# bogwi/sarpro

Measured on AMD Instinct MI355X. Metric: Mpix/s calibrate+CLAHE+synRGB, 400MP dual-pol scene; % HBM roofline, higher is better.
Workload: dtype f64

## Files before the change

### include/sarpro_hip.h

```cpp
#ifndef SARPRO_HIP_H
#define SARPRO_HIP_H

#include <stddef.h>
#include <stdint.h>

#ifdef __cplusplus
extern "C" {
#endif

#define SARPRO_HIP_OK 0
#define SARPRO_HIP_ERR_INVALID_ARG (-1)
#define SARPRO_HIP_ERR_SHAPE_MISMATCH (-2)
#define SARPRO_HIP_ERR_UNSUPPORTED_SHAPE (-3)
#define SARPRO_HIP_ERR_HIP (-4)
#define SARPRO_HIP_ERR_RCCL (-5)
#define SARPRO_HIP_ERR_OOM (-6)
#define SARPRO_HIP_ERR_NO_DEVICE (-7)
#define SARPRO_HIP_ERR_IO (-8)
#define SARPRO_HIP_ERR_BUFFER_TOO_SMALL (-9)

typedef enum {
    SARPRO_STRATEGY_STANDARD = 0,
    SARPRO_STRATEGY_ROBUST = 1,
    SARPRO_STRATEGY_ADAPTIVE = 2,
// ... 305 lines not shown
int sarpro_hip_stripe_run_resized_u16(sarpro_hip_ctx *ctx, const uint16_t *d_band1, const uint16_t *d_band2, size_t rows_total, size_t cols,
                                      size_t row0, size_t rows_local, size_t in_pitch, int strategy, int mode, size_t target_size, int pad,
                                      uint8_t *d_rgb_slice, size_t *out_row0, size_t *out_rows, sarpro_hip_resize_meta *meta);
int sarpro_hip_stripe_run_resized_f32(sarpro_hip_ctx *ctx, const float *d_band1, const float *d_band2, size_t rows_total, size_t cols, size_t row0,
                                      size_t rows_local, size_t in_pitch, int strategy, int mode, unsigned flags, size_t target_size, int pad,
                                      uint8_t *d_rgb_slice, size_t *out_row0, size_t *out_rows, sarpro_hip_resize_meta *meta);

int sarpro_hip_selftest_polop_division(sarpro_hip_ctx *ctx, uint64_t *mismatches_out);

typedef struct {
    uint64_t count;
    double sum_db, sumsq_db;
    float min_v, max_v;
} sarpro_hip_f32_partial;
typedef struct sarpro_hip_stripe_f32 sarpro_hip_stripe_f32;
int sarpro_hip_stripe_begin_f32(sarpro_hip_ctx *ctx, const float *d_in, size_t rows_total, size_t cols, size_t row0,
                                size_t rows_local, size_t in_pitch, int strategy, int bit_depth, void *d_out, size_t out_pitch,
                                sarpro_hip_stripe_f32 **out);
int sarpro_hip_stripe_begin_polop(sarpro_hip_ctx *ctx, int op, const void *d_a, const void *d_b, int elem_u16, size_t rows_total,
                                  size_t cols, size_t row0, size_t rows_local, size_t in_pitch, int strategy, int bit_depth,
                                  void *d_out, size_t out_pitch, sarpro_hip_stripe_f32 **out);
int sarpro_hip_stripe_f32_phase1(sarpro_hip_stripe_f32 *s, sarpro_hip_f32_partial *local_out);
int sarpro_hip_host_f32_merge_partials(const sarpro_hip_f32_partial *parts, size_t n, sarpro_hip_f32_partial *out);
int sarpro_hip_stripe_f32_phase2(sarpro_hip_stripe_f32 *s, const sarpro_hip_f32_partial *global, uint64_t **d_buf, size_t *count);
int sarpro_hip_stripe_f32_phase3(sarpro_hip_stripe_f32 *s, uint64_t **d_buf, size_t *count);
int sarpro_hip_stripe_f32_phase4(sarpro_hip_stripe_f32 *s, uint64_t **d_buf, size_t *count);
int sarpro_hip_stripe_f32_phase5(sarpro_hip_stripe_f32 *s, sarpro_hip_stats *stats_out);
void sarpro_hip_stripe_f32_end(sarpro_hip_stripe_f32 *s);
int sarpro_hip_stripe_run_f32(sarpro_hip_ctx *ctx, const float *d_in, size_t rows_total, size_t cols, size_t row0, size_t rows_local,
                              size_t in_pitch, int strategy, int bit_depth, void *d_out, size_t out_pitch, sarpro_hip_stats *stats_out);
int sarpro_hip_stripe_run_polop(sarpro_hip_ctx *ctx, int op, const void *d_a, const void *d_b, int elem_u16, size_t rows_total,
                                size_t cols, size_t row0, size_t rows_local, size_t in_pitch, int strategy, int bit_depth,
                                void *d_out, size_t out_pitch, sarpro_hip_stats *stats_out);

int sarpro_hip_comm_unique_id(uint8_t uid_out[128]);
int sarpro_hip_comm_init(sarpro_hip_ctx *ctx, int nranks, int rank, const uint8_t uid[128]);
int sarpro_hip_comm_allreduce_sum_u64(sarpro_hip_ctx *ctx, uint64_t *d_buf, size_t count);
typedef struct sarpro_hip_local_group sarpro_hip_local_group;
int sarpro_hip_local_group_create(int nranks, sarpro_hip_local_group **out);
void sarpro_hip_local_group_destroy(sarpro_hip_local_group *group);
int sarpro_hip_comm_init_local(sarpro_hip_ctx *ctx, sarpro_hip_local_group *group, int rank);
void sarpro_hip_comm_destroy(sarpro_hip_ctx *ctx);

int sarpro_hip_host_stats_from_dn_hist(const uint64_t dn_hist[65536], sarpro_hip_stats *out);
int sarpro_hip_host_window(sarpro_hip_stats *stats, int strategy, int tamed_synrgb);
int sarpro_hip_host_level_lut_u16(const sarpro_hip_stats *stats, int bit_depth, int tamed_synrgb,
                                  uint16_t lut_out[65536]);
int sarpro_hip_host_clahe_bin_lut_u16(const sarpro_hip_stats *stats, uint8_t lut_out[65536]);
int sarpro_hip_host_clahe_cdfs(const uint64_t *tile_hists, size_t rows, size_t cols,
                               double *cdfs_out);
int sarpro_hip_host_u8_rescale_lut(unsigned min_level, unsigned max_level, uint8_t lut_out[256]);
int sarpro_hip_host_synrgb_luts(int strategy, const uint64_t combined_hist[256], uint64_t n_per_band,
                                uint8_t *luts_out, int *floor_out);
int sarpro_hip_host_clahe_shape_ok(size_t rows, size_t cols);
int sarpro_hip_host_clahe_saturated_levels(size_t rows, size_t cols, uint8_t *col_class, uint8_t *row_bits);
int sarpro_hip_host_stripe_plan(size_t rows, int nranks, size_t *row0_out, size_t *nrows_out);

int sarpro_hip_host_stats_from_bins4096(uint64_t valid_count, double min_db, double max_db, double mean_db,
                                        double std_db, const uint64_t hist4096[4096], sarpro_hip_stats *out);
float sarpro_hip_host_f32_valid_threshold(void);
int sarpro_hip_host_f32_bin4096_thresholds(double min_db, double max_db, float thr_out[4096]);
int sarpro_hip_host_f32_level_thresholds(const sarpro_hip_stats *stats, int bit_depth, float *thr_out);
int sarpro_hip_host_f32_clahe_bin_thresholds(const sarpro_hip_stats *stats, float thr_out[256]);

int sarpro_hip_synth_scene_u16_dev(sarpro_hip_ctx *ctx, uint64_t seed, int band,
                                   const uint16_t *q_tables_host, size_t rows_total, size_t cols,
                                   size_t row0, size_t rows_local, uint16_t *d_out, size_t pitch);
#define SARPRO_HIP_SYNTH_NO_WEDGE 1u
#define SARPRO_HIP_SYNTH_NO_BRIGHT 2u
#define SARPRO_HIP_SYNTH_NO_BAND2 4u
#define SARPRO_HIP_SYNTH_MAP(m) (((unsigned)(m) & 15u) << 4)
#define SARPRO_HIP_SYNTH_BLOCKS(n) (((unsigned)(n) & 255u) << 8)
int sarpro_hip_synth_scene_u16_dev_ex(sarpro_hip_ctx *ctx, uint64_t seed, int band,
                                      const uint16_t *q_tables_host, size_t rows_total, size_t cols,
                                      size_t row0, size_t rows_local, uint16_t *d_out, size_t pitch, uint32_t flags);

#ifdef __cplusplus
}
#endif
#endif
```

### rust/sarpro-hip-sys/src/lib.rs

```rust
#![allow(non_camel_case_types, clippy::too_many_arguments)]

use std::os::raw::{c_char, c_int, c_uint, c_void};

pub const SARPRO_HIP_OK: c_int = 0;
pub const SARPRO_HIP_ERR_INVALID_ARG: c_int = -1;
pub const SARPRO_HIP_ERR_SHAPE_MISMATCH: c_int = -2;
pub const SARPRO_HIP_ERR_UNSUPPORTED_SHAPE: c_int = -3;
pub const SARPRO_HIP_ERR_HIP: c_int = -4;
pub const SARPRO_HIP_ERR_RCCL: c_int = -5;
pub const SARPRO_HIP_ERR_OOM: c_int = -6;
pub const SARPRO_HIP_ERR_NO_DEVICE: c_int = -7;
pub const SARPRO_HIP_ERR_IO: c_int = -8;
pub const SARPRO_HIP_ERR_BUFFER_TOO_SMALL: c_int = -9;
pub const SARPRO_HIP_CTX_TIMING: c_uint = 1;
pub const SARPRO_HIP_CTX_ASYNC_DEV: c_uint = 2;
pub const SARPRO_HIP_DUALPOL_PLAIN_PIPELINE: c_uint = 1;
pub const SARPRO_HIP_ROUTE_NONE: c_int = -1;
pub const SARPRO_HIP_ROUTE_ACCEPTED: c_int = 0;
pub const SARPRO_HIP_ROUTE_REFUTED: c_int = 1;
pub const SARPRO_HIP_ROUTE_UNPROVEN: c_int = 2;
pub const SARPRO_HIP_ROUTE_POOL_OVERFLOW: c_int = 3;
pub const SARPRO_HIP_ROUTE_RETRIED: c_int = 4;
pub const SARPRO_HIP_ERR_UNSUPPORTED: c_int = -10;
pub const SARPRO_HIP_SYNTH_NO_WEDGE: c_uint = 1;
pub const SARPRO_HIP_SYNTH_NO_BRIGHT: c_uint = 2;
pub const SARPRO_HIP_SYNTH_NO_BAND2: c_uint = 4;

pub const SARPRO_STRATEGY_STANDARD: c_int = 0;
pub const SARPRO_STRATEGY_ROBUST: c_int = 1;
pub const SARPRO_STRATEGY_ADAPTIVE: c_int = 2;
pub const SARPRO_STRATEGY_EQUALIZED: c_int = 3;
pub const SARPRO_STRATEGY_CLAHE: c_int = 4;
pub const SARPRO_STRATEGY_TAMED: c_int = 5;
pub const SARPRO_STRATEGY_DEFAULT: c_int = 6;
pub const SARPRO_BITDEPTH_U8: c_int = 0;
pub const SARPRO_BITDEPTH_U16: c_int = 1;
pub const SARPRO_OP_SUM: c_int = 0;
pub const SARPRO_OP_DIFF: c_int = 1;
pub const SARPRO_OP_RATIO: c_int = 2;
pub const SARPRO_OP_NDIFF: c_int = 3;
pub const SARPRO_OP_LOGRATIO: c_int = 4;
pub const SARPRO_SYNRGB_DEFAULT: c_int = 0;
pub const SARPRO_SYNRGB_RGB_RATIO: c_int = 1;
pub const SARPRO_SYNRGB_SAR_URBAN: c_int = 2;
pub const SARPRO_SYNRGB_ENHANCED: c_int = 3;
pub const SARPRO_READ_DEFAULT: c_int = -1;
pub const SARPRO_READ_AVERAGE: c_int = 0;
pub const SARPRO_READ_LANCZOS: c_int = 1;

#[repr(C)]
pub struct sarpro_hip_ctx { _private: [u8; 0] }
#[repr(C)]
pub struct sarpro_hip_stripe { _private: [u8; 0] }
#[repr(C)]
pub struct sarpro_hip_tiff { _private: [u8; 0] }
#[repr(C)]
pub struct sarpro_hip_tiff_writer { _private: [u8; 0] }
#[repr(C)]
pub struct sarpro_hip_stripe_f32 { _private: [u8; 0] }
#[repr(C)]
pub struct sarpro_hip_local_group { _private: [u8; 0] }

pub type sarpro_hip_row_reader = Option<unsafe extern "C" fn(user: *mut c_void, band: c_int, row0: usize, nrows: usize, dst: *mut u16, dst_pitch: usize) -> c_int>;
pub type sarpro_hip_row_sink = Option<unsafe extern "C" fn(user: *mut c_void, row0: usize, nrows: usize, src: *const u8, src_pitch_bytes: usize) -> c_int>;

#[repr(C)]
#[derive(Debug, Clone, Copy)]
pub struct sarpro_hip_stats {
    pub valid_count: u64,
    pub min_db: f64,
    pub max_db: f64,
    pub mean_db: f64,
    pub std_db: f64,
    pub median_db: f64,
    pub p01: f64,
    pub p02: f64,
// ... 181 lines not shown
    pub fn sarpro_hip_stripe_phase4(s: *mut sarpro_hip_stripe, d_rgb: *mut u8, rgb_pitch_px: usize, stats_out: *mut sarpro_hip_stats) -> c_int;
    pub fn sarpro_hip_stripe_end(s: *mut sarpro_hip_stripe);
    pub fn sarpro_hip_dualpol_synrgb_stream_u16(ctx: *mut sarpro_hip_ctx, reader: sarpro_hip_row_reader, reader_user: *mut c_void, rows: usize, cols: usize, strategy: c_int, mode: c_int, chunk_rows: usize, sink: sarpro_hip_row_sink, sink_user: *mut c_void, stats_out: *mut sarpro_hip_stats) -> c_int;
    pub fn sarpro_hip_dualpol_synrgb_resized_stream_u16(ctx: *mut sarpro_hip_ctx, reader: sarpro_hip_row_reader, reader_user: *mut c_void, rows: usize, cols: usize, strategy: c_int, mode: c_int, target_size: usize, pad: c_int, rgb_out: *mut u8, meta: *mut sarpro_hip_resize_meta) -> c_int;
    pub fn sarpro_hip_read_output_dims(cols: usize, rows: usize, target_size: usize, out_cols: *mut usize, out_rows: *mut usize, alg: *mut c_int) -> c_int;
    pub fn sarpro_hip_host_read_average_axis(n_src: usize, n_dst: usize, first: *mut u32, count: *mut u32, w_first: *mut f64, w_last: *mut f64, w_sum: *mut f64) -> c_int;
    pub fn sarpro_hip_read_average_u16_dev(ctx: *mut sarpro_hip_ctx, d_in: *const u16, rows: usize, cols: usize, in_pitch: usize, out_rows: usize, out_cols: usize, d_out_f32: *mut f32, out_pitch: usize) -> c_int;
    pub fn sarpro_hip_read_average_u16(ctx: *mut sarpro_hip_ctx, input: *const u16, rows: usize, cols: usize, out_rows: usize, out_cols: usize, out_f32: *mut f32) -> c_int;
    pub fn sarpro_hip_dualpol_synrgb_read_u16_dev(ctx: *mut sarpro_hip_ctx, d_band1: *const u16, d_band2: *const u16, rows: usize, cols: usize, in_pitch: usize, alg: c_int, strategy: c_int, mode: c_int, flags: c_uint, target_size: usize, pad: c_int, d_rgb_out: *mut u8, meta: *mut sarpro_hip_resize_meta) -> c_int;
    pub fn sarpro_hip_dualpol_synrgb_read_u16(ctx: *mut sarpro_hip_ctx, band1: *const u16, band2: *const u16, rows: usize, cols: usize, alg: c_int, strategy: c_int, mode: c_int, flags: c_uint, target_size: usize, pad: c_int, rgb_out: *mut u8, meta: *mut sarpro_hip_resize_meta) -> c_int;
    pub fn sarpro_hip_dualpol_synrgb_read_stream_u16(ctx: *mut sarpro_hip_ctx, reader: sarpro_hip_row_reader, reader_user: *mut c_void, rows: usize, cols: usize, alg: c_int, strategy: c_int, mode: c_int, flags: c_uint, target_size: usize, pad: c_int, rgb_out: *mut u8, meta: *mut sarpro_hip_resize_meta) -> c_int;
    pub fn sarpro_hip_dualpol_synrgb_read_stream_u16_jpeg(ctx: *mut sarpro_hip_ctx, reader: sarpro_hip_row_reader, reader_user: *mut c_void, rows: usize, cols: usize, alg: c_int, strategy: c_int, mode: c_int, flags: c_uint, target_size: usize, pad: c_int, jpeg_out: *mut u8, jpeg_capacity: usize, jpeg_bytes_out: *mut usize, restart_mcus: c_uint, meta: *mut sarpro_hip_resize_meta) -> c_int;
    pub fn sarpro_hip_tiff_open(path: *const c_char, out: *mut *mut sarpro_hip_tiff, info_out: *mut sarpro_hip_tiff_info) -> c_int;
    pub fn sarpro_hip_tiff_read_rows_u16(t: *mut sarpro_hip_tiff, sample: c_int, row0: usize, nrows: usize, dst: *mut u16, dst_pitch: usize) -> c_int;
    pub fn sarpro_hip_tiff_close(t: *mut sarpro_hip_tiff);
    pub fn sarpro_hip_tiff_pair_reader(user: *mut c_void, band: c_int, row0: usize, nrows: usize, dst: *mut u16, dst_pitch: usize) -> c_int;
    pub fn sarpro_hip_tiff_create(path: *const c_char, width: u64, height: u64, samples: u32, bits: u32, geotransform6: *const f64, geo_keys_from: *const sarpro_hip_tiff, out: *mut *mut sarpro_hip_tiff_writer) -> c_int;
    pub fn sarpro_hip_tiff_write_rows(w: *mut sarpro_hip_tiff_writer, row0: usize, nrows: usize, src: *const c_void, src_pitch_bytes: usize) -> c_int;
    pub fn sarpro_hip_tiff_row_sink(user: *mut c_void, row0: usize, nrows: usize, src: *const u8, src_pitch_bytes: usize) -> c_int;
    pub fn sarpro_hip_tiff_finish(w: *mut sarpro_hip_tiff_writer) -> c_int;
    pub fn sarpro_hip_tiff_last_error() -> *const c_char;
    pub fn sarpro_hip_host_parse_cpulist(s: *const c_char, cpus: *mut c_int, max: c_int) -> c_int;
    pub fn sarpro_hip_host_update_geotransform(gt: *mut f64, cols: usize, rows: usize, m: *const sarpro_hip_resize_meta);
    pub fn sarpro_hip_stripe_run_u16(ctx: *mut sarpro_hip_ctx, d_band1: *const u16, d_band2: *const u16, rows_total: usize, cols: usize, row0: usize, rows_local: usize, in_pitch: usize, strategy: c_int, mode: c_int, d_rgb: *mut u8, rgb_pitch_px: usize, stats_out: *mut sarpro_hip_stats) -> c_int;
    pub fn sarpro_hip_stripe_resized_rows(rows_total: usize, cols: usize, row0: usize, rows_local: usize, target_size: usize, pad: c_int, out_row0: *mut usize, out_rows: *mut usize, final_cols: *mut usize, final_rows: *mut usize) -> c_int;
    pub fn sarpro_hip_stripe_run_resized_u16(ctx: *mut sarpro_hip_ctx, d_band1: *const u16, d_band2: *const u16, rows_total: usize, cols: usize, row0: usize, rows_local: usize, in_pitch: usize, strategy: c_int, mode: c_int, target_size: usize, pad: c_int, d_rgb_slice: *mut u8, out_row0: *mut usize, out_rows: *mut usize, meta: *mut sarpro_hip_resize_meta) -> c_int;
    pub fn sarpro_hip_stripe_run_resized_f32(ctx: *mut sarpro_hip_ctx, d_band1: *const f32, d_band2: *const f32, rows_total: usize, cols: usize, row0: usize, rows_local: usize, in_pitch: usize, strategy: c_int, mode: c_int, flags: c_uint, target_size: usize, pad: c_int, d_rgb_slice: *mut u8, out_row0: *mut usize, out_rows: *mut usize, meta: *mut sarpro_hip_resize_meta) -> c_int;
    pub fn sarpro_hip_selftest_polop_division(ctx: *mut sarpro_hip_ctx, mismatches_out: *mut u64) -> c_int;
    pub fn sarpro_hip_stripe_begin_f32(ctx: *mut sarpro_hip_ctx, d_in: *const f32, rows_total: usize, cols: usize, row0: usize, rows_local: usize, in_pitch: usize, strategy: c_int, bit_depth: c_int, d_out: *mut c_void, out_pitch: usize, out: *mut *mut sarpro_hip_stripe_f32) -> c_int;
    pub fn sarpro_hip_stripe_begin_polop(ctx: *mut sarpro_hip_ctx, op: c_int, d_a: *const c_void, d_b: *const c_void, elem_u16: c_int, rows_total: usize, cols: usize, row0: usize, rows_local: usize, in_pitch: usize, strategy: c_int, bit_depth: c_int, d_out: *mut c_void, out_pitch: usize, out: *mut *mut sarpro_hip_stripe_f32) -> c_int;
    pub fn sarpro_hip_stripe_f32_phase1(s: *mut sarpro_hip_stripe_f32, local_out: *mut sarpro_hip_f32_partial) -> c_int;
    pub fn sarpro_hip_host_f32_merge_partials(parts: *const sarpro_hip_f32_partial, n: usize, out: *mut sarpro_hip_f32_partial) -> c_int;
    pub fn sarpro_hip_stripe_f32_phase2(s: *mut sarpro_hip_stripe_f32, global: *const sarpro_hip_f32_partial, d_buf: *mut *mut u64, count: *mut usize) -> c_int;
    pub fn sarpro_hip_stripe_f32_phase3(s: *mut sarpro_hip_stripe_f32, d_buf: *mut *mut u64, count: *mut usize) -> c_int;
    pub fn sarpro_hip_stripe_f32_phase4(s: *mut sarpro_hip_stripe_f32, d_buf: *mut *mut u64, count: *mut usize) -> c_int;
    pub fn sarpro_hip_stripe_f32_phase5(s: *mut sarpro_hip_stripe_f32, stats_out: *mut sarpro_hip_stats) -> c_int;
    pub fn sarpro_hip_stripe_f32_end(s: *mut sarpro_hip_stripe_f32);
    pub fn sarpro_hip_stripe_run_f32(ctx: *mut sarpro_hip_ctx, d_in: *const f32, rows_total: usize, cols: usize, row0: usize, rows_local: usize, in_pitch: usize, strategy: c_int, bit_depth: c_int, d_out: *mut c_void, out_pitch: usize, stats_out: *mut sarpro_hip_stats) -> c_int;
    pub fn sarpro_hip_stripe_run_polop(ctx: *mut sarpro_hip_ctx, op: c_int, d_a: *const c_void, d_b: *const c_void, elem_u16: c_int, rows_total: usize, cols: usize, row0: usize, rows_local: usize, in_pitch: usize, strategy: c_int, bit_depth: c_int, d_out: *mut c_void, out_pitch: usize, stats_out: *mut sarpro_hip_stats) -> c_int;
    pub fn sarpro_hip_comm_unique_id(uid_out: *mut u8) -> c_int;
    pub fn sarpro_hip_comm_init(ctx: *mut sarpro_hip_ctx, nranks: c_int, rank: c_int, uid: *const u8) -> c_int;
    pub fn sarpro_hip_comm_allreduce_sum_u64(ctx: *mut sarpro_hip_ctx, d_buf: *mut u64, count: usize) -> c_int;
    pub fn sarpro_hip_local_group_create(nranks: c_int, out: *mut *mut sarpro_hip_local_group) -> c_int;
    pub fn sarpro_hip_local_group_destroy(group: *mut sarpro_hip_local_group);
    pub fn sarpro_hip_comm_init_local(ctx: *mut sarpro_hip_ctx, group: *mut sarpro_hip_local_group, rank: c_int) -> c_int;
    pub fn sarpro_hip_comm_destroy(ctx: *mut sarpro_hip_ctx);
    pub fn sarpro_hip_host_stats_from_dn_hist(dn_hist: *const u64, out: *mut sarpro_hip_stats) -> c_int;
    pub fn sarpro_hip_host_window(stats: *mut sarpro_hip_stats, strategy: c_int, tamed_synrgb: c_int) -> c_int;
    pub fn sarpro_hip_host_level_lut_u16(stats: *const sarpro_hip_stats, bit_depth: c_int, tamed_synrgb: c_int, lut_out: *mut u16) -> c_int;
    pub fn sarpro_hip_host_clahe_bin_lut_u16(stats: *const sarpro_hip_stats, lut_out: *mut u8) -> c_int;
    pub fn sarpro_hip_host_clahe_cdfs(tile_hists: *const u64, rows: usize, cols: usize, cdfs_out: *mut f64) -> c_int;
    pub fn sarpro_hip_host_u8_rescale_lut(min_level: c_uint, max_level: c_uint, lut_out: *mut u8) -> c_int;
    pub fn sarpro_hip_host_synrgb_luts(strategy: c_int, combined_hist: *const u64, n_per_band: u64, luts_out: *mut u8, floor_out: *mut c_int) -> c_int;
    pub fn sarpro_hip_host_clahe_shape_ok(rows: usize, cols: usize) -> c_int;
    pub fn sarpro_hip_host_clahe_saturated_levels(rows: usize, cols: usize, col_class: *mut u8, row_bits: *mut u8) -> c_int;
    pub fn sarpro_hip_host_stripe_plan(rows: usize, nranks: c_int, row0_out: *mut usize, nrows_out: *mut usize) -> c_int;
    pub fn sarpro_hip_host_stats_from_bins4096(valid_count: u64, min_db: f64, max_db: f64, mean_db: f64, std_db: f64, hist4096: *const u64, out: *mut sarpro_hip_stats) -> c_int;
    pub fn sarpro_hip_host_f32_valid_threshold() -> f32;
    pub fn sarpro_hip_host_f32_bin4096_thresholds(min_db: f64, max_db: f64, thr_out: *mut f32) -> c_int;
    pub fn sarpro_hip_host_f32_level_thresholds(stats: *const sarpro_hip_stats, bit_depth: c_int, thr_out: *mut f32) -> c_int;
    pub fn sarpro_hip_host_f32_clahe_bin_thresholds(stats: *const sarpro_hip_stats, thr_out: *mut f32) -> c_int;
    pub fn sarpro_hip_synth_scene_u16_dev(ctx: *mut sarpro_hip_ctx, seed: u64, band: c_int, q_tables_host: *const u16, rows_total: usize, cols: usize, row0: usize, rows_local: usize, d_out: *mut u16, pitch: usize) -> c_int;
    pub fn sarpro_hip_synth_scene_u16_dev_ex(ctx: *mut sarpro_hip_ctx, seed: u64, band: c_int, q_tables_host: *const u16, rows_total: usize, cols: usize, row0: usize, rows_local: usize, d_out: *mut u16, pitch: usize, flags: u32) -> c_int;
}
```

### sarpro_amd/__init__.py

```python
from .types import AutoscaleStrategy, BitDepth, PolarizationOperation, SyntheticRgbMode
from .api import (LocalGroup, Context, SarproHipError, Stripe, StripeF32, host_f32_merge_partials, comm_unique_id, host_clahe_bin_lut_u16,
                  host_clahe_cdfs, host_clahe_saturated_levels, host_clahe_shape_ok, host_level_lut_u16, host_stats_from_dn_hist,
                  host_stripe_plan, host_stripe_resized_rows, host_synrgb_luts, host_u8_rescale_lut, host_window,
                  host_f32_valid_threshold, host_f32_bin4096_thresholds, host_f32_level_thresholds,
                  host_f32_clahe_bin_thresholds, host_stats_from_bins4096, resize_output_dims, host_jpeg_header, jpeg_bound,
                  read_output_dims, host_read_average_axis,
                  batch_dualpol_synrgb_resized, batch_dualpol_synrgb_resized_f32, TiffReader, TiffPair, TiffWriter, host_update_geotransform)
from ._lib import Stats, F32Partial
```

### sarpro_amd/_lib.py

```python
from __future__ import annotations

import ctypes as C
import os

_HERE = os.path.dirname(os.path.abspath(__file__))
LIB_PATH = os.environ.get("SARPRO_HIP_LIB") or os.path.join(_HERE, "libsarpro_hip.so")

OK = 0
ERR_INVALID_ARG, ERR_SHAPE_MISMATCH, ERR_UNSUPPORTED_SHAPE = -1, -2, -3
ERR_HIP, ERR_RCCL, ERR_OOM, ERR_NO_DEVICE, ERR_IO = -4, -5, -6, -7, -8
ERR_BUFFER_TOO_SMALL = -9
ERR_UNSUPPORTED = -10
READ_DEFAULT, READ_AVERAGE, READ_LANCZOS = -1, 0, 1


class Stats(C.Structure):
    _fields_ = [("valid_count", C.c_uint64)] + [
        (n, C.c_double)
        for n in ("min_db", "max_db", "mean_db", "std_db", "median_db", "p01", "p02", "p05", "p10",
                  "p25", "p75", "p90", "p95", "p98", "p99", "low_clip", "high_clip", "gamma",
                  "skew_factor", "tail_heaviness")
    ]

    def as_dict(self):
# ... 16 lines not shown
    ] + [("pixel_scale", C.c_double * 3), ("tiepoint", C.c_double * 6)]


ROW_READER = C.CFUNCTYPE(C.c_int, C.c_void_p, C.c_int, C.c_size_t, C.c_size_t, C.c_void_p, C.c_size_t)
ROW_SINK = C.CFUNCTYPE(C.c_int, C.c_void_p, C.c_size_t, C.c_size_t, C.c_void_p, C.c_size_t)


class BatchScene(C.Structure):
    _fields_ = [("band1", C.c_void_p), ("band2", C.c_void_p), ("rows", C.c_size_t), ("cols", C.c_size_t),
                ("rgb_out", C.c_void_p), ("status_out", C.POINTER(C.c_int)), ("reader", C.c_void_p), ("reader_user", C.c_void_p)]


class BatchSceneF32(C.Structure):
    _fields_ = [("band1", C.c_void_p), ("band2", C.c_void_p), ("rows", C.c_size_t), ("cols", C.c_size_t),
                ("rgb_out", C.c_void_p), ("status_out", C.POINTER(C.c_int))]


class ResidentSceneF32(C.Structure):
    _fields_ = [("d_band1", C.c_void_p), ("d_band2", C.c_void_p), ("d_rgb", C.c_void_p), ("status", C.c_int)]


class ResidentScene(C.Structure):
    _fields_ = [("d_band1", C.c_void_p), ("d_band2", C.c_void_p), ("d_rgb", C.c_void_p), ("status", C.c_int), ("route", C.c_int)]


class BatchReport(C.Structure):
    _fields_ = [("processed", C.c_size_t), ("skipped", C.c_size_t), ("errors", C.c_size_t)]


SYMBOLS = [
    "sarpro_hip_ctx_create", "sarpro_hip_ctx_destroy", "sarpro_hip_last_error", "sarpro_hip_version",
    "sarpro_hip_ctx_stream", "sarpro_hip_ctx_synchronize",
    "sarpro_hip_autoscale_band_f32", "sarpro_hip_autoscale_band_u16", "sarpro_hip_db_mask_f32",
    "sarpro_hip_tamed_synrgb_u8_f32", "sarpro_hip_tamed_synrgb_u8_u16", "sarpro_hip_polop_f32",
    "sarpro_hip_synrgb_u8", "sarpro_hip_dualpol_synrgb_u16", "sarpro_hip_dualpol_synrgb_f32",
    "sarpro_hip_autoscale_band_u16_dev", "sarpro_hip_autoscale_band_f32_dev",
    "sarpro_hip_polop_autoscale_band_f32", "sarpro_hip_polop_autoscale_band_u16", "sarpro_hip_polop_autoscale_band_f32_dev", "sarpro_hip_polop_autoscale_band_u16_dev",
    "sarpro_hip_dualpol_synrgb_u16_dev", "sarpro_hip_polop_f32_dev", "sarpro_hip_synrgb_u8_dev",
    "sarpro_hip_last_kernel_times",
    "sarpro_hip_ctx_time_only", "sarpro_hip_ctx_spec_report", "sarpro_hip_ctx_chain_report",
    "sarpro_hip_stripe_begin_u16", "sarpro_hip_stripe_phase1", "sarpro_hip_stripe_phase2",
    "sarpro_hip_stripe_phase3", "sarpro_hip_stripe_phase4", "sarpro_hip_stripe_end", "sarpro_hip_stripe_run_u16", "sarpro_hip_stripe_resized_rows", "sarpro_hip_stripe_run_resized_u16", "sarpro_hip_stripe_run_resized_f32",
    "sarpro_hip_dualpol_synrgb_stream_u16", "sarpro_hip_dualpol_synrgb_resized_stream_u16", "sarpro_hip_tiff_open", "sarpro_hip_tiff_read_rows_u16", "sarpro_hip_tiff_close",
    "sarpro_hip_tiff_pair_reader", "sarpro_hip_tiff_create", "sarpro_hip_tiff_write_rows", "sarpro_hip_tiff_row_sink",
    "sarpro_hip_tiff_finish", "sarpro_hip_tiff_last_error", "sarpro_hip_host_update_geotransform",
    "sarpro_hip_selftest_polop_division",
    "sarpro_hip_stripe_begin_f32", "sarpro_hip_stripe_begin_polop", "sarpro_hip_stripe_f32_phase1", "sarpro_hip_stripe_f32_phase2",
    "sarpro_hip_stripe_f32_phase3", "sarpro_hip_stripe_f32_phase4", "sarpro_hip_stripe_f32_phase5", "sarpro_hip_stripe_f32_end",
    "sarpro_hip_stripe_run_f32", "sarpro_hip_stripe_run_polop", "sarpro_hip_host_f32_merge_partials",
    "sarpro_hip_comm_unique_id", "sarpro_hip_comm_init", "sarpro_hip_comm_allreduce_sum_u64",
    "sarpro_hip_comm_destroy",
    "sarpro_hip_host_stats_from_dn_hist", "sarpro_hip_host_window", "sarpro_hip_host_level_lut_u16",
    "sarpro_hip_host_clahe_bin_lut_u16", "sarpro_hip_host_clahe_cdfs", "sarpro_hip_host_u8_rescale_lut",
    "sarpro_hip_host_synrgb_luts", "sarpro_hip_host_clahe_shape_ok", "sarpro_hip_host_parse_cpulist", "sarpro_hip_host_stripe_plan",
    "sarpro_hip_host_stats_from_bins4096", "sarpro_hip_host_f32_valid_threshold", "sarpro_hip_host_f32_bin4096_thresholds",
    "sarpro_hip_host_f32_level_thresholds", "sarpro_hip_host_f32_clahe_bin_thresholds",
    "sarpro_hip_resize_output_dims", "sarpro_hip_resize_image_data", "sarpro_hip_resize_image_data_dev",
    "sarpro_hip_dualpol_synrgb_resized_u16", "sarpro_hip_dualpol_synrgb_resized_u16_dev", "sarpro_hip_dualpol_synrgb_f32_dev",
    "sarpro_hip_dualpol_synrgb_resized_f32", "sarpro_hip_dualpol_synrgb_resized_f32_dev", "sarpro_hip_batch_dualpol_synrgb_resized_f32", "sarpro_hip_process_band_resized_u16", "sarpro_hip_process_band_resized_f32",
    "sarpro_hip_batch_dualpol_synrgb_resized_u16", "sarpro_hip_batch_dualpol_synrgb_u16_dev", "sarpro_hip_batch_dualpol_synrgb_resized_f32_dev",
    "sarpro_hip_synth_scene_u16_dev", "sarpro_hip_synth_scene_u16_dev_ex",
    "sarpro_hip_local_group_create", "sarpro_hip_local_group_destroy", "sarpro_hip_comm_init_local", "sarpro_hip_host_clahe_saturated_levels", "sarpro_hip_ctx_set_attr", "sarpro_hip_ctx_reset_attr", "sarpro_hip_ctx_get_attr", "sarpro_hip_attr_name",
    "sarpro_hip_host_jpeg_header", "sarpro_hip_jpeg_bound", "sarpro_hip_jpeg_encode_dev", "sarpro_hip_jpeg_encode",
    "sarpro_hip_dualpol_synrgb_resized_u16_jpeg", "sarpro_hip_dualpol_synrgb_resized_f32_jpeg",
    "sarpro_hip_read_output_dims", "sarpro_hip_host_read_average_axis", "sarpro_hip_read_average_u16_dev", "sarpro_hip_read_average_u16",
    "sarpro_hip_dualpol_synrgb_read_u16_dev", "sarpro_hip_dualpol_synrgb_read_u16", "sarpro_hip_dualpol_synrgb_read_stream_u16",
    "sarpro_hip_dualpol_synrgb_read_stream_u16_jpeg",
]

if not os.path.exists(LIB_PATH):
    raise ImportError(
        f"{LIB_PATH} is missing: build it first (python -c 'import __graft_entry__ as g; g.build()' "
        "or make -C sarpro_amd/csrc). sarpro_amd has no fallback implementation.")



def _share_hip_runtime_with_torch():
    if os.environ.get("SARPRO_HIP_RUNTIME", "") == "system":
        return
    try:
        import importlib.util
        spec = importlib.util.find_spec("torch")
        if spec is None or not spec.submodule_search_locations:
            return
        cand = os.path.join(list(spec.submodule_search_locations)[0], "lib", "libamdhip64.so")
        if os.path.exists(cand):
            C.CDLL(cand, mode=C.RTLD_GLOBAL)
    except Exception:
        pass


_share_hip_runtime_with_torch()
lib = C.CDLL(LIB_PATH)

_vp, _sz, _i, _u64 = C.c_void_p, C.c_size_t, C.c_int, C.c_uint64
_S = C.POINTER(Stats)


def _proto(name, restype, *argtypes):
    f = getattr(lib, name)
    f.restype = restype
    f.argtypes = list(argtypes)


_proto("sarpro_hip_ctx_create", _i, _i, C.c_uint, C.POINTER(_vp))
_proto("sarpro_hip_ctx_destroy", None, _vp)
_proto("sarpro_hip_last_error", C.c_char_p, _vp)
# ... 23 lines not shown


class SpecReport(C.Structure):
    _fields_ = [("spec_ok", C.c_uint32), ("verdict", C.c_uint32), ("floor_pred", C.c_int32), ("pool_overflow", C.c_uint32),
                ("n_lt", C.c_uint64 * 2), ("target", C.c_uint64), ("est_lt", C.c_double * 2), ("sample_valid", C.c_uint64 * 2),
                ("n_below_min", C.c_uint64), ("min_pred", C.c_uint32 * 2), ("retried", C.c_uint32), ("floor_first", C.c_int32)]


_proto("sarpro_hip_ctx_spec_report", _i, _vp, C.POINTER(SpecReport))


class ChainReport(C.Structure):
    _fields_ = [("floor_with_cushion", C.c_int32), ("identity", C.c_uint8 * 2), ("reserved", C.c_uint8 * 2),
                ("rescale", C.c_uint8 * 512), ("level_hist", C.c_uint64 * 512)]


_proto("sarpro_hip_ctx_chain_report", _i, _vp, C.POINTER(ChainReport))
_proto("sarpro_hip_ctx_set_attr", _i, _vp, C.c_char_p, C.c_int64)
_proto("sarpro_hip_ctx_reset_attr", _i, _vp, C.c_char_p)
_proto("sarpro_hip_ctx_get_attr", _i, _vp, C.c_char_p, C.POINTER(C.c_int64), C.POINTER(C.c_int))
_proto("sarpro_hip_attr_name", C.c_char_p, _i)
_proto("sarpro_hip_stripe_begin_u16", _i, _vp, _vp, _vp, _sz, _sz, _sz, _sz, _sz, _i, _i, C.POINTER(_vp))
_proto("sarpro_hip_stripe_phase1", _i, _vp, C.POINTER(_vp), C.POINTER(_sz))
_proto("sarpro_hip_stripe_phase2", _i, _vp, C.POINTER(_vp), C.POINTER(_sz))
_proto("sarpro_hip_stripe_phase3", _i, _vp, C.POINTER(_vp), C.POINTER(_sz))
_proto("sarpro_hip_stripe_phase4", _i, _vp, _vp, _sz, _S)
_proto("sarpro_hip_stripe_end", None, _vp)
_proto("sarpro_hip_selftest_polop_division", _i, _vp, C.POINTER(C.c_uint64))
_proto("sarpro_hip_stripe_begin_f32", _i, _vp, _vp, _sz, _sz, _sz, _sz, _sz, _i, _i, _vp, _sz, C.POINTER(_vp))
_proto("sarpro_hip_stripe_begin_polop", _i, _vp, _i, _vp, _vp, _i, _sz, _sz, _sz, _sz, _sz, _i, _i, _vp, _sz, C.POINTER(_vp))
_proto("sarpro_hip_stripe_f32_phase1", _i, _vp, C.POINTER(F32Partial))
_proto("sarpro_hip_stripe_f32_phase2", _i, _vp, C.POINTER(F32Partial), C.POINTER(_vp), C.POINTER(_sz))
_proto("sarpro_hip_stripe_f32_phase3", _i, _vp, C.POINTER(_vp), C.POINTER(_sz))
_proto("sarpro_hip_stripe_f32_phase4", _i, _vp, C.POINTER(_vp), C.POINTER(_sz))
_proto("sarpro_hip_stripe_f32_phase5", _i, _vp, _S)
_proto("sarpro_hip_stripe_f32_end", None, _vp)
_proto("sarpro_hip_stripe_run_f32", _i, _vp, _vp, _sz, _sz, _sz, _sz, _sz, _i, _i, _vp, _sz, _S)
_proto("sarpro_hip_stripe_run_polop", _i, _vp, _i, _vp, _vp, _i, _sz, _sz, _sz, _sz, _sz, _i, _i, _vp, _sz, _S)
_proto("sarpro_hip_host_f32_merge_partials", _i, _vp, _sz, C.POINTER(F32Partial))
_proto("sarpro_hip_comm_unique_id", _i, _vp)
_proto("sarpro_hip_comm_init", _i, _vp, _i, _i, _vp)
_proto("sarpro_hip_comm_allreduce_sum_u64", _i, _vp, _vp, _sz)
_proto("sarpro_hip_local_group_create", _i, _i, C.POINTER(_vp))
_proto("sarpro_hip_local_group_destroy", None, _vp)
_proto("sarpro_hip_comm_init_local", _i, _vp, _vp, _i)
_proto("sarpro_hip_comm_destroy", None, _vp)
_proto("sarpro_hip_host_stats_from_dn_hist", _i, _vp, _S)
_proto("sarpro_hip_host_window", _i, _S, _i, _i)
_proto("sarpro_hip_host_level_lut_u16", _i, _S, _i, _i, _vp)
_proto("sarpro_hip_host_clahe_bin_lut_u16", _i, _S, _vp)
_proto("sarpro_hip_host_clahe_cdfs", _i, _vp, _sz, _sz, _vp)
_proto("sarpro_hip_host_u8_rescale_lut", _i, C.c_uint, C.c_uint, _vp)
_proto("sarpro_hip_host_synrgb_luts", _i, _i, _vp, _u64, _vp, C.POINTER(_i))
_proto("sarpro_hip_host_clahe_shape_ok", _i, _sz, _sz)
_proto("sarpro_hip_host_clahe_saturated_levels", _i, _sz, _sz, _vp, _vp)
_proto("sarpro_hip_host_stripe_plan", _i, _sz, _i, _vp, _vp)
_proto("sarpro_hip_synth_scene_u16_dev", _i, _vp, _u64, _i, _vp, _sz, _sz, _sz, _sz, _vp, _sz)
_proto("sarpro_hip_synth_scene_u16_dev_ex", _i, _vp, _u64, _i, _vp, _sz, _sz, _sz, _sz, _vp, _sz, C.c_uint32)
_proto("sarpro_hip_host_f32_valid_threshold", C.c_float)
_proto("sarpro_hip_host_f32_bin4096_thresholds", _i, C.c_double, C.c_double, _vp)
_proto("sarpro_hip_host_f32_level_thresholds", _i, _S, _i, _vp)
_proto("sarpro_hip_host_f32_clahe_bin_thresholds", _i, _S, _vp)
_proto("sarpro_hip_host_stats_from_bins4096", _i, _u64, C.c_double, C.c_double, C.c_double, C.c_double, _vp, _S)
_M = C.POINTER(ResizeMeta)
_proto("sarpro_hip_resize_output_dims", _i, _sz, _sz, _sz, _i, C.POINTER(_sz), C.POINTER(_sz))
_proto("sarpro_hip_resize_image_data", _i, _vp, _vp, _sz, _sz, _sz, _i, _i, _vp, _M)
_proto("sarpro_hip_resize_image_data_dev", _i, _vp, _vp, _sz, _sz, _sz, _sz, _i, _i, _vp, _sz, _M)
_proto("sarpro_hip_dualpol_synrgb_resized_u16", _i, _vp, _vp, _vp, _sz, _sz, _i, _i, _sz, _i, _vp, _M)
_proto("sarpro_hip_host_parse_cpulist", _i, C.c_char_p, _vp, _i)
_u = C.c_uint
_proto("sarpro_hip_dualpol_synrgb_f32_dev", _i, _vp, _vp, _vp, _sz, _sz, _sz, _i, _i, _u, _vp, _sz, _vp, _vp, _sz, C.POINTER(Stats))
_proto("sarpro_hip_dualpol_synrgb_resized_f32", _i, _vp, _vp, _vp, _sz, _sz, _i, _i, _u, _sz, _i, _vp, _M)
_proto("sarpro_hip_dualpol_synrgb_resized_f32_dev", _i, _vp, _vp, _vp, _sz, _sz, _sz, _i, _i, _u, _sz, _i, _vp, _M)
_proto("sarpro_hip_batch_dualpol_synrgb_resized_f32", _i, C.POINTER(C.c_int), _i, _i, C.POINTER(BatchSceneF32), _sz, _i, _i, _u, _sz, _i, _i, C.POINTER(BatchReport))
_proto("sarpro_hip_dualpol_synrgb_resized_u16_dev", _i, _vp, _vp, _vp, _sz, _sz, _sz, _i, _i, _sz, _i, _vp, _M)
_proto("sarpro_hip_process_band_resized_u16", _i, _vp, _vp, _sz, _sz, _i, _i, _sz, _i, _vp, _M)
_proto("sarpro_hip_process_band_resized_f32", _i, _vp, _vp, _sz, _sz, _i, _i, _sz, _i, _vp, _M)
_proto("sarpro_hip_batch_dualpol_synrgb_resized_u16", _i, C.POINTER(_i), _i, _i, C.POINTER(BatchScene), _sz, _i, _i, _sz, _i, _i,
       C.POINTER(BatchReport))
_proto("sarpro_hip_batch_dualpol_synrgb_resized_f32_dev", _i, _vp, C.POINTER(ResidentSceneF32), _sz, _sz, _sz, _sz, _i, _i, C.c_uint, _sz, _i, _i, _i, C.POINTER(BatchReport))
_proto("sarpro_hip_batch_dualpol_synrgb_u16_dev", _i, _vp, C.POINTER(ResidentScene), _sz, _sz, _sz, _sz, _i, _i, _sz, _i, _i, C.POINTER(BatchReport))
_proto("sarpro_hip_stripe_run_u16", _i, _vp, _vp, _vp, _sz, _sz, _sz, _sz, _sz, _i, _i, _vp, _sz, _S)
_proto("sarpro_hip_stripe_resized_rows", _i, _sz, _sz, _sz, _sz, _sz, _i, C.POINTER(_sz), C.POINTER(_sz), C.POINTER(_sz), C.POINTER(_sz))
_proto("sarpro_hip_stripe_run_resized_u16", _i, _vp, _vp, _vp, _sz, _sz, _sz, _sz, _sz, _i, _i, _sz, _i, _vp, C.POINTER(_sz), C.POINTER(_sz), _M)
_proto("sarpro_hip_stripe_run_resized_f32", _i, _vp, _vp, _vp, _sz, _sz, _sz, _sz, _sz, _i, _i, C.c_uint, _sz, _i, _vp, C.POINTER(_sz), C.POINTER(_sz), _M)
_proto("sarpro_hip_dualpol_synrgb_stream_u16", _i, _vp, _vp, _vp, _sz, _sz, _i, _i, _sz, _vp, _vp, _S)
_proto("sarpro_hip_tiff_open", _i, C.c_char_p, C.POINTER(_vp), C.POINTER(TiffInfo))
_proto("sarpro_hip_tiff_read_rows_u16", _i, _vp, _i, _sz, _sz, _vp, _sz)
_proto("sarpro_hip_tiff_close", None, _vp)
_proto("sarpro_hip_tiff_pair_reader", _i, _vp, _i, _sz, _sz, _vp, _sz)
_proto("sarpro_hip_tiff_create", _i, C.c_char_p, _u64, _u64, C.c_uint32, C.c_uint32, _vp, _vp, C.POINTER(_vp))
_proto("sarpro_hip_tiff_write_rows", _i, _vp, _sz, _sz, _vp, _sz)
_proto("sarpro_hip_tiff_row_sink", _i, _vp, _sz, _sz, _vp, _sz)
_proto("sarpro_hip_tiff_finish", _i, _vp)
_proto("sarpro_hip_tiff_last_error", C.c_char_p)
_proto("sarpro_hip_host_update_geotransform", None, _vp, _sz, _sz, _M)
_proto("sarpro_hip_dualpol_synrgb_resized_stream_u16", _i, _vp, _vp, _vp, _sz, _sz, _i, _i, _sz, _i, _vp, _M)
_proto("sarpro_hip_host_jpeg_header", _i, _sz, _sz, _i, _u, _vp, _sz, C.POINTER(_sz))
_proto("sarpro_hip_jpeg_bound", _i, _sz, _sz, _i, _u, C.POINTER(_sz))
_proto("sarpro_hip_jpeg_encode_dev", _i, _vp, _vp, _sz, _sz, _sz, _i, _u, _vp, _sz, C.POINTER(_sz))
_proto("sarpro_hip_jpeg_encode", _i, _vp, _vp, _sz, _sz, _sz, _i, _u, _vp, _sz, C.POINTER(_sz))
_proto("sarpro_hip_dualpol_synrgb_resized_u16_jpeg", _i, _vp, _vp, _vp, _sz, _sz, _i, _i, _sz, _i, _vp, _sz, C.POINTER(_sz), _u, _M)
_proto("sarpro_hip_dualpol_synrgb_resized_f32_jpeg", _i, _vp, _vp, _vp, _sz, _sz, _i, _i, _u, _sz, _i, _vp, _sz, C.POINTER(_sz), _u, _M)
_proto("sarpro_hip_read_output_dims", _i, _sz, _sz, _sz, C.POINTER(_sz), C.POINTER(_sz), C.POINTER(_i))
_proto("sarpro_hip_host_read_average_axis", _i, _sz, _sz, _vp, _vp, _vp, _vp, _vp)
_proto("sarpro_hip_read_average_u16_dev", _i, _vp, _vp, _sz, _sz, _sz, _sz, _sz, _vp, _sz)
# ... 6 lines not shown
```

### sarpro_amd/api.py

```python
from __future__ import annotations

import ctypes as C

import numpy as np

from . import _lib
from ._lib import F32Partial, Stats, lib
from .types import AutoscaleStrategy, BitDepth, PolarizationOperation, SyntheticRgbMode


class SarproHipError(RuntimeError):

    def __init__(self, code: int, msg: str):
        super().__init__(f"sarpro_hip status {code}: {msg}")
        self.code = code


def _vp(a):
    if a is None:
        return None
    if isinstance(a, np.ndarray):
        return a.ctypes.data_as(C.c_void_p)
    return C.c_void_p(int(a))

# ... 732 lines not shown
        raise SarproHipError(rc, "host_stats_from_dn_hist")
    return st


def host_window(st: Stats, strategy, tamed_synrgb: int = 0) -> Stats:
    rc = lib.sarpro_hip_host_window(C.byref(st), int(strategy), tamed_synrgb)
    if rc:
        raise SarproHipError(rc, "host_window")
    return st


def host_level_lut_u16(st: Stats, bit_depth, tamed_synrgb: int = 0) -> np.ndarray:
    lut = np.empty(65536, np.uint16)
    rc = lib.sarpro_hip_host_level_lut_u16(C.byref(st), int(bit_depth), tamed_synrgb, _vp(lut))
    if rc:
        raise SarproHipError(rc, "host_level_lut_u16")
    return lut


def host_clahe_bin_lut_u16(st: Stats) -> np.ndarray:
    lut = np.empty(65536, np.uint8)
    rc = lib.sarpro_hip_host_clahe_bin_lut_u16(C.byref(st), _vp(lut))
    if rc:
        raise SarproHipError(rc, "host_clahe_bin_lut_u16")
    return lut


def host_clahe_cdfs(tile_hists: np.ndarray, rows: int, cols: int) -> np.ndarray:
    th = np.ascontiguousarray(tile_hists, np.uint64)
    assert th.size == 64 * 256
    cdfs = np.empty((64, 256), np.float64)
    rc = lib.sarpro_hip_host_clahe_cdfs(_vp(th), rows, cols, _vp(cdfs))
    if rc:
        raise SarproHipError(rc, "host_clahe_cdfs")
    return cdfs


def host_u8_rescale_lut(min_level: int, max_level: int) -> np.ndarray:
    lut = np.empty(256, np.uint8)
    rc = lib.sarpro_hip_host_u8_rescale_lut(min_level, max_level, _vp(lut))
    if rc:
        raise SarproHipError(rc, "host_u8_rescale_lut")
    return lut


def host_synrgb_luts(strategy, combined_hist: np.ndarray | None = None, n_per_band: int = 0):
    luts = np.empty(66048, np.uint8)
    fl = C.c_int(-1)
    h = None if combined_hist is None else np.ascontiguousarray(combined_hist, np.uint64)
    rc = lib.sarpro_hip_host_synrgb_luts(int(strategy), _vp(h), n_per_band, _vp(luts), C.byref(fl))
    if rc:
        raise SarproHipError(rc, "host_synrgb_luts")
    return luts[:256].copy(), luts[256:512].copy(), luts[512:].reshape(256, 256).copy(), fl.value


def host_clahe_saturated_levels(rows: int, cols: int):
    cc, rb = np.zeros(cols, np.uint8), np.zeros(rows, np.uint8)
    rc = lib.sarpro_hip_host_clahe_saturated_levels(rows, cols, _vp(cc), _vp(rb))
    if rc != _lib.OK:
        raise SarproHipError(rc, "no saturation table for this shape")
    return cc, rb


def host_clahe_shape_ok(rows: int, cols: int) -> bool:
    return bool(lib.sarpro_hip_host_clahe_shape_ok(rows, cols))


def host_stripe_plan(rows: int, nranks: int):
    r0 = np.empty(nranks, np.uint64)
    nr = np.empty(nranks, np.uint64)
    rc = lib.sarpro_hip_host_stripe_plan(rows, nranks, _vp(r0), _vp(nr))
    if rc:
        raise SarproHipError(rc, "host_stripe_plan")
    return [int(x) for x in r0], [int(x) for x in nr]


def host_stripe_resized_rows(rows_total: int, cols: int, row0: int, rows_local: int, target_size: int, pad: bool):
    v = [C.c_size_t() for _ in range(4)]
    rc = lib.sarpro_hip_stripe_resized_rows(rows_total, cols, row0, rows_local, int(target_size or 0), int(bool(pad)), *[C.byref(x) for x in v])
    if rc:
        raise SarproHipError(rc, "stripe_resized_rows")
    return tuple(int(x.value) for x in v)


def host_f32_valid_threshold() -> float:
    return float(lib.sarpro_hip_host_f32_valid_threshold())


def host_f32_bin4096_thresholds(min_db: float, max_db: float) -> np.ndarray:
    thr = np.empty(4096, np.float32)
    rc = lib.sarpro_hip_host_f32_bin4096_thresholds(min_db, max_db, _vp(thr))
    if rc:
        raise SarproHipError(rc, "host_f32_bin4096_thresholds")
    return thr


def host_f32_level_thresholds(st: Stats, bit_depth) -> np.ndarray:
    thr = np.empty(256 if int(bit_depth) == 0 else 65536, np.float32)
    rc = lib.sarpro_hip_host_f32_level_thresholds(C.byref(st), int(bit_depth), _vp(thr))
    if rc:
        raise SarproHipError(rc, "host_f32_level_thresholds")
    return thr


def host_f32_clahe_bin_thresholds(st: Stats) -> np.ndarray:
    thr = np.empty(256, np.float32)
# ... 184 lines not shown
```

### sarpro_amd/csrc/api_u16_chain.cpp

```cpp
#include <algorithm>
#include <chrono>
#include <cstdio>
#include <cstdlib>
#include <cstring>
#include <future>
#include <string>

#include "api_common.h"
#include "chain_kernels.h"
#include "context.h"
#include "internal.h"
#include "resize_kernels.h"
#include "u16_job.h"

using namespace sarpro;

namespace sarpro {

constexpr size_t kChainOffDb = 0, kChainOffSupp = 65536 * 8, kChainOffBlue = kChainOffSupp + 21504;
constexpr size_t kChainOffBlueDef = kChainOffBlue + 65536, kChainOffDefRg = kChainOffBlueDef + 65536;
constexpr size_t kChainOffGamma = kChainOffDefRg + 512, kChainOffBluePQ = kChainOffGamma + 3 * 256 * 8, kChainConstBytes = kChainOffBluePQ + 512 * 4;
constexpr size_t kTablesOffPQ = 66048 + 512, kTablesBytes = kTablesOffPQ + 2 * 256 * 4;
constexpr size_t kStateOffResc = 2 * sizeof(ChainBandState), kStateOffIdent = kStateOffResc + 512,
                 kStateOffFloor = kStateOffIdent + 16, kStateBytes = kStateOffFloor + 16;

extern "C" int sarpro_hip_ctx_chain_report(sarpro_hip_ctx *ctx, sarpro_hip_chain_report *out) {
    if (!ctx || !out) return SARPRO_HIP_ERR_INVALID_ARG;
    memset(out, 0, sizeof(*out));
    out->floor_with_cushion = -1;
    if (!ctx->chain_state.p || !ctx->last_final_hist) return fail(ctx, SARPRO_HIP_ERR_INVALID_ARG, "no CLAHE chain has run on this context");
    HIPCHK(ctx, hipSetDevice(ctx->device));
    HIPCHK(ctx, hipStreamSynchronize(ctx->stream));
    const uint8_t *state = ctx->chain_state.as<uint8_t>();
    HIPCHK(ctx, hipMemcpy(out->rescale, state + kStateOffResc, 512, hipMemcpyDeviceToHost));
    HIPCHK(ctx, hipMemcpy(out->identity, state + kStateOffIdent, 2, hipMemcpyDeviceToHost));
    HIPCHK(ctx, hipMemcpy(&out->floor_with_cushion, state + kStateOffFloor, sizeof(int32_t), hipMemcpyDeviceToHost));
    HIPCHK(ctx, hipMemcpy(out->level_hist, ctx->last_final_hist, sizeof(out->level_hist), hipMemcpyDeviceToHost));
    return SARPRO_HIP_OK;
}


static int chain_prepare(sarpro_hip_ctx *ctx) {
    if (ctx->chain_ready) return SARPRO_HIP_OK;
    HIPCHK(ctx, ctx->chain_consts.reserve(kChainConstBytes));
    HIPCHK(ctx, ctx->chain_state.reserve(kStateBytes));
    uint8_t *d = ctx->chain_consts.as<uint8_t>();
    HIPCHK(ctx, hipMemcpyAsync(d + kChainOffDb, db_table_u16(), 65536 * 8, hipMemcpyHostToDevice, ctx->stream));
    HIPCHK(ctx, hipMemcpyAsync(d + kChainOffSupp, synrgb_supp_rg_tables(), 41 * 512, hipMemcpyHostToDevice, ctx->stream));
    HIPCHK(ctx, hipMemcpyAsync(d + kChainOffBlue, synrgb_blue_pair_supp(), 65536, hipMemcpyHostToDevice, ctx->stream));
    HIPCHK(ctx, hipMemcpyAsync(d + kChainOffBlueDef, synrgb_blue_pair_default(), 65536, hipMemcpyHostToDevice, ctx->stream));
    std::vector<uint8_t> dflt(66048);
    synrgb_luts_default(dflt.data());
    HIPCHK(ctx, hipMemcpyAsync(d + kChainOffDefRg, dflt.data(), 512, hipMemcpyHostToDevice, ctx->stream));
    HIPCHK(ctx, hipMemcpyAsync(d + kChainOffGamma, gamma_level_thresholds_u8(), 3 * 256 * 8, hipMemcpyHostToDevice, ctx->stream));
    if (const float *pq = synrgb_blue_factors_supp()) {
        HIPCHK(ctx, hipMemcpyAsync(d + kChainOffBluePQ, pq, 512 * 4, hipMemcpyHostToDevice, ctx->stream));
        ctx->blue_factors_ok = true;
    }
    HIPCHK(ctx, hipStreamSynchronize(ctx->stream));
    ctx->chain_ready = true;
    return SARPRO_HIP_OK;
}

bool chain_eligible(const U16Job &J) {
    if (J.ctx->attrs.on(A_NO_CHAIN)) return false;
    return J.clahe() && (J.u8_out() || !J.synrgb) && J.vec && !J.tamed_force && (J.reduce || (J.row0 == 0 && J.rows_local == J.rows_total));
}

static int chain_stats_scratch(sarpro_hip_ctx *ctx, ChainStatsArgs *sa) {
    const size_t part_bytes = (sizeof(ChainStatsPartial) * kChainStatsParts * kMaxBands + 255) & ~(size_t)255;
    HIPCHK(ctx, ctx->chain_scratch.reserve(part_bytes + sizeof(uint64_t) * 4096 * kMaxBands));
    sa->partials = ctx->chain_scratch.as<ChainStatsPartial>();
    sa->bins4096 = reinterpret_cast<unsigned long long *>(ctx->chain_scratch.as<uint8_t>() + part_bytes);
    return SARPRO_HIP_OK;
}
// ... 16 lines not shown
    uint32_t hi = 0;
    for (int b = 0; b < J.nbands; ++b) {
        J.stats[b] = h_state[b].stats;
        if (stats_out) stats_out[b] = J.stats[b];
        hi = std::max(hi, h_state[b].win_hi);
    }
    ctx->chain_lut_cap = std::min<uint32_t>(16384, std::max<uint32_t>(1024, (hi + 1 + 255) / 256 * 256));
    return SARPRO_HIP_OK;
}

constexpr size_t kSampledHistMinPx = 32u << 20;
static uint32_t spec_force_flags(const sarpro_hip_ctx *ctx) {
    return (uint32_t)ctx->attrs.val(A_SPEC_FORCE, 0) & (kSpecForceMispredict | kSpecForceNoSpec | kSpecForceMinMispredict | kSpecForceNoRetry | kSpecForceMispredict2);
}

static int chain_tail(U16Job &J, sarpro_hip_stats *stats_out, ChainBandState *d_state);

struct FusedTail {
    sarpro_hip_ctx *ctx; U16Job *J; ClaheRgbArgs fa; ClaheApplyArgs a; ChainSpecState *d_spec; ChainBandState *d_state;
    unsigned long long *exact_hist; StripePlan *plan; uint8_t *d_levels[2]; size_t lvl_pitch; uint32_t rows, cols;
    unsigned long long total_px; uint8_t *d_rgb; size_t rgb_pitch_px;
    ChainPredictArgs pa;
};
static int fused_rgb_tail(const FusedTail &T) {
    sarpro_hip_ctx *ctx = T.ctx;
    uint8_t *consts = ctx->chain_consts.as<uint8_t>(), *state = ctx->chain_state.as<uint8_t>();
    ChainSpecState *d_spec = T.d_spec;
    ClaheApplyArgs a = T.a;
    const bool reduce = T.J && T.J->reduce;
    {
        if (ctx->pipe_wait_before_fused) HIPCHK(ctx, hipStreamWaitEvent(ctx->stream, ctx->pipe_wait_before_fused, 0));
        if (ctx->pipe_record_before_fused) { HIPCHK(ctx, hipEventRecord(ctx->pipe_record_before_fused, ctx->stream)); ctx->pipe_record_before_fused = nullptr; }
        int grid = std::max(ctx->cu_count, 1);
        if (ctx->attrs.is_set(A_RGB_GRID)) grid = (int)std::min<long long>(1024, std::max<long long>(1, ctx->attrs.val(A_RGB_GRID, grid)));
        {
            KernelTimer t(ctx, "clahe_rgb_fused");
            HIPCHK(ctx, launch_clahe_rgb_fused(T.fa, grid, ctx->stream));
        }
        if (ctx->pipe_record_after_fused) {
            HIPCHK(ctx, hipEventRecord(ctx->pipe_record_after_fused, ctx->stream));
            ctx->pipe_record_after_fused = nullptr;
        }
    }
    if (reduce) {
        static_assert(offsetof(ChainSpecState, n_below_min) == offsetof(ChainSpecState, n_lt) + 16 && offsetof(ChainSpecState, below_hist) == offsetof(ChainSpecState, n_lt) + 24,
                      "the verification counts are one buffer");
        RETCHK(chain_reduce(*T.J, &d_spec->n_lt[0], kSpecCountWords, "allreduce_spec_counts"));
        HIPCHK(ctx, launch_spec_verdict(d_spec, T.d_state, ctx->stream));
    }
    {
        ChainRepredictArgs ra{};
        ra.spec = d_spec; ra.resc_in = state + kStateOffResc; ra.floor_out = reinterpret_cast<int *>(state + kStateOffFloor);
        ra.tables = ctx->tables.as<uint8_t>(); ra.supp_rg = consts + kChainOffSupp; ra.blue_pair_supp = consts + kChainOffBlue;
        ra.blue_pq = ctx->blue_factors_ok ? reinterpret_cast<const float *>(consts + kChainOffBluePQ) : nullptr;
        ra.blue_by_level = reinterpret_cast<float *>(ctx->tables.as<uint8_t>() + kTablesOffPQ);
        ra.stripes = reduce ? 1u : 0u;
        {
            KernelTimer t(ctx, "chain_repredict");
            HIPCHK(ctx, launch_chain_repredict(ra, ctx->stream));
            {
                ChainPredictArgs p2 = T.pa;
                p2.second = 1u;
                HIPCHK(ctx, launch_chain_predict(p2, ctx->stream));
            }
        }
        ClaheRgbArgs fr = T.fa;
        fr.retry = 1u;
        int grid = std::max(ctx->cu_count, 1);
        if (ctx->attrs.is_set(A_RGB_GRID)) grid = (int)std::min<long long>(1024, std::max<long long>(1, ctx->attrs.val(A_RGB_GRID, grid)));
        {
            KernelTimer t(ctx, "clahe_rgb_fused_retry");
            HIPCHK(ctx, launch_clahe_rgb_fused_retry(fr, grid, ctx->stream));
        }
        if (reduce) {
            RETCHK(chain_reduce(*T.J, &d_spec->n_lt[0], kSpecCountWords, "allreduce_spec_counts_retry"));
            HIPCHK(ctx, launch_spec_verdict(d_spec, T.d_state, ctx->stream, 1));
        }
    }
    {
        KernelTimer t(ctx, "spec_fallback_apply");
        a.hist_mode = 0u; a.gate = d_spec;
        a.rects = T.plan->d_apply_rects.as<Rect>();
        for (int b = 0; b < 2; ++b) a.level_hist[b] = T.exact_hist + (size_t)b * 256;
        HIPCHK(ctx, launch_clahe_apply_u8_spec(a, (int)T.plan->apply_rects.size(), 2, ctx->stream));
    }
    if (reduce) RETCHK(chain_reduce(*T.J, T.exact_hist, (size_t)256 * kMaxBands, "allreduce_level_hist"));
    {
        ChainFinishArgs f{};
        f.level_hist = T.exact_hist; f.gate = d_spec;
        f.total_px = T.total_px; f.nbands = 2;
        f.resc_out = state + kStateOffResc; f.identity_out = state + kStateOffIdent;
        f.tables = ctx->tables.as<uint8_t>();
        f.supp_rg = consts + kChainOffSupp; f.blue_pair_supp = consts + kChainOffBlue;
        f.floor_out = reinterpret_cast<int *>(state + kStateOffFloor);
        f.suppressed = 1;
        KernelTimer t(ctx, "chain_finish");
        HIPCHK(ctx, launch_chain_finish(f, ctx->stream));
    }
    {
        ComposeArgs c{};
        c.b1 = T.d_levels[0]; c.b2 = T.d_levels[1]; c.in_pitch = T.lvl_pitch;
        c.rgb = T.d_rgb; c.rgb_pitch_px = T.rgb_pitch_px; c.rows = T.rows; c.cols = T.cols;
        c.tables = ctx->tables.as<uint8_t>();
        c.spec = d_spec; c.speculative = 0;
        KernelTimer t(ctx, "spec_fallback_compose");
        HIPCHK(ctx, launch_compose_u8(c, 16, ctx->stream));
    }
    return SARPRO_HIP_OK;
}

static int job_run_fused_rgb(U16Job &J, const ClaheRgbArgs &fa, uint8_t *d_rgb, size_t rgb_pitch_px, uint32_t sample_stride,
                             sarpro_hip_stats *stats_out) {
    sarpro_hip_ctx *ctx = J.ctx;
    uint8_t *consts = ctx->chain_consts.as<uint8_t>(), *state = ctx->chain_state.as<uint8_t>();
    ChainBandState *d_state = reinterpret_cast<ChainBandState *>(state);
    ChainSpecState *d_spec = ctx->spec_state.as<ChainSpecState>();
    const uint32_t rows = (uint32_t)J.rows_local, cols = (uint32_t)J.cols;
    RETCHK(ensure_levels(J));
    HIPCHK(ctx, ctx->spec_dump.reserve(kSpecDumpBytes));
    unsigned long long *sample_hist = ctx->level_hist.as<unsigned long long>(), *exact_hist = sample_hist + 256 * kMaxBands * kSampleReplicas;
    ctx->last_final_hist = exact_hist;
    ClaheApplyArgs a{};
    for (int b = 0; b < 2; ++b) {
        a.in[b] = J.d_in[b];
        a.out[b] = J.d_levels[b];
        a.cdfs[b] = fa.cdfs[b];
        a.binlut[b] = fa.binlut[b];
        a.level_hist[b] = sample_hist + (size_t)b * 256;
    }
    a.in_pitch = J.in_pitch; a.out_pitch = J.lvl_pitch;
    a.row_w = fa.row_w; a.col_w = fa.col_w; a.row_off = fa.row_off;
    a.max_val = 255.0; a.dev_state = d_state; a.lut_cap = ctx->chain_lut_cap;
    a.dump = ctx->spec_dump.as<uint8_t>();
    a.sample_stride = sample_stride; a.sample_phase = sample_stride / 2; a.sample_valid = d_spec->sample_valid_rep;
    {
        a.hist_mode = 3u;
        a.rects = J.plan->d_sample_rects.as<Rect>();
        KernelTimer t(ctx, "clahe_sample");
        HIPCHK(ctx, launch_clahe_apply_u8_spec(a, (int)J.plan->sample_rects.size(), 2, ctx->stream));
    }
    RETCHK(chain_reduce(J, sample_hist, (size_t)256 * kMaxBands * kSampleReplicas, "allreduce_sample_hist"));
    RETCHK(chain_reduce(J, d_spec->sample_valid_rep, (size_t)kSampleReplicas * 2, "allreduce_sample_valid"));
    ChainPredictArgs pa_first{};
    {
        ChainPredictArgs pa{};
        pa.sample_hist = sample_hist; pa.exact_hist = exact_hist; pa.spec = d_spec; pa.state = d_state;
        pa.total_px = (unsigned long long)J.rows_total * J.cols;
        pa.resc_out = state + kStateOffResc; pa.identity_out = state + kStateOffIdent;
        pa.floor_out = reinterpret_cast<int *>(state + kStateOffFloor);
        pa.tables = ctx->tables.as<uint8_t>();
        pa.supp_rg = consts + kChainOffSupp; pa.blue_pair_supp = consts + kChainOffBlue;
        pa.force = spec_force_flags(ctx);
        pa.allow_rescaled = ctx->attrs.on(A_NO_SPEC_RESCALE) ? 0u : 1u;
        pa.blue_pq = ctx->blue_factors_ok ? reinterpret_cast<const float *>(consts + kChainOffBluePQ) : nullptr;
        pa.blue_by_level = reinterpret_cast<float *>(ctx->tables.as<uint8_t>() + kTablesOffPQ);
        pa_first = pa;
        KernelTimer t(ctx, "chain_predict");
        HIPCHK(ctx, launch_chain_predict(pa, ctx->stream));
    }
    FusedTail T{};
    T.ctx = ctx; T.J = &J; T.fa = fa; T.a = a; T.d_spec = d_spec; T.d_state = d_state; T.exact_hist = exact_hist;
    T.plan = J.plan; T.d_levels[0] = J.d_levels[0]; T.d_levels[1] = J.d_levels[1]; T.lvl_pitch = J.lvl_pitch;
    T.rows = rows; T.cols = cols; T.total_px = (unsigned long long)J.rows_total * J.cols; T.d_rgb = d_rgb; T.rgb_pitch_px = rgb_pitch_px;
    T.pa = pa_first;
    if (ctx->pipe_defer && !J.reduce && ctx->async_dev && J.allow_async && !stats_out) {
        T.J = nullptr;
        ctx->pipe_deferred = [T]() { return fused_rgb_tail(T); };
        ctx->async_pending = ctx->timing;
        return SARPRO_HIP_OK;
    }
    RETCHK(fused_rgb_tail(T));
    return chain_tail(J, stats_out, d_state);
}

int job_run_chain(U16Job &J, void *const d_out[kMaxBands], size_t out_pitch, uint8_t *d_rgb, size_t rgb_pitch_px,
                         sarpro_hip_stats *stats_out) {
    sarpro_hip_ctx *ctx = J.ctx;
    RETCHK(chain_prepare(ctx));
    const uint32_t rows = (uint32_t)J.rows_local, cols = (uint32_t)J.cols;
    HIPCHK(ctx, ctx->luts.reserve(2 * 131072));
    HIPCHK(ctx, ctx->tile_bins.reserve(sizeof(uint64_t) * 64 * 256 * kMaxBands));
    HIPCHK(ctx, ctx->cdfs.reserve(sizeof(double) * 64 * 256 * kMaxBands));
    HIPCHK(ctx, ctx->level_hist.reserve(sizeof(uint64_t) * 256 * kMaxBands * (kSampleReplicas + 1)));
    HIPCHK(ctx, ctx->tables.reserve(kTablesBytes));
    HIPCHK(ctx, ctx->h_small.reserve(sizeof(uint64_t) * 64 * 256 * kMaxBands + sizeof(uint64_t) * 256 * kMaxBands));
    uint8_t *consts = ctx->chain_consts.as<uint8_t>(), *state = ctx->chain_state.as<uint8_t>();
    ChainBandState *d_state = reinterpret_cast<ChainBandState *>(state);
    const bool exact_only = ctx->attrs.on(A_NO_SPEC);
    const size_t rgb_pitch_ok = rgb_pitch_px % 16 == 0 && ptr_aligned16(d_rgb);
    const bool whole = J.row0 == 0 && J.rows_local == J.rows_total;
    const bool fused_wanted = !d_out[0] && !d_out[1] && !ctx->attrs.on(A_NO_FUSED_RGB) && J.in_pitch % 8 == 0;
    bool sampled = J.synrgb && J.nbands == 2 && J.u8_out() && !exact_only && !ctx->attrs.on(A_FULL_LEVEL_HIST) &&
                   !ctx->attrs.on(A_NO_SAMPLED_HIST) && rgb_pitch_px % 16 == 0 && (J.reduce ? fused_wanted : (d_rgb && rgb_pitch_ok && whole));
    uint32_t sample_stride = J.rows_total >= 12000 ? 33 : 17;
    if (sampled) {
        size_t min_px = kSampledHistMinPx;
        if (ctx->attrs.is_set(A_SAMPLED_HIST_MIN_PX)) min_px = (size_t)std::max<long long>(0, ctx->attrs.val(A_SAMPLED_HIST_MIN_PX, 0));
        if (ctx->attrs.is_set(A_SAMPLE_STRIDE)) sample_stride = (uint32_t)std::max<long long>(5, ctx->attrs.val(A_SAMPLE_STRIDE, 0));
        if ((size_t)J.rows_total * J.cols < min_px) sampled = false;
    }
    ChainSpecState *d_spec = nullptr;
    ctx->spec_ran = sampled;
    if (sampled) {
        HIPCHK(ctx, ctx->spec_state.reserve(sizeof(ChainSpecState)));
        d_spec = ctx->spec_state.as<ChainSpecState>();
    }

    RETCHK(job_phase1(J));
    RETCHK(chain_reduce(J, ctx->ghist.p, 65536 * (size_t)J.nbands, "allreduce_dn_hist"));
    {
        ChainStatsArgs sa{};
        sa.ghist = ctx->ghist.as<unsigned long long>();
        sa.db = reinterpret_cast<const double *>(consts + kChainOffDb);
        sa.state = d_state;
        sa.binlut = ctx->luts.as<uint8_t>();
        sa.binlut_stride = 131072;
        sa.level_hist = ctx->level_hist.as<unsigned long long>();
        sa.sample_valid = d_spec ? d_spec->sample_valid_rep : nullptr;
        KernelTimer t(ctx, "chain_stats");
        RETCHK(chain_stats_scratch(ctx, &sa));
        HIPCHK(ctx, launch_chain_stats(sa, J.nbands, ctx->stream));
    }
    {
        TileBinHistArgs ta{};
        for (int b = 0; b < J.nbands; ++b) {
            ta.tile_hist[b] = tile_hist_of(ctx, b, kTiles * kTiles);
            ta.binlut[b] = ctx->luts.as<uint8_t>() + (size_t)b * 131072;
            ta.out[b] = ctx->tile_bins.as<unsigned long long>() + (size_t)b * 64 * 256;
        }
        ta.clear = 1u;
        if (!J.reduce && !ctx->attrs.on(A_SEPARATE_CDFS)) {
            for (int b = 0; b < J.nbands; ++b) ta.cdfs_out[b] = ctx->cdfs.as<double>() + (size_t)b * 64 * 256;
            ta.rows = (uint32_t)J.rows_total; ta.cols = cols;
        }
        KernelTimer t(ctx, "tile_bin_hist");
        HIPCHK(ctx, launch_tile_bin_hist(ta, kTiles * kTiles, J.nbands, ctx->stream));
        mark_tile_hist_clean(J);
    }
    RETCHK(chain_reduce(J, ctx->tile_bins.p, 64 * 256 * (size_t)J.nbands, "allreduce_tile_hists"));
    if (J.reduce || ctx->attrs.on(A_SEPARATE_CDFS)) {
        KernelTimer t(ctx, "chain_cdfs");
        HIPCHK(ctx, launch_chain_cdfs(ctx->tile_bins.as<unsigned long long>(), ctx->cdfs.as<double>(), (uint32_t)J.rows_total, cols,
                                      J.nbands, ctx->stream));
    }
    if (sampled && fused_wanted && (J.reduce || !J.plan->rgb_rects.empty())) {
        ClaheRgbArgs fa{};
        for (int b = 0; b < 2; ++b) {
            fa.in[b] = J.d_in[b];
            fa.cdfs[b] = ctx->cdfs.as<double>() + (size_t)b * 64 * 256;
            fa.binlut[b] = ctx->luts.as<uint8_t>() + (size_t)b * 131072;
        }
        fa.in_pitch = J.in_pitch; fa.rgb = d_rgb; fa.rgb_pitch_px = rgb_pitch_px;
        fa.rects = J.plan->d_rgb_rects.as<Rect>(); fa.nrects = (int)J.plan->rgb_rects.size();
        fa.row_w = J.plan->d_row_w.as<RowWeight>(); fa.col_w = J.plan->d_col_w.as<RowWeight>(); fa.row_off = (int32_t)J.row0;
        fa.dev_state = d_state; fa.spec = d_spec; fa.tables = ctx->tables.as<uint8_t>();
        fa.blue_by_level = ctx->blue_factors_ok ? reinterpret_cast<const float *>(ctx->tables.as<uint8_t>() + kTablesOffPQ) : nullptr;
        fa.sat_ok = J.plan->sat_ok ? 1u : 0u; fa.sat_col = J.plan->d_sat_col.as<uint8_t>(); fa.sat_row = J.plan->d_sat_row.as<uint8_t>() + J.row0;
        fa.sat_cols = (uint32_t)(round_up(J.cols, 64) + 64);
        const uint32_t fused_stride = ctx->attrs.is_set(A_SAMPLE_STRIDE) ? sample_stride : 33u;
        fa.no_verdict = J.reduce ? 1u : 0u;
        if (clahe_rgb_fused_supported(fa)) return job_run_fused_rgb(J, fa, d_rgb, rgb_pitch_px, fused_stride, stats_out);
        if (J.reduce) return fail(ctx, SARPRO_HIP_ERR_INVALID_ARG, "row stripe: the rasters of every rank must be 16-byte aligned (pitches % 8 / % 16)");
    }
    const bool direct = !J.synrgb;
    if (!direct) RETCHK(ensure_levels(J));
    ClaheApplyArgs a{};
    for (int b = 0; b < J.nbands; ++b) {
        a.in[b] = J.d_in[b];
        a.out[b] = direct ? d_out[b] : (void *)J.d_levels[b];
        a.cdfs[b] = ctx->cdfs.as<double>() + (size_t)b * 64 * 256;
        a.binlut[b] = ctx->luts.as<uint8_t>() + (size_t)b * 131072;
        a.level_hist[b] = ctx->level_hist.as<unsigned long long>() + (size_t)b * 256;
    }
    a.in_pitch = J.in_pitch;
    a.out_pitch = direct ? out_pitch : J.lvl_pitch;
    a.rects = J.plan->d_apply_rects.as<Rect>();
    a.row_w = J.plan->d_row_w.as<RowWeight>();
    a.col_w = J.plan->d_col_w.as<RowWeight>();
    a.row_off = (int32_t)J.row0;
    const bool u16o = !J.u8_out();
    a.max_val = u16o ? 65535.0 : 255.0;
    a.dev_state = d_state;
    a.lut_cap = ctx->chain_lut_cap;
    if (a.out_pitch % 8 != 0 || !ptr_aligned16(a.out[0]) || (J.nbands > 1 && !ptr_aligned16(a.out[1])))
        return fail(ctx, SARPRO_HIP_ERR_INVALID_ARG, "output raster must be 16-byte aligned with pitch % 8 == 0 when the input is");
    if (u16o) {
        for (int b = 0; b < J.nbands; ++b) a.level_hist[b] = nullptr;
        {
            KernelTimer t(ctx, "clahe_apply_u16");
            if (!ctx->attrs.on(A_NO_U16_CF) && J.nbands <= kMaxBands && J.plan->u16_nwg[J.nbands - 1] > 0 &&
                clahe_apply_u16_cf_supported(a, J.nbands, J.plan->u16_item_rows)) {
                a.rects = J.plan->d_u16_items[J.nbands - 1].as<Rect>();
                HIPCHK(ctx, launch_clahe_apply_u16_cf(a, J.plan->d_u16_first[J.nbands - 1].as<int32_t>(), J.plan->u16_nwg[J.nbands - 1], J.nbands, ctx->stream));
            } else {
                HIPCHK(ctx, launch_clahe_apply_u16(a, (int)J.plan->apply_rects.size(), J.nbands, true, true, ctx->stream));
            }
        }
        ChainBandState *h_state = ctx->h_small.as<ChainBandState>();
        HIPCHK(ctx, hipMemcpyAsync(h_state, d_state, sizeof(ChainBandState) * (size_t)J.nbands, hipMemcpyDeviceToHost, ctx->stream));
        HIPCHK(ctx, hipStreamSynchronize(ctx->stream));
        uint32_t hi = 0;
        for (int b = 0; b < J.nbands; ++b) {
            J.stats[b] = h_state[b].stats;
            if (stats_out) stats_out[b] = J.stats[b];
            hi = std::max(hi, h_state[b].win_hi);
        }
        ctx->chain_lut_cap = std::min<uint32_t>(16384, std::max<uint32_t>(1024, (hi + 1 + 255) / 256 * 256));
        return SARPRO_HIP_OK;
    }
// ... 245 lines not shown
```

### sarpro_amd/csrc/chain_kernels.h

```cpp
#pragma once
#include "kernels.h"

namespace sarpro {

struct ChainBandState {
    sarpro_hip_stats stats;
    uint32_t win_hi;
    uint32_t uncertain;
};

struct ChainStatsPartial {
    unsigned long long count;
    uint32_t min_dn, max_dn;
    double sum1, sum2;
};
constexpr int kChainStatsParts = 16;

struct ChainStatsArgs {
    const unsigned long long *ghist;
    const double *db;
    ChainBandState *state;
    uint8_t *binlut;
    size_t binlut_stride;
    int levels_mode;
// ... 6 lines not shown
    const double *gamma_thr;
    ChainStatsPartial *partials;
    unsigned long long *bins4096;
};

struct ChainFinishArgs {
    const unsigned long long *level_hist;
    unsigned long long total_px;
    int nbands;
    uint8_t *resc_out;
    uint8_t *identity_out;
    uint8_t *tables;
    const uint8_t *supp_rg;
    const uint8_t *blue_pair_supp;
    int *floor_out;
    int levels_mode;
    int no_rescale[2];
    int suppressed;
    uint8_t *dn_tables;
    size_t dn_table_stride;
    const uint8_t *default_rg;
    const uint8_t *blue_pair_default;
    const ChainSpecState *gate;
};

hipError_t launch_chain_stats(const ChainStatsArgs &a, int nbands, hipStream_t s);
hipError_t launch_chain_cdfs(const unsigned long long *tile_bins, double *cdfs, uint32_t rows, uint32_t cols, int nbands,
                             hipStream_t s);
hipError_t launch_chain_finish(const ChainFinishArgs &a, hipStream_t s);
hipError_t launch_level_hist_guard(unsigned long long *level_hist, unsigned long long total_px, int nbands, uint32_t *d_flags,
                                   hipStream_t s);
struct LevelRecountArgs {
    const uint8_t *levels[kMaxBands];
    size_t pitch;
    uint32_t rows, cols;
    unsigned long long *level_hist;
    const uint32_t *flags;
    const ChainSpecState *gate;
};
struct ChainPredictArgs {
    const unsigned long long *sample_hist;
    unsigned long long *exact_hist;
    ChainSpecState *spec;
    const ChainBandState *state;
    unsigned long long total_px;
    uint8_t *resc_out, *identity_out;
    int *floor_out;
    uint8_t *tables;
    const uint8_t *supp_rg;
    const uint8_t *blue_pair_supp;
    uint32_t force;
    uint32_t allow_rescaled;
    const float *blue_pq;
    float *blue_by_level;
    uint32_t second;
};
hipError_t launch_chain_predict(const ChainPredictArgs &a, hipStream_t s);
struct ChainRepredictArgs {
    ChainSpecState *spec;
    const uint8_t *resc_in;
    int *floor_out;
    uint8_t *tables;
    const uint8_t *supp_rg;
    const uint8_t *blue_pair_supp;
    const float *blue_pq;
    float *blue_by_level;
    uint32_t stripes;
};
hipError_t launch_chain_repredict(const ChainRepredictArgs &a, hipStream_t s);
hipError_t launch_level_hist_if_flagged(const LevelRecountArgs &a, int nbands, hipStream_t s);
hipError_t launch_chain_remap(const uint8_t *src, size_t src_pitch, uint8_t *dst, size_t dst_pitch, uint32_t rows,
                              uint32_t cols, const uint8_t *d_map, const uint8_t *d_skip_flag, hipStream_t s);

}
```

### sarpro_amd/csrc/chain_kernels.hip

```cpp
#include "chain_kernels.h"
#include "device_cdf.h"

#include <cfloat>

namespace sarpro {
namespace {

constexpr int kStatsBlock = 1024;
constexpr int kTileDns = 256;

__device__ inline double clampd(double x, double lo, double hi) { return x < lo ? lo : (x > hi ? hi : x); }

constexpr int kStatsParts = kChainStatsParts;
constexpr int kPartBlock = 256;
constexpr int kPartDns = 65536 / kStatsParts;
constexpr int kPartWaveDns = kPartDns / (kPartBlock / 64);

template <typename T, typename Op>
__device__ T part_reduce(T v, T *scratch , Op op) {
#pragma unroll
    for (int m = 32; m > 0; m >>= 1) v = op(v, __shfl_xor(v, m, 64));
    __syncthreads();
    if ((threadIdx.x & 63) == 0) scratch[threadIdx.x >> 6] = v;
    __syncthreads();
// ... 416 lines not shown
    if (t < 256) for (int b = 0; b < a.nbands; ++b) atomicAdd(&combined[resc[b][t]], lh[b][t]);
    const bool lead = blockIdx.x == 0;
    if (lead && t < 512 && a.resc_out) a.resc_out[t] = (t >> 8) < a.nbands ? resc[t >> 8][t & 255] : (uint8_t)(t & 255);
    if (lead && wb < a.nbands && a.identity_out) {
        bool ident = true;
#pragma unroll
        for (int k = 0; k < 4; ++k) if (lh[wb][ln * 4 + k] && resc[wb][ln * 4 + k] != ln * 4 + k) ident = false;
        const bool all = __builtin_amdgcn_ballot_w64(!ident) == 0ull;
        if (ln == 0) a.identity_out[wb] = all ? 1 : 0;
    }
    __syncthreads();
    if (a.levels_mode)
        for (int i = blockIdx.x * kStatsBlock + t; i < 2 * 65536; i += gridDim.x * kStatsBlock) {
            const int b = i >> 16;
            if (b < a.nbands) { uint8_t *p = a.dn_tables + (size_t)b * a.dn_table_stride + (i & 65535); *p = resc[b][*p]; }
        }
    if (a.nbands < 2 || !a.tables) return;
    if (t == 0 && a.suppressed) {
        const uint32_t total = (uint32_t)(a.total_px + a.total_px);
        const double tc = round((double)total * 0.05);
        const uint32_t target = tc >= 4294967295.0 ? 4294967295u : (uint32_t)tc;
        uint32_t cumulative = 0;
        int floor_value = 0;
        for (int i = 0; i < 256; ++i) {
            const unsigned long long hi = combined[i] > 4294967295ull ? 4294967295ull : combined[i];
            const unsigned long long c = (unsigned long long)cumulative + hi;
            cumulative = c > 4294967295ull ? 4294967295u : (uint32_t)c;
            if (cumulative >= target) { floor_value = i; break; }
        }
        const int fwc = floor_value + 3 < 40 ? floor_value + 3 : 40;
        s_fwc = fwc;
        if (lead && a.floor_out) *a.floor_out = fwc;
    }
    __syncthreads();
    const int fwc = a.suppressed ? s_fwc : -1;
    const uint8_t *lut_r = a.suppressed ? a.supp_rg + (size_t)fwc * 512 : a.default_rg, *lut_g = lut_r + 256;
    const uint8_t *pair = a.suppressed ? a.blue_pair_supp : a.blue_pair_default;
    uint8_t *R2 = a.tables, *G2 = a.tables + 256, *B2 = a.tables + 512;
    const bool fold = !a.levels_mode;
    if (lead && t < 256) {
        const int r1 = fold ? resc[0][t] : t, r2 = fold ? resc[1][t] : t;
        R2[t] = r1 <= fwc ? 0 : lut_r[r1];
        G2[t] = r2 <= fwc ? 0 : lut_g[r2];
    }
    for (int i = blockIdx.x * kStatsBlock + t; i < 65536; i += gridDim.x * kStatsBlock) {
        const int v1 = i >> 8, v2 = i & 255;
        const int r1 = fold ? resc[0][v1] : v1, r2 = fold ? resc[1][v2] : v2;
        const bool water = r1 <= fwc && r2 <= fwc;
        const bool b2zero = !a.suppressed && r2 == 0;
        B2[i] = (water || b2zero) ? 0 : pair[((size_t)lut_r[r1] << 8) | lut_g[r2]];
    }
}

__global__ __launch_bounds__(kStatsBlock) void k_chain_predict(ChainPredictArgs a) {
    if (a.second && !(a.spec->spec_ok == kSpecRescaled && a.spec->verdict == 1u && !a.spec->pool_overflow && a.spec->retry_min == 1u &&
                      !a.spec->retried && !(a.spec->force & kSpecForceNoRetry))) return;
    __shared__ double est[2][256], fin[2][256];
    __shared__ uint8_t resc[2][256];
    __shared__ int s_ok[2], s_fwc, s_f;
    __shared__ unsigned s_mn[2];
    const int t = threadIdx.x, wb = t >> 6, ln = t & 63;
    if (t < 512) (&fin[0][0])[t] = 0.0;
    if (wb < 2) {
        const unsigned long long *sh = a.sample_hist + (size_t)wb * 256;
        unsigned long long v[4], others = 0, sv = 0;
#pragma unroll
        for (int k = 0; k < 4; ++k) {
            v[k] = 0ull;
            for (int r = 0; r < kSampleReplicas; ++r) v[k] += sh[(size_t)r * kMaxBands * 256 + ln * 4 + k];
            if (ln * 4 + k) others += v[k];
        }
        for (int r = 0; r < kSampleReplicas; ++r) sv += a.spec->sample_valid_rep[r * kMaxBands + wb];
#pragma unroll
        for (int m = 32; m > 0; m >>= 1) others += __shfl_xor(others, m, 64);
        const unsigned long long valid = a.state[wb].stats.valid_count;
        if (blockIdx.x == 0 && ln == 0) a.spec->sample_valid[wb] = sv;
        const unsigned long long invalid = a.total_px - valid;
        const bool empty_band = valid == 0ull;
        const bool consistent = sv >= others && sv > 0;
        const unsigned long long s0v = consistent ? sv - others : 0ull;
        const bool has255 = __builtin_amdgcn_ballot_w64(ln == 63 && v[3] != 0ull) != 0ull;
        const bool has0 = invalid > 0ull || s0v > 0ull;
        unsigned mn = 256u;
#pragma unroll
        for (int k = 3; k >= 0; --k) if (v[k] && (ln * 4 + k)) mn = (unsigned)(ln * 4 + k);
#pragma unroll
        for (int m = 32; m > 0; m >>= 1) mn = min(mn, (unsigned)__shfl_xor((int)mn, m, 64));
        if (has0 || empty_band || mn == 256u) mn = 0u;
        if ((a.force & kSpecForceMinMispredict) && mn && mn < 255u) mn += 1u;
        bool min_is_exact = false;
        if (a.second) {
            const unsigned tm = a.spec->true_min[wb];
            if (tm < mn) { mn = tm; min_is_exact = true; }
        }
        const double scale = consistent ? (double)valid / (double)sv : 0.0;
#pragma unroll
        for (int k = 0; k < 4; ++k) {
            const int l = ln * 4 + k;
            est[wb][l] = l ? scale * (double)v[k] : (double)invalid + scale * (double)s0v;
        }
        const float fmn = (float)mn, fmx = 255.0f;
        const float rs = fmx > fmn ? 255.0f / (fmx - fmn) : 1.0f;
#pragma unroll
        for (int k = 0; k < 4; ++k) {
            const unsigned x = ln * 4 + k;
            float val = roundf(((float)x - fmn) * rs);
            val = val < 0.0f ? 0.0f : (val > 255.0f ? 255.0f : val);
            resc[wb][x] = (uint8_t)val;
        }
        if (ln == 0) {
            s_mn[wb] = mn;
            s_ok[wb] = (empty_band || (consistent && has255 && (mn == 0u ? (has0 || min_is_exact) : a.allow_rescaled != 0u))) ? 1 : 0;
        }
    }
    __syncthreads();
    if (t < 512) {
        const int b = t >> 8, x = t & 255;
        if ((unsigned)x >= s_mn[b]) fin[b][resc[b][x]] = est[b][x];
    }
    __syncthreads();
    if (t == 0) {
        const uint32_t total = (uint32_t)(a.total_px + a.total_px);
        const double tc = round((double)total * 0.05);
        const uint32_t target = tc >= 4294967295.0 ? 4294967295u : (uint32_t)tc;
        double cum = 0.0, lt0 = 0.0, lt1 = 0.0;
        int f = kSpecFloorCap;
        for (int i = 0; i < kSpecFloorCap; ++i) {
            cum += fin[0][i] + fin[1][i];
            if (cum >= (double)target) { f = i; break; }
        }
        bool ok = s_ok[0] && s_ok[1];
        if (a.force & kSpecForceNoSpec) ok = false;
        if (a.force & kSpecForceMispredict) f = f < kSpecFloorCap ? f + 1 : kSpecFloorCap - 1;
        if (a.force & kSpecForceMispredict2) f = f + 2 <= kSpecFloorCap ? f + 2 : (f >= 2 ? f - 2 : f);
        for (int i = 0; i <= f && i < 64; ++i) { if (i < f) lt0 += fin[0][i] + fin[1][i]; lt1 += fin[0][i] + fin[1][i]; }
        s_fwc = f + 3 < 40 ? f + 3 : 40;
        s_f = f;
        if (blockIdx.x == 0) {
            ChainSpecState *sp = a.spec;
            sp->spec_ok = !ok ? 0u : (s_mn[0] | s_mn[1]) ? kSpecRescaled : kSpecIdentity;
            sp->verdict = 1u;
            sp->floor_pred = f;
            sp->done = 0u;
            sp->n_lt[0] = 0ull; sp->n_lt[1] = 0ull; sp->n_below_min = 0ull;
            sp->target = target;
            sp->min_pred[0] = s_mn[0]; sp->min_pred[1] = s_mn[1];
            sp->est_lt[0] = lt0; sp->est_lt[1] = lt1;
            sp->force = a.force;
            sp->pool_overflow = 0u;
            sp->next_item = 0u;
            sp->retry_floor = -1; sp->retry_armed = a.second ? 1u : 0u;
            if (!a.second) { sp->retried = 0u; sp->floor_first = f; sp->retry_min = 0u; }
            if (!a.second) { sp->true_min[0] = 256u; sp->true_min[1] = 256u; }
            for (int i = 0; i < 256; ++i) (&sp->below_hist[0][0])[i] = 0ull;
            if (a.floor_out) *a.floor_out = s_fwc;
        }
    }
    __syncthreads();
    if (blockIdx.x == 0 && wb < 2) {
        const unsigned mn = s_mn[wb];
#pragma unroll
        for (int q = 0; q < 2; ++q) {
            unsigned thr = 256u;
#pragma unroll
            for (int k = 3; k >= 0; --k) {
                const unsigned x = ln * 4 + k;
                if (x >= mn && (int)resc[wb][x] >= s_f + q) thr = x;
            }
#pragma unroll
            for (int m = 32; m > 0; m >>= 1) thr = min(thr, (unsigned)__shfl_xor((int)thr, m, 64));
            if (ln == 0) a.spec->thr[wb][q] = thr;
        }
    }
    if (blockIdx.x == 0) {
        if (t < 512) { a.exact_hist[t] = 0ull; if (a.resc_out) a.resc_out[t] = resc[t >> 8][t & 255]; }
        if (t < 2 && a.identity_out) a.identity_out[t] = s_mn[t] == 0u ? 1 : 0;
    }
    const int fwc = s_fwc;
    const uint8_t *lut_r = a.supp_rg + (size_t)fwc * 512, *lut_g = lut_r + 256;
    uint8_t *R2 = a.tables, *G2 = a.tables + 256, *B2 = a.tables + 512;
    if (blockIdx.x == 0 && t < 256) {
        const int r1 = resc[0][t], r2 = resc[1][t];
        const uint8_t r = r1 <= fwc ? 0 : lut_r[r1], g = r2 <= fwc ? 0 : lut_g[r2];
        R2[t] = r;
        G2[t] = g;
        if (a.blue_pq && a.blue_by_level) { a.blue_by_level[t] = a.blue_pq[r]; a.blue_by_level[256 + t] = a.blue_pq[256 + g]; }
    }
    for (int i = blockIdx.x * kStatsBlock + t; i < 65536; i += gridDim.x * kStatsBlock) {
        const int r1 = resc[0][i >> 8], r2 = resc[1][i & 255];
        B2[i] = (r1 <= fwc && r2 <= fwc) ? 0 : a.blue_pair_supp[((size_t)lut_r[r1] << 8) | lut_g[r2]];
    }
}

__global__ __launch_bounds__(kStatsBlock) void k_chain_repredict(ChainRepredictArgs a) {
    ChainSpecState *sp = a.spec;
    if (!sp->spec_ok || sp->verdict == 0u || sp->pool_overflow || sp->retry_floor < 0 || (sp->force & kSpecForceNoRetry)) {
        if (a.stripes && blockIdx.x == 0 && threadIdx.x == 0) {
            sp->saved_counts[0] = sp->n_lt[0]; sp->saved_counts[1] = sp->n_lt[1]; sp->saved_counts[2] = sp->n_below_min;
            sp->n_lt[0] = 0ull; sp->n_lt[1] = 0ull; sp->n_below_min = 0ull;
            for (int i = 0; i < 256; ++i) (&sp->below_hist[0][0])[i] = 0ull;
        }
        return;
    }
    __shared__ uint8_t resc[2][256];
    const int t = threadIdx.x, wb = t >> 6, ln = t & 63;
    if (t < 512) resc[t >> 8][t & 255] = a.resc_in[t];
    __syncthreads();
    const int f = sp->retry_floor, fwc = f + 3 < 40 ? f + 3 : 40;
    if (blockIdx.x == 0 && wb < 2) {
        const unsigned mn = sp->min_pred[wb];
#pragma unroll
        for (int q = 0; q < 2; ++q) {
            unsigned thr = 256u;
#pragma unroll
            for (int k = 3; k >= 0; --k) {
                const unsigned x = ln * 4 + k;
                if (x >= mn && (int)resc[wb][x] >= f + q) thr = x;
            }
#pragma unroll
            for (int m = 32; m > 0; m >>= 1) thr = min(thr, (unsigned)__shfl_xor((int)thr, m, 64));
            if (ln == 0) sp->thr[wb][q] = thr;
        }
    }
    const uint8_t *lut_r = a.supp_rg + (size_t)fwc * 512, *lut_g = lut_r + 256;
    uint8_t *R2 = a.tables, *G2 = a.tables + 256, *B2 = a.tables + 512;
    if (blockIdx.x == 0 && t < 256) {
        const int r1 = resc[0][t], r2 = resc[1][t];
        const uint8_t r = r1 <= fwc ? 0 : lut_r[r1], g = r2 <= fwc ? 0 : lut_g[r2];
        R2[t] = r;
        G2[t] = g;
        if (a.blue_pq && a.blue_by_level) { a.blue_by_level[t] = a.blue_pq[r]; a.blue_by_level[256 + t] = a.blue_pq[256 + g]; }
    }
    for (int i = blockIdx.x * kStatsBlock + t; i < 65536; i += gridDim.x * kStatsBlock) {
        const int r1 = resc[0][i >> 8], r2 = resc[1][i & 255];
        B2[i] = (r1 <= fwc && r2 <= fwc) ? 0 : a.blue_pair_supp[((size_t)lut_r[r1] << 8) | lut_g[r2]];
    }
    if (blockIdx.x == 0 && t == 0) {
        sp->floor_pred = f;
        sp->done = 0u;
        sp->n_lt[0] = 0ull; sp->n_lt[1] = 0ull; sp->n_below_min = 0ull;
        for (int i = 0; i < 256; ++i) (&sp->below_hist[0][0])[i] = 0ull;
        sp->next_item = 0u;
        sp->retry_armed = 1u;
        if (a.floor_out) *a.floor_out = fwc;
    }
}

__global__ __launch_bounds__(256) void k_chain_remap(const uint8_t *src, size_t src_pitch, uint8_t *dst,
                                                     size_t dst_pitch, uint32_t rows, uint32_t cols,
                                                     const uint8_t *__restrict__ map, const uint8_t *__restrict__ skip) {
    if (skip && *skip && src == dst) return;
    __shared__ uint8_t m[256];
    m[threadIdx.x] = map[threadIdx.x];
    __syncthreads();
    const uint64_t total = (uint64_t)rows * cols;
    for (uint64_t idx = (uint64_t)blockIdx.x * 256 + threadIdx.x; idx < total; idx += (uint64_t)gridDim.x * 256) {
        const uint32_t r = (uint32_t)(idx / cols), c = (uint32_t)(idx - (uint64_t)r * cols);
        dst[(size_t)r * dst_pitch + c] = m[src[(size_t)r * src_pitch + c]];
    }
}

constexpr int kGuardMinLevel = 27;
__global__ __launch_bounds__(256) void k_level_hist_guard(unsigned long long *level_hist, unsigned long long total_px,
                                                          uint32_t *flags) {
    __shared__ unsigned long long part[256];
    __shared__ int low_occupied;
    unsigned long long *lh = level_hist + (size_t)blockIdx.x * 256;
    const int t = threadIdx.x;
    const unsigned long long v = t ? lh[t] : 0ull;
    part[t] = v;
    if (t == 0) low_occupied = 0;
    __syncthreads();
    for (int s = 128; s > 0; s >>= 1) {
        if (t < s) part[t] += part[t + s];
        __syncthreads();
    }
    if (t >= 1 && t <= kGuardMinLevel && v) low_occupied = 1;
    if (t == 0 && total_px > part[0]) low_occupied = 1;
    __syncthreads();
    const bool recount = !low_occupied;
    if (t == 0) flags[blockIdx.x] = recount ? 1u : 0u;
    if (recount) lh[t] = 0ull;
}

__global__ __launch_bounds__(256) void k_level_hist_if_flagged(LevelRecountArgs a) {
    const int band = blockIdx.y;
    if (a.gate ? a.gate->verdict == 0 : !a.flags[band]) return;
    const uint8_t *__restrict__ in = a.levels[band];
    const size_t pitch = a.pitch;
    const uint32_t rows = a.rows, cols = a.cols;
    unsigned long long *__restrict__ hist = a.level_hist + (size_t)band * 256;
    __shared__ uint32_t h[4][256];
    for (int i = threadIdx.x; i < 1024; i += 256) (&h[0][0])[i] = 0;
    __syncthreads();
    uint32_t *hw = h[threadIdx.x >> 6];
    if (pitch % 16 == 0 && (reinterpret_cast<uintptr_t>(in) & 15) == 0) {
        const uint32_t vpr = (cols + 15) / 16;
        const uint64_t total = (uint64_t)rows * vpr;
        for (uint64_t idx = (uint64_t)blockIdx.x * 256 + threadIdx.x; idx < total; idx += (uint64_t)gridDim.x * 256) {
            const uint32_t r = (uint32_t)(idx / vpr), c = (uint32_t)(idx - (uint64_t)r * vpr) * 16;
            const uint4 q = *reinterpret_cast<const uint4 *>(in + (size_t)r * pitch + c);
            const uint32_t w[4] = {q.x, q.y, q.z, q.w};
            const uint32_t nvalid = min(16u, cols - c);
#pragma unroll
            for (int k = 0; k < 16; ++k)
                if ((uint32_t)k < nvalid) atomicAdd(&hw[(w[k >> 2] >> (8 * (k & 3))) & 0xFFu], 1u);
        }
    } else {
        const uint64_t total = (uint64_t)rows * cols;
        for (uint64_t idx = (uint64_t)blockIdx.x * 256 + threadIdx.x; idx < total; idx += (uint64_t)gridDim.x * 256) {
            const uint32_t r = (uint32_t)(idx / cols), c = (uint32_t)(idx - (uint64_t)r * cols);
            atomicAdd(&hw[in[(size_t)r * pitch + c]], 1u);
        }
    }
    __syncthreads();
    const uint32_t n = h[0][threadIdx.x] + h[1][threadIdx.x] + h[2][threadIdx.x] + h[3][threadIdx.x];
    if (n && threadIdx.x) atomicAdd(&hist[threadIdx.x], (unsigned long long)n);
}

}

hipError_t launch_chain_stats(const ChainStatsArgs &a, int nbands, hipStream_t s) {
    hipLaunchKernelGGL(k_chain_stats_a, dim3(nbands, kStatsParts), dim3(kPartBlock), 0, s, a);
    hipLaunchKernelGGL(k_chain_stats_b, dim3(nbands, kStatsParts), dim3(kPartBlock), 0, s, a);
    hipLaunchKernelGGL(k_chain_stats_c, dim3(nbands, kStatsParts), dim3(kPartBlock), 0, s, a);
    return hipGetLastError();
}
hipError_t launch_chain_cdfs(const unsigned long long *tile_bins, double *cdfs, uint32_t rows, uint32_t cols, int nbands,
                             hipStream_t s) {
    hipLaunchKernelGGL(k_chain_cdfs, dim3(kTiles * kTiles, nbands), dim3(256), 0, s, tile_bins, cdfs, rows, cols);
    return hipGetLastError();
}
hipError_t launch_chain_finish(const ChainFinishArgs &a, hipStream_t s) {
    hipLaunchKernelGGL(k_chain_finish, dim3((a.nbands == 2 && a.tables) || a.levels_mode ? 64 : 1), dim3(kStatsBlock), 0, s, a);
    return hipGetLastError();
}
hipError_t launch_chain_repredict(const ChainRepredictArgs &a, hipStream_t s) {
    hipLaunchKernelGGL(k_chain_repredict, dim3(64), dim3(kStatsBlock), 0, s, a);
    return hipGetLastError();
}
hipError_t launch_chain_predict(const ChainPredictArgs &a, hipStream_t s) {
    hipLaunchKernelGGL(k_chain_predict, dim3(64), dim3(kStatsBlock), 0, s, a);
    return hipGetLastError();
}
hipError_t launch_chain_remap(const uint8_t *src, size_t src_pitch, uint8_t *dst, size_t dst_pitch, uint32_t rows,
                              uint32_t cols, const uint8_t *d_map, const uint8_t *d_skip_flag, hipStream_t s) {
    if (!rows || !cols) return hipSuccess;
    const uint64_t want = ((uint64_t)rows * cols + 255) / 256;
    hipLaunchKernelGGL(k_chain_remap, dim3((unsigned)(want < 2048 ? want : 2048)), dim3(256), 0, s, src, src_pitch, dst,
                       dst_pitch, rows, cols, d_map, d_skip_flag);
    return hipGetLastError();
}

}

namespace sarpro {
hipError_t launch_level_hist_guard(unsigned long long *level_hist, unsigned long long total_px, int nbands, uint32_t *d_flags,
                                   hipStream_t s) {
    hipLaunchKernelGGL(k_level_hist_guard, dim3(nbands), dim3(256), 0, s, level_hist, total_px, d_flags);
    return hipGetLastError();
}
hipError_t launch_level_hist_if_flagged(const LevelRecountArgs &a, int nbands, hipStream_t s) {
    if (!a.rows || !a.cols) return hipSuccess;
    hipLaunchKernelGGL(k_level_hist_if_flagged, dim3(1024, nbands), dim3(256), 0, s, a);
    return hipGetLastError();
}
}
```

### sarpro_amd/csrc/context.h

```cpp
#pragma once
#include <hip/hip_runtime.h>

#include <atomic>
#include <condition_variable>
#include <functional>
#include <map>
#include <mutex>
#include <string>
#include <thread>
#include <tuple>
#include <vector>

#include "kernels.h"
#include "piece_kernels.h"

namespace sarpro {

struct DevBuf {
    void *p = nullptr;
    size_t cap = 0;
    DevBuf() = default;
    DevBuf(const DevBuf &) = delete;
    DevBuf &operator=(const DevBuf &) = delete;
    ~DevBuf() { release(); }
// ... 82 lines not shown
            std::this_thread::yield();
#endif
        }
        return flag.load(std::memory_order_acquire);
    }
    void run() {
        for (;;) {
            if (!spin_until(pending, 4000)) {
                std::unique_lock<std::mutex> lk(m);
                cv.wait(lk, [&] { return pending.load(std::memory_order_acquire) || quit; });
                if (quit) return;
            }
            const int r = job();
            {
                std::lock_guard<std::mutex> lk(m);
                rc = r;
                pending.store(false, std::memory_order_release);
                finished.store(true, std::memory_order_release);
            }
            cv.notify_all();
        }
    }
    void submit(std::function<int()> j) {
        {
            std::lock_guard<std::mutex> lk(m);
            job = std::move(j);
            finished.store(false, std::memory_order_release);
            pending.store(true, std::memory_order_release);
        }
        cv.notify_all();
    }
    int wait() {
        if (!spin_until(finished, 20000)) {
            std::unique_lock<std::mutex> lk(m);
            cv.wait(lk, [&] { return finished.load(std::memory_order_acquire); });
        }
        std::lock_guard<std::mutex> lk(m);
        return rc;
    }
    void stop() {
        { std::lock_guard<std::mutex> lk(m); quit = true; }
        cv.notify_all();
        if (th.joinable()) th.join();
    }
};
}

#define SARPRO_ATTR_LIST(X) \
    X(NO_CHAIN) X(NO_FUSED) X(NO_SPEC) X(NO_PIECE_HIST) X(NO_LINEAR_HIST) X(NO_SWEEP_ORDER) X(FULL_LEVEL_HIST) X(NO_SAMPLED_HIST) \
    X(SAMPLED_HIST_MIN_PX) X(SAMPLE_STRIDE) X(SEPARATE_CDFS) X(NO_FUSED_RGB) X(SPEC_FORCE) X(FORCE_UNCERTAIN) \
    X(STRIP_ALIGN) X(PIECE_ALIGN) X(CHUNK_ROWS) X(RGB_ITEM_ROWS) X(SAMPLE_ITEM_ROWS) \
    X(NO_MAILBOX) X(NO_STEP_ESTIMATE) X(F32_ZONES) X(F32_ZONES_DEBUG) X(F32_DIRECT) X(F32_DIRECT_QCAP) X(F32_LEVEL_GENERAL) \
    X(F32_LEVEL_TABLE) X(F32_LEVEL_QCAP) X(F32_HOST_CDFS) X(F32_NO_VEC8) X(NO_BAND_TWIN) X(RESIZE_GENERIC) X(NO_RESIZE_LUT) \
    X(NO_U16_CF) X(U16_ITEM_ROWS) X(PIPE_LANES) X(PIPE_ORDER) X(RGB_GRID) X(PIECE_GRID) X(COMM_RECORD) X(COMM_REPLAY) X(NO_SPEC_RESCALE) X(RGB_TAIL_ROWS) X(RGB_TAIL_ITEM_ROWS)
namespace sarpro {
enum Attr : int {
#define X(n) A_##n,
    SARPRO_ATTR_LIST(X)
#undef X
    A_COUNT
};
struct AttrSet {
    long long v[A_COUNT] = {};
    bool set[A_COUNT] = {};
    bool on(Attr a) const { return set[a] && v[a] != 0; }
    long long val(Attr a, long long dflt) const { return set[a] ? v[a] : dflt; }
    bool is_set(Attr a) const { return set[a]; }
};
const char *attr_name(int a);
int attr_index(const char *name);
void attrs_from_environment(AttrSet *out);
}

struct sarpro_hip_ctx {
    int device = 0;
    unsigned flags = 0;
    sarpro::AttrSet attrs;
    hipStream_t stream = nullptr;
    std::string err;

    sarpro::DevBuf tile_hist[sarpro::kMaxBands];
    size_t tile_hist_clean_bytes = 0;
    const void *tile_hist_clean_ptr = nullptr;
    sarpro::DevBuf ghist;
    sarpro::DevBuf tile_bins;
    sarpro::DevBuf cdfs;
    sarpro::DevBuf luts;
    sarpro::DevBuf level_hist;
    sarpro::DevBuf spec_dump;
    sarpro::DevBuf hist_flags;
    sarpro::DevBuf tables;
    sarpro::DevBuf spec_state;
    int cu_count = 0;
    sarpro::DevBuf levels[sarpro::kMaxBands];
    sarpro::DevBuf stage_in[sarpro::kMaxBands];
    sarpro::DevBuf stage_out[3];
    sarpro::DevBuf qtab;
    sarpro::DevBuf f32ws;
    sarpro::DevBuf f32zone;
    uint32_t resize_key[2][6] = {{0, 0, 0, 0, 0, 0}, {0, 0, 0, 0, 0, 0}};
    sarpro::DevBuf resize_tmp, resize_coef[2], resized[2];
    sarpro::DevBuf resize_halo, resize_geom;
    sarpro::DevBuf jpeg_coef, jpeg_seg, jpeg_tables, jpeg_band[2], jpeg_rgb, jpeg_file;
    sarpro::PinnedBuf jpeg_host;
    sarpro::DevBuf read_tab, read_src[2], read_band[2];
    sarpro::PinnedBuf read_host;
    size_t read_key[4] = {0, 0, 0, 0};
// ... 52 lines not shown
```

### sarpro_amd/csrc/host_logic.cpp

```cpp
#include "host_logic.h"

#include <algorithm>
#include <cfloat>
#include <cmath>
#include <cstring>
#include <mutex>
#include <thread>
#include <vector>

namespace sarpro {

static inline uint64_t as_u64(double x) {
    if (!(x == x) || x <= 0.0) return 0;
    if (x >= 18446744073709551615.0) return UINT64_MAX;
    return (uint64_t)x;
}
static inline int64_t as_i64(double x) {
    if (!(x == x)) return 0;
    if (x <= -9223372036854775808.0) return INT64_MIN;
    if (x >= 9223372036854775807.0) return INT64_MAX;
    return (int64_t)x;
}
static inline uint32_t as_u32(double x) {
    if (!(x == x) || x <= 0.0) return 0;
// ... 392 lines not shown
    }
    blue_lut(lut_r, lut_g, true, lut_b);
}

int synrgb_floor_from_hist(const uint64_t *hist, uint64_t n_per_band) {
    uint32_t total = (uint32_t)(n_per_band + n_per_band);
    uint32_t target = as_u32(std::round((double)total * 0.05));
    uint32_t cumulative = 0;
    size_t floor_value = 0;
    for (size_t i = 0; i < 256; ++i) {
        uint64_t hi = std::min<uint64_t>(hist[i], UINT32_MAX);
        uint64_t c = (uint64_t)cumulative + hi;
        cumulative = c > UINT32_MAX ? UINT32_MAX : (uint32_t)c;
        if (cumulative >= target) { floor_value = i; break; }
    }
    return (int)std::min<size_t>(floor_value + 3, 40);
}

void synrgb_luts_suppressed(int fwc, uint8_t *luts) {
    uint8_t *lut_r = luts, *lut_g = luts + 256, *lut_b = luts + 512;
    float floor_f = (float)fwc;
    float denom = std::fmax(255.0f - floor_f, 1.0f);
    for (unsigned v = 0; v < 256; ++v) {
        if ((int)v <= fwc) { lut_r[v] = 0; lut_g[v] = 0; continue; }
        float shifted = ((float)v - floor_f) / denom;
        lut_r[v] = f32_as_u8(clampf(std::round(std::pow(shifted, 1.15f) * 255.0f), 0.0f, 255.0f));
        lut_g[v] = f32_as_u8(clampf(std::round(std::pow(shifted, 1.10f) * 255.0f), 0.0f, 255.0f));
    }
    blue_lut(lut_r, lut_g, false, lut_b);
}

const uint8_t *synrgb_blue_pair_supp() { return blue_pair_table(false); }

const float *synrgb_blue_factors_supp() {
    static float tab[512];
    static bool ok = false;
    static std::once_flag once;
    std::call_once(once, [] {
        for (unsigned i = 0; i < 256; ++i) {
            tab[i] = (float)(45.9 * std::pow((double)i + 8.0, 0.1));
            tab[256 + i] = (float)std::pow((double)i + 8.0, -0.1);
        }
        const uint8_t *pair = blue_pair_table(false);
        ok = true;
        for (unsigned r = 0; r < 256 && ok; ++r)
            for (unsigned g = 0; g < 256; ++g) {
                const float prod = tab[r] * tab[256 + g];
                if ((unsigned)std::nearbyintf(prod) != pair[(r << 8) | g]) { ok = false; break; }
            }
    });
    return ok ? tab : nullptr;
}
const uint8_t *synrgb_blue_pair_default() { return blue_pair_table(true); }

const double *gamma_level_thresholds_u8() {
    static double tab[3][256];
    static std::once_flag once;
    std::call_once(once, [] {
        const double gammas[3] = {0.8, 0.9, 1.1};
        for (int g = 0; g < 3; ++g) {
            auto level = [&](double x) { return (int)as_u16(clampd(std::pow(x, gammas[g]) * 255.0, 0.0, 255.0)); };
            tab[g][0] = 0.0;
            uint64_t lo_bits = 0;
            for (int k = 1; k < 256; ++k) {
                uint64_t lo = lo_bits, hi;
                const double one = 1.0;
                std::memcpy(&hi, &one, 8);
                while (hi - lo > 1) {
                    const uint64_t mid = lo + (hi - lo) / 2;
                    double xm;
                    std::memcpy(&xm, &mid, 8);
                    if (level(xm) >= k) hi = mid; else lo = mid;
                }
                std::memcpy(&tab[g][k], &hi, 8);
                lo_bits = lo;
            }
        }
    });
    return &tab[0][0];
}

const uint8_t *synrgb_supp_rg_tables() {
    static uint8_t tab[41][512];
    static std::once_flag once;
    std::call_once(once, [] {
        std::vector<uint8_t> luts(66048);
        for (int fwc = 0; fwc <= 40; ++fwc) {
            synrgb_luts_suppressed(fwc, luts.data());
            std::memcpy(tab[fwc], luts.data(), 512);
        }
    });
    return &tab[0][0];
}

void fold_compose_tables(const uint8_t *luts, int fwc, const uint8_t *resc1, const uint8_t *resc2,
                         uint8_t *tables) {
    const uint8_t *lut_r = luts, *lut_g = luts + 256, *lut_b = luts + 512;
    uint8_t *R2 = tables, *G2 = tables + 256, *B2 = tables + 512;
    for (unsigned v = 0; v < 256; ++v) {
        R2[v] = lut_r[resc1[v]];
        G2[v] = lut_g[resc2[v]];
    }
    for (unsigned v1 = 0; v1 < 256; ++v1) {
        unsigned r1 = resc1[v1];
        for (unsigned v2 = 0; v2 < 256; ++v2) {
            unsigned r2 = resc2[v2];
// ... 28 lines not shown

int sarpro_hip_host_stats_from_dn_hist(const uint64_t dn_hist[65536], sarpro_hip_stats *out) {
    if (!dn_hist || !out) return SARPRO_HIP_ERR_INVALID_ARG;
    return stats_from_dn_hist(dn_hist, out);
}

int sarpro_hip_host_window(sarpro_hip_stats *stats, int strategy, int tamed_synrgb) {
    if (!stats || tamed_synrgb < 0 || tamed_synrgb > 2) return SARPRO_HIP_ERR_INVALID_ARG;
    return select_window(stats, strategy, tamed_synrgb);
}

int sarpro_hip_host_level_lut_u16(const sarpro_hip_stats *stats, int bit_depth, int tamed_synrgb,
                                  uint16_t lut_out[65536]) {
    if (!stats || !lut_out || (bit_depth != SARPRO_BITDEPTH_U8 && bit_depth != SARPRO_BITDEPTH_U16))
        return SARPRO_HIP_ERR_INVALID_ARG;
    DnLut lut;
    build_level_lut_u16(*stats, bit_depth, tamed_synrgb, &lut);
    std::memcpy(lut_out, lut.full.data(), 65536 * sizeof(uint16_t));
    return SARPRO_HIP_OK;
}

int sarpro_hip_host_clahe_bin_lut_u16(const sarpro_hip_stats *stats, uint8_t lut_out[65536]) {
    if (!stats || !lut_out) return SARPRO_HIP_ERR_INVALID_ARG;
    DnLut lut;
    build_clahe_bin_lut_u16(*stats, &lut);
    for (int i = 0; i < 65536; ++i) lut_out[i] = (uint8_t)lut.full[i];
    return SARPRO_HIP_OK;
}

int sarpro_hip_host_clahe_cdfs(const uint64_t *tile_hists, size_t rows, size_t cols, double *cdfs_out) {
    if (!tile_hists || !cdfs_out) return SARPRO_HIP_ERR_INVALID_ARG;
    return clahe_cdfs(tile_hists, rows, cols, cdfs_out);
}

int sarpro_hip_host_u8_rescale_lut(unsigned min_level, unsigned max_level, uint8_t lut_out[256]) {
    if (!lut_out || min_level > 65535 || max_level > 65535) return SARPRO_HIP_ERR_INVALID_ARG;
    u8_rescale_lut(min_level, max_level, lut_out);
    return SARPRO_HIP_OK;
}

int sarpro_hip_host_synrgb_luts(int strategy, const uint64_t combined_hist[256], uint64_t n_per_band,
                                uint8_t *luts_out, int *floor_out) {
    if (!luts_out || strategy < 0 || strategy > SARPRO_STRATEGY_DEFAULT) return SARPRO_HIP_ERR_INVALID_ARG;
    if (strategy == SARPRO_STRATEGY_TAMED || strategy == SARPRO_STRATEGY_CLAHE) {
        if (!combined_hist) return SARPRO_HIP_ERR_INVALID_ARG;
        int fwc = synrgb_floor_from_hist(combined_hist, n_per_band);
        synrgb_luts_suppressed(fwc, luts_out);
        if (floor_out) *floor_out = fwc;
    } else {
        synrgb_luts_default(luts_out);
        if (floor_out) *floor_out = -1;
    }
    return SARPRO_HIP_OK;
}

int sarpro_hip_host_clahe_shape_ok(size_t rows, size_t cols) { return clahe_shape_ok(rows, cols) ? 1 : 0; }
int sarpro_hip_host_clahe_saturated_levels(size_t rows, size_t cols, uint8_t *col_class, uint8_t *row_bits) {
    if (!clahe_shape_ok(rows, cols) || !col_class || !row_bits) return SARPRO_HIP_ERR_INVALID_ARG;
    ClaheGeometry g;
    build_clahe_geometry(rows, cols, &g);
    std::vector<uint8_t> cc, rb;
    if (!clahe_saturated_levels(g, &cc, &rb)) return SARPRO_HIP_ERR_UNSUPPORTED_SHAPE;
    std::memcpy(col_class, cc.data(), cols);
    std::memcpy(row_bits, rb.data(), rows);
    return SARPRO_HIP_OK;
}

int sarpro_hip_host_stripe_plan(size_t rows, int nranks, size_t *row0_out, size_t *nrows_out) {
    if (!row0_out || !nrows_out) return SARPRO_HIP_ERR_INVALID_ARG;
    return stripe_plan(rows, nranks, row0_out, nrows_out);
}

}

namespace sarpro {

double db_of_f32(float v) { return 10.0 * std::log10(std::fmax((double)v, 1e-10)); }

static inline float bits_to_f32(uint32_t b) { float f; std::memcpy(&f, &b, 4); return f; }
static inline uint32_t f32_to_bits(float f) { uint32_t b; std::memcpy(&b, &f, 4); return b; }
static const uint32_t kMaxFiniteBits = 0x7F7FFFFFu;

template <typename P>
static uint32_t find_first_bits(P pred, uint32_t lo, uint32_t hi, uint32_t guess) {
    if (!pred(hi)) return hi + 1;
    if (pred(lo)) return lo;
    uint32_t g = std::min(std::max(guess, lo + 1), hi);
    if (g != hi) {
        if (pred(g)) {
            hi = g;
            uint32_t step = 1;
            while (hi - lo > step && pred(hi - step)) { hi -= step; step *= 2; }
            if (hi - lo > step) lo = hi - step;
        } else {
            lo = g;
            uint32_t step = 1;
            while (hi - lo > step && !pred(lo + step)) { lo += step; step *= 2; }
            if (hi - lo > step) hi = lo + step;
        }
    }
    while (hi - lo > 1) {
        uint32_t mid = lo + (hi - lo) / 2;
        if (pred(mid)) hi = mid; else lo = mid;
    }
    return hi;
}
// ... 213 lines not shown
```

### sarpro_amd/csrc/host_logic.h

```cpp
#pragma once
#include <cstddef>
#include <cstdint>
#include <vector>

#include "../../include/sarpro_hip.h"

namespace sarpro {

constexpr int kTiles = 8;
constexpr int kClaheBins = 256;
constexpr double kClipLimit = 2.0;
constexpr int kStatBins = 4096;

const double *db_table_u16();

enum TamedSynrgb { kNotTamedSynrgb = 0, kTamedCopol = 1, kTamedCrosspol = 2 };

int stats_from_dn_hist(const uint64_t *dn_hist, sarpro_hip_stats *out);
int stats_from_bins4096(uint64_t count, double min_db, double max_db, double mean, double std_db,
                        const uint64_t *hist4096, sarpro_hip_stats *out);
int select_window(sarpro_hip_stats *s, int strategy, int tamed_synrgb);

uint16_t level_of_db(double db, double low_clip, double high_clip, double gamma, double max_val);
uint8_t clahe_bin_of_db(double db, double low_clip, double high_clip);

struct DnLut {
    std::vector<uint16_t> full;
    uint32_t win_lo = 1, win_hi = 1;
};
void build_level_lut_u16(const sarpro_hip_stats &s, int bit_depth, int tamed_synrgb, DnLut *out);
void build_clahe_bin_lut_u16(const sarpro_hip_stats &s, DnLut *out);

struct RowWeight { double d, omd; int32_t t0, t1; };
struct ClaheGeometry {
    size_t rows = 0, cols = 0, tile_h = 0, tile_w = 0;
    std::vector<RowWeight> row_w, col_w;
    std::vector<size_t> row_cell_start, col_cell_start;
};
bool clahe_shape_ok(size_t rows, size_t cols);
bool clahe_saturated_levels(const ClaheGeometry &g, std::vector<uint8_t> *col_class, std::vector<uint8_t> *row_bits);
void build_clahe_geometry(size_t rows, size_t cols, ClaheGeometry *g);
void clahe_tile_cdf(uint64_t *hist , size_t tile_rows, size_t tile_cols,
                    double *cdf );
int clahe_cdfs(const uint64_t *tile_hists, size_t rows, size_t cols, double *cdfs_out);

void u8_rescale_lut(unsigned min_level, unsigned max_level, uint8_t *lut256);

void synrgb_luts_default(uint8_t *luts);
int synrgb_floor_from_hist(const uint64_t *combined_hist256, uint64_t n_per_band);
void synrgb_luts_suppressed(int floor_with_cushion, uint8_t *luts);

void fold_compose_tables(const uint8_t *luts, int floor_with_cushion ,
                         const uint8_t *resc1, const uint8_t *resc2, uint8_t *tables);

int stripe_plan(size_t rows, int nranks, size_t *row0, size_t *nrows);

const uint8_t *synrgb_supp_rg_tables();
const uint8_t *synrgb_blue_pair_supp();
const float *synrgb_blue_factors_supp();
const uint8_t *synrgb_blue_pair_default();
const double *gamma_level_thresholds_u8();

}

namespace sarpro {
int bin4096_of_f32(float x, double min_db, double max_db);
void build_bin4096_thresholds_range(double min_db, double max_db, int k0, int k1, float *thr_out);
double percentile_from_bin(double min_db, double max_db, int bin, uint64_t target, uint64_t cum_below, uint64_t in_bin);
uint64_t percentile_target(uint64_t n, double p);
double db_of_f32(float v);
float valid_threshold_f32();
void build_bin4096_thresholds(double min_db, double max_db, float *thr4096);
void build_level_thresholds(const sarpro_hip_stats &s, int nlevels , float *thr);
float level_threshold_one(const sarpro_hip_stats &s, int nlevels, int k);
void build_clahe_bin_thresholds(const sarpro_hip_stats &s, float *thr256);
}

namespace sarpro {
struct ResizeCoeffs {
    uint32_t in_size = 0, out_size = 0, window = 0;
    int precision = 0;
    std::vector<uint32_t> start, size;
    std::vector<int32_t> k;
};
void build_resize_coeffs(uint32_t in_size, uint32_t out_size, int elem_size , ResizeCoeffs *out);
void resize_bounds(uint32_t in_size, uint32_t out_size, uint32_t *window, std::vector<uint32_t> *start, std::vector<uint32_t> *size);
void resize_dimensions(size_t original_cols, size_t original_rows, size_t target_size, size_t *new_cols, size_t *new_rows);
}
```

### sarpro_amd/csrc/kernels.h

```cpp
#pragma once
#include <hip/hip_runtime.h>

#include <cstddef>
#include <cstdint>

#include "host_logic.h"

namespace sarpro {

constexpr int kMaxBands = 2;

struct Rect {
    int32_t r0, r1;
    int32_t c0, c1;
    int32_t cstart;
    int32_t id[4];
    int32_t pad[3];
};
static_assert(sizeof(Rect) == 48, "Rect layout");

struct DnHistArgs {
    const uint16_t *in[kMaxBands];
    uint32_t *tile_hist[kMaxBands];
    size_t pitch;
// ... 46 lines not shown
    struct ChainSpecState *spec;
    int speculative;
};

constexpr unsigned long long kSampleWeightOne = 4096;
constexpr int kSampleReplicas = 16;
constexpr int kSpecFloorCap = 37;
struct ChainSpecState {
    uint32_t spec_ok;
    uint32_t verdict;
    int32_t floor_pred;
    uint32_t done;
    unsigned long long n_lt[2];
    unsigned long long n_below_min;
    unsigned long long below_hist[2][128];
    unsigned long long target;
    uint32_t min_pred[2];
    uint32_t thr[2][2];
    unsigned long long sample_valid[2];
    unsigned long long sample_valid_rep[kSampleReplicas * 2];
    double est_lt[2];
    uint32_t force;
    uint32_t pool_overflow;
    uint32_t next_item;
    int32_t retry_floor;
    uint32_t retry_armed;
    uint32_t retried;
    int32_t floor_first;
    unsigned long long saved_counts[3];
    uint32_t true_min[2];
    uint32_t retry_min;
};
constexpr uint32_t kSpecIdentity = 1u, kSpecRescaled = 2u;
constexpr size_t kSpecCountWords = 3 + 2 * 128;
constexpr uint32_t kSpecForceMispredict = 1u;
constexpr uint32_t kSpecForceNoSpec = 2u;
constexpr uint32_t kSpecForceMinMispredict = 4u;
constexpr uint32_t kSpecForceNoRetry = 8u;
constexpr uint32_t kSpecForceMispredict2 = 16u;

struct ClaheRgbArgs {
    const uint16_t *in[kMaxBands];
    size_t in_pitch;
    uint8_t *rgb;
    size_t rgb_pitch_px;
    const Rect *rects;
    int nrects;
    const double *cdfs[kMaxBands];
    const uint8_t *binlut[kMaxBands];
    const RowWeight *row_w, *col_w;
    int32_t row_off;
    const struct ChainBandState *dev_state;
    struct ChainSpecState *spec;
    const uint8_t *tables;
    const uint8_t *sat_col, *sat_row;
    const float *blue_by_level;
    uint32_t no_verdict;
    uint32_t sat_cols;
    uint32_t sat_ok;
    uint32_t retry;
};
bool clahe_rgb_fused_supported(const ClaheRgbArgs &a);
hipError_t launch_clahe_rgb_fused(const ClaheRgbArgs &a, int grid , hipStream_t s);
hipError_t launch_clahe_rgb_fused_retry(const ClaheRgbArgs &a, int grid, hipStream_t s);
hipError_t launch_spec_verdict(struct ChainSpecState *spec, const struct ChainBandState *state, hipStream_t s, int second = 0);

constexpr size_t kSpecDumpBytes = 256 * 1024;
hipError_t launch_dn_hist_u16(const DnHistArgs &a, int nrects, int nbands, bool vec, hipStream_t s);
hipError_t launch_dn_hist_u16_interior(const DnHistArgs &a, int nrects, int nbands, hipStream_t s);
hipError_t launch_dn_hist_u16_linear(const DnHistArgs &a, uint32_t rows, uint32_t cols, int nbands, hipStream_t s);
struct SumTileHistArgs {
    uint32_t *tile_hist[kMaxBands];
    unsigned long long *out[kMaxBands];
    uint32_t clear;
};
hipError_t launch_sum_tile_hists(const SumTileHistArgs &a, int ntiles, int nbands, hipStream_t s);
struct TileBinHistArgs {
    uint32_t *tile_hist[kMaxBands];
    const uint8_t *binlut[kMaxBands];
    unsigned long long *out[kMaxBands];
    uint32_t clear;
    double *cdfs_out[kMaxBands];
    uint32_t rows, cols;
};
hipError_t launch_tile_bin_hist(const TileBinHistArgs &a, int ntiles, int nbands, hipStream_t s);
hipError_t launch_clahe_apply_u16(const ClaheApplyArgs &a, int nrects, int nbands, bool vec, bool out16,
                                  hipStream_t s);
bool clahe_apply_spec_ok(const ClaheApplyArgs &a, int nbands);
hipError_t launch_clahe_apply_u8_spec(ClaheApplyArgs a, int nrects, int nbands, hipStream_t s);
constexpr uint32_t kChainLutEntries = 8192;
hipError_t launch_lut_apply_u16(const LutApplyArgs &a, bool vec, bool out16, hipStream_t s);
hipError_t launch_compose_u8(const ComposeArgs &a, int vec, hipStream_t s);
struct LutComposeArgs {
    const uint16_t *in[kMaxBands];
    uint8_t *rgb;
    size_t in_pitch, rgb_pitch_px;
    uint32_t rows, cols;
    const uint8_t *lut[kMaxBands];
    uint32_t win_hi[kMaxBands];
    const uint8_t *tables;
    const struct ChainBandState *dev_state;
    uint32_t lut_cap;
};
bool lut_compose_fits(const LutComposeArgs &a);
hipError_t launch_lut_compose_u16(const LutComposeArgs &a, hipStream_t s);
hipError_t launch_polop_f32(int op, const float *a, const float *b, size_t n, float *out, hipStream_t s);
hipError_t launch_synth_scene_u16(uint64_t seed, int band, const uint16_t *d_q ,
                                  size_t rows_total, size_t cols, size_t row0, size_t rows_local,
                                  uint16_t *d_out, size_t pitch, uint32_t flags, hipStream_t s);
// ... 13 lines not shown
```

### sarpro_amd/csrc/kernels.hip

```cpp
#include "kernels.h"
#include "chain_kernels.h"
#include "device_cdf.h"

#include <algorithm>
#include <mutex>
#include <set>
#include <type_traits>
#include <utility>

namespace sarpro {

namespace {

constexpr int kWave = 64;
constexpr int kBlock = 256;
constexpr int kWavesPerBlock = kBlock / kWave;

template <int VEC> struct U16Vec;
template <> struct U16Vec<8> {
    uint4 v;
    __device__ static U16Vec load(const uint16_t *p) { U16Vec r; r.v = *reinterpret_cast<const uint4 *>(p); return r; }
    __device__ static U16Vec load_stream(const uint16_t *p) {
        typedef uint32_t v4u __attribute__((ext_vector_type(4)));
        const v4u t = __builtin_nontemporal_load(reinterpret_cast<const v4u *>(p));
// ... 536 lines not shown
                    v4u pk;
                    pk.x = pw[0]; pk.y = pw[1]; pk.z = pw[2]; pk.w = pw[3];
                    const uint32_t soff = on ? (uint32_t)(wave + kCfWaves * (k + i)) * out_row_bytes : 0u;
                    __builtin_amdgcn_raw_buffer_store_b128(pk, rs_out, on ? voff_st : 0xFFFFFFFFu, soff, 2 );
                    asm volatile("s_nop 1" : : "v"(pk) : "memory");
                    uint32_t e16 = 0u;
                    if (edge_l >= 0 || edge_r >= 0) {
                        const int el = max(edge_l, 0), er = max(edge_r, 0);
                        uint32_t lid;
                        asm volatile("v_mbcnt_lo_u32_b32 %0, -1, 0\n\tv_mbcnt_hi_u32_b32 %0, -1, %0" : "=v"(lid));
                        const bool lid8 = lid < 8u;
                        const uint32_t j = lid & 7u;
                        uint32_t xs[4];
#pragma unroll
                        for (int q = 0; q < 4; ++q) {
                            const uint32_t xl = (uint32_t)__builtin_amdgcn_readlane((int)pw[q], el), xr = (uint32_t)__builtin_amdgcn_readlane((int)pw[q], er);
                            xs[q] = lid8 ? xl : xr;
                        }
                        const uint32_t w2 = (j & 4u) ? ((j & 2u) ? xs[3] : xs[2]) : ((j & 2u) ? xs[1] : xs[0]);
                        e16 = (j & 1u) ? w2 >> 16 : w2 & 0xFFFFu;
                    }
                    __builtin_amdgcn_raw_buffer_store_b16((uint16_t)e16, rs_out, on ? voff_edge : 0xFFFFFFFFu, soff, 0);
                }
#pragma unroll
                for (int i = 0; i < NR; ++i) cur[i] = nxt[i];
            }
        };
        if (lut_lds) {
            if (rc.pad[0] & 1) item_rows(std::true_type{}, std::true_type{});
            else item_rows(std::false_type{}, std::true_type{});
        } else {
            if (rc.pad[0] & 1) item_rows(std::true_type{}, std::false_type{});
            else item_rows(std::false_type{}, std::false_type{});
        }
    }
#ifdef SARPRO_RGB_WG_TIMES
    __syncthreads();
    if (threadIdx.x == 0) { unsigned long long *o = g_rgb_wg_times[blockIdx.x & 1023]; o[1] = wall_clock64(); for (int k = 0; k < 5; ++k) o[2 + k] = cf_n[k]; }
#endif
}

constexpr float kSpecDeltaEdgeY = 3.0e-4f, kSpecDeltaEdgeX = 2.6e-4f;
constexpr float kSpecDeltaEdge = 6.2e-4f, kSpecDeltaInner = 1.6e-4f;
__device__ __forceinline__ float spec_delta(int pad0) {
    return !(pad0 & 1) ? kSpecDeltaInner : (pad0 & 6) == 2 ? kSpecDeltaEdgeY : (pad0 & 6) == 4 ? kSpecDeltaEdgeX : kSpecDeltaEdge;
}
#ifdef SARPRO_SPEC_MEASURE
__device__ uint32_t g_spec_max_err[4];
__device__ __forceinline__ int spec_class(int pad0) { return !(pad0 & 1) ? 0 : (pad0 & 6) == 2 ? 1 : (pad0 & 6) == 4 ? 2 : 3; }
#endif
constexpr uint32_t kPartialHistLevels = 64;
typedef float v2f __attribute__((ext_vector_type(2)));
typedef float v4f __attribute__((ext_vector_type(4)));
constexpr uint32_t kSpecLutMaxEntries = 16384;

#ifndef SARPRO_CDF_COPIES
#define SARPRO_CDF_COPIES 1
#endif
constexpr uint32_t kCdfCopies = SARPRO_CDF_COPIES;
constexpr uint32_t kCdfPerRow = 16 / kCdfCopies;
constexpr uint32_t kCdf32Bytes = ((257 + kCdfPerRow - 1) / kCdfPerRow) * 256;
__host__ __device__ constexpr uint32_t cdf32_offset(uint32_t entry) {
    return (entry / kCdfPerRow) * 256u + (entry % kCdfPerRow) * kCdfCopies * 16u;
}
__host__ __device__ constexpr uint32_t cdf32_entry(uint32_t offset) {
    return (offset / 256u) * kCdfPerRow + (offset % 256u) / (kCdfCopies * 16u);
}

struct SpecLds {
    static constexpr uint32_t cdf64 = 0;
    static constexpr uint32_t cdf32 = 257 * 32 + 224;
    static constexpr uint32_t colw = cdf32 + kCdf32Bytes;
    static constexpr uint32_t hist = colw + 512 * 8;
    static constexpr uint32_t lut = hist + (256 + 64 + 4) * 4;
};


__device__ __forceinline__ float to_sgpr(float x) {
    return __builtin_bit_cast(float, __builtin_amdgcn_readfirstlane(__builtin_bit_cast(int, x)));
}
__device__ __forceinline__ uint32_t lshl_or(uint32_t hi, uint32_t sh, uint32_t lo) {
    uint32_t d;
    asm("v_lshl_or_b32 %0, %1, %2, %3" : "=v"(d) : "v"(hi), "n"(sh), "v"(lo));
    return d;
}
#define pack4(b0, b1, b2, b3) lshl_or(lshl_or((b3), 8, (b2)), 16, lshl_or((b1), 8, (b0)))
__device__ __forceinline__ uint32_t to_sgpr_u32(uint32_t x) { return (uint32_t)__builtin_amdgcn_readfirstlane((int)x); }
__device__ __forceinline__ double to_sgpr(double x) {
    const unsigned long long u = __builtin_bit_cast(unsigned long long, x);
    const uint32_t lo = (uint32_t)__builtin_amdgcn_readfirstlane((int)(uint32_t)u);
    const uint32_t hi = (uint32_t)__builtin_amdgcn_readfirstlane((int)(uint32_t)(u >> 32));
    return __builtin_bit_cast(double, ((unsigned long long)hi << 32) | lo);
}

#define SPEC_LOAD(p) U16Vec<VEC>::load(p)
template <bool LUT_LDS, int HIST>
__device__ __forceinline__ void clahe_spec_rows(const ClaheApplyArgs &a, const Rect &rc, int band, unsigned char *lds,
                                                uint32_t win_hi) {
    constexpr int VEC = 8;
    const uint16_t *__restrict__ in = a.in[band];
    const uint8_t *__restrict__ glut = a.binlut[band];
    const RowWeight *__restrict__ row_w = a.row_w + a.row_off;
    const bool count_levels = a.level_hist[band] != nullptr;
    const int col = rc.cstart + lane_id() * VEC;
    const bool full = col >= rc.c0 && col + VEC <= rc.c1;
    uint32_t keep[2] = {0u, 0u};
#pragma unroll
    for (int j = 0; j < VEC; ++j)
        if (col + j >= rc.c0 && col + j < rc.c1) keep[j >> 2] |= 0xFFu << (8 * (j & 3));
    uint8_t *dump = a.dump + ((((size_t)blockIdx.y * gridDim.x + blockIdx.x) * kWavesPerBlock + wave_id()) % (kSpecDumpBytes / 512)) * 512 +
                    lane_id() * 8;

    float dxf[VEC];
#pragma unroll
    for (int j = 0; j < VEC; ++j) dxf[j] = (float)*reinterpret_cast<const double *>(lds + SpecLds::colw + (lane_id() * VEC + j) * 8);
    const uint32_t copy_off = ((uint32_t)lane_id() & (kCdfCopies - 1)) * 16u;
    const float near_delta = spec_delta(rc.pad[0]);
    const float bias = -0.5f - near_delta, two_delta = 2.0f * near_delta;
    const uint32_t win_hi2 = win_hi | (win_hi << 16);
    constexpr bool PARTIAL_HIST = HIST != 0;
    uint32_t lane_max = 0u, lane_high = 0u;
    uint32_t lane_valid = 0u;
#ifdef SARPRO_SPEC_MEASURE
    float spec_err = 0.0f;
#endif

    auto process_row = [&](int r, const U16Vec<VEC> &v, const double dy_v, const bool sampled) {
        if (HIST >= 2 && count_levels && sampled) {
            const uint32_t w[4] = {v.v.x, v.v.y, v.v.z, v.v.w};
#pragma unroll
            for (int k = 0; k < 4; ++k) {
                const uint32_t nz = (((w[k] & 0x7FFF7FFFu) + 0x7FFF7FFFu) | w[k]) & 0x80008000u;
                const uint32_t kb = keep[k >> 1] >> (16 * (k & 1));
                lane_valid += (uint32_t)__builtin_popcount(nz & (((kb & 0x80u) << 8) | ((kb & 0x8000u) << 16)));
            }
        }
        const double dy = to_sgpr(dy_v), omdy = to_sgpr(1.0 - dy);
        const float wy1 = to_sgpr((float)omdy * 255.0f), wy2 = to_sgpr((float)dy * 255.0f);
        uint32_t off[VEC];
// ... 398 lines not shown
                const uint8_t *p1 = a.b1 + (size_t)r * a.in_pitch + col, *p2 = a.b2 + (size_t)r * a.in_pitch + col;
                uint8_t *po = a.rgb + ((size_t)r * a.rgb_pitch_px + col) * 3;
                for (uint32_t j = 0; col + j < a.cols; ++j) {
                    const uint32_t v1 = p1[j], v2 = p2[j];
                    po[3 * j + 0] = R2[v1]; po[3 * j + 1] = G2[v2]; po[3 * j + 2] = B2[(v1 << 8) | v2];
                    if (SPEC) {
                        n_px += 2u;
                        n_ge[0] += (v1 >= fpred) + (v2 >= fpred);
                        n_ge[1] += (v1 >= fpred + 1u) + (v2 >= fpred + 1u);
                    }
                }
            }
        }
    } else {
        for (uint64_t idx = (uint64_t)blockIdx.x * kComposeBlock + threadIdx.x; idx < total; idx += (uint64_t)gridDim.x * kComposeBlock) {
            const uint32_t r = (uint32_t)(idx / vpr);
            const uint32_t col = (uint32_t)(idx - (uint64_t)r * vpr) * VEC;
            const uint8_t *p1 = a.b1 + (size_t)r * a.in_pitch + col, *p2 = a.b2 + (size_t)r * a.in_pitch + col;
            uint8_t *po = a.rgb + ((size_t)r * a.rgb_pitch_px + col) * 3;
            for (int j = 0; j < VEC && col + j < a.cols; ++j) {
                const uint32_t v1 = p1[j], v2 = p2[j];
                po[3 * j + 0] = R2[v1]; po[3 * j + 1] = G2[v2]; po[3 * j + 2] = B2[(v1 << 8) | v2];
            }
        }
    }
    if (SPEC) {
        n_ge[0] += fpred ? (n_vec_px + sad[0] - sad[1]) >> 1 : n_vec_px;
        n_ge[1] += (n_vec_px + sad[1] - sad[2]) >> 1;
        n_px += n_vec_px;
        uint32_t lt0 = n_px - n_ge[0], lt1 = n_px - n_ge[1];
#pragma unroll
        for (int m = 32; m > 0; m >>= 1) { lt0 += __shfl_xor(lt0, m, 64); lt1 += __shfl_xor(lt1, m, 64); }
        uint32_t *s_lt = reinterpret_cast<uint32_t *>(lds_raw);
        __syncthreads();
        if (threadIdx.x == 0) { s_lt[0] = 0u; s_lt[1] = 0u; }
        __syncthreads();
        if (lane == 0) { atomicAdd(&s_lt[0], lt0); atomicAdd(&s_lt[1], lt1); }
        __syncthreads();
        if (threadIdx.x == 0) {
            ChainSpecState *sp = a.spec;
            atomicAdd(&sp->n_lt[0], (unsigned long long)s_lt[0]);
            atomicAdd(&sp->n_lt[1], (unsigned long long)s_lt[1]);
            __threadfence();
            if (atomicAdd(&sp->done, 1u) == gridDim.x - 1u) {
                __threadfence();
                const unsigned long long c0 = atomicAdd(&sp->n_lt[0], 0ull), c1 = atomicAdd(&sp->n_lt[1], 0ull), target = sp->target;
                const bool ok = sp->floor_pred >= kSpecFloorCap ? c0 < target : (c0 < target && target <= c1);
                sp->verdict = ok ? 0u : 1u;
            }
        }
    }
}

#ifndef SARPRO_RGB_B2_STRIDE
#define SARPRO_RGB_B2_STRIDE 260
#endif
constexpr uint32_t kRgbB2Stride = SARPRO_RGB_B2_STRIDE;
static_assert(kRgbB2Stride == 256 || kRgbB2Stride == 260, "blue table rows: 256 (as in global memory) or 260 bytes");
#ifndef SARPRO_RGB_BLOCK
#define SARPRO_RGB_BLOCK 1024
#endif
#ifndef SARPRO_RGB_POOL
#define SARPRO_RGB_POOL (SARPRO_RGB_B2_STRIDE == 256 ? 3072 : 3008)
#endif
constexpr int kRgbBlock = SARPRO_RGB_BLOCK, kRgbWaves = kRgbBlock / kWave;
constexpr uint32_t kRgbPoolEntries = SARPRO_RGB_POOL;
constexpr uint32_t kRgbTableBytes = 512 + 256 * kRgbB2Stride;
struct RgbLds {
    static constexpr uint32_t tables = 0;
    static constexpr uint32_t stage = kRgbTableBytes;
    static constexpr uint32_t cdf64 = stage + kRgbWaves * 1536;
    static constexpr uint32_t colw = cdf64 + 2 * 257 * 32;
    static constexpr uint32_t binof = colw + 512 * 8;
    static constexpr uint32_t pool = binof + kRgbPoolEntries;
    static constexpr uint32_t misc = pool + kRgbPoolEntries * 16;
    static constexpr uint32_t total = misc + 128;
};
constexpr uint32_t kWideEnt = RgbLds::misc - 2u * 257u * 16u;
constexpr uint32_t kWideBytes = kWideEnt - RgbLds::binof;
static_assert(kWideEnt % 16 == 0, "alignment");
static_assert(RgbLds::total <= 160 * 1024, "fused pass: LDS budget");
static_assert(RgbLds::stage % 16 == 0 && RgbLds::pool % 16 == 0 && RgbLds::cdf64 % 16 == 0, "alignment");

__device__ __forceinline__ int spec_retry_floor(int f, unsigned long long c0, unsigned long long target) {
    if (c0 >= target) return f > 0 ? f - 1 : -1;
    return f < kSpecFloorCap ? f + 1 : -1;
}
template <bool GENERAL>
__device__ __forceinline__ void clahe_rgb_fused_body(const ClaheRgbArgs &a) {
    extern __shared__ __align__(16) unsigned char lds[];
    constexpr int VEC = 8;
    ChainSpecState *sp = a.spec;
#ifdef SARPRO_RGB_WG_TIMES
    if (threadIdx.x == 0) g_rgb_wg_times[blockIdx.x & 1023][0] = wall_clock64();
    unsigned long long wg_t_wait = 0ull, wg_t_pro = 0ull, wg_t_rows = 0ull, wg_items = 0ull, wg_ta = 0ull, wg_tb = 0ull, wg_tc = 0ull;
#endif
    const uint32_t win_hi[2] = {a.dev_state[0].win_hi, a.dev_state[1].win_hi};
    const uint64_t nwin = (uint64_t)win_hi[0] + win_hi[1] + 2u;
    const bool wide = nwin > kRgbPoolEntries;
    if (wide && nwin > kWideBytes) {
        if (blockIdx.x == 0 && threadIdx.x == 0) sp->pool_overflow = 1u;
        return;
    }
    const uint32_t kb[2] = {0u, win_hi[0] + 1u};
    const int lane = lane_id(), wave = wave_id();
    {
        for (int b = 0; b < 2; ++b)
            for (uint32_t i = threadIdx.x; i <= win_hi[b]; i += kRgbBlock) lds[RgbLds::binof + kb[b] + i] = a.binlut[b][i];
    }
    {
        const uint32_t *src = reinterpret_cast<const uint32_t *>(a.tables);
        for (int i = threadIdx.x; i < 512 / 4; i += kRgbBlock) LDS_AT(uint32_t, RgbLds::tables + 4 * i) = src[i];
        for (int i = threadIdx.x; i < 65536 / 4; i += kRgbBlock)
            LDS_AT(uint32_t, RgbLds::tables + 512 + (uint32_t)(i >> 6) * kRgbB2Stride + (uint32_t)(i & 63) * 4u) = src[128 + i];
    }
    const uint32_t fpred = (uint32_t)sp->floor_pred;
    const uint32_t t4[3] = {(fpred ? fpred - 1u : 0u) * 0x01010101u, fpred * 0x01010101u, (fpred + 1u) * 0x01010101u};
    uint32_t sad[3] = {0u, 0u, 0u}, n_all = 0u, n_kept = 0u;
    uint32_t tg[2][5] = {{0u, 0u, 0u, 0u, 0u}, {0u, 0u, 0u, 0u, 0u}}, sadg[2][5] = {{0u, 0u, 0u, 0u, 0u}, {0u, 0u, 0u, 0u, 0u}};
    uint32_t min_track = 0u;
    if (GENERAL) {
#pragma unroll
        for (int b = 0; b < 2; ++b) {
            if (sp->min_pred[b] >= 1u && sp->min_pred[b] <= 127u) min_track |= 1u << b;
        }
        min_track = to_sgpr_u32(min_track);
    }
    if (GENERAL) {
#pragma unroll
        for (int b = 0; b < 2; ++b) {
            const uint32_t T0 = sp->thr[b][0], mn = sp->min_pred[b];
            tg[b][0] = min(T0 ? T0 - 1u : 0u, 255u) * 0x01010101u; tg[b][1] = min(T0, 255u) * 0x01010101u; tg[b][2] = min(T0 + 1u, 255u) * 0x01010101u;
            tg[b][3] = (mn ? mn - 1u : 0u) * 0x01010101u; tg[b][4] = mn * 0x01010101u;
        }
    }
    const RowWeight *__restrict__ row_w = a.row_w + a.row_off;
    const uint32_t stage_w = RgbLds::stage + (uint32_t)wave * 1536u;

    uint32_t *const s_next = reinterpret_cast<uint32_t *>(lds + RgbLds::misc) + 8;
    uint32_t *const s_rect = reinterpret_cast<uint32_t *>(lds + RgbLds::misc) + 16;
    uint32_t rect_word = 0u;
    {
        uint32_t first = 0u;
        if (threadIdx.x == 0) { first = atomicAdd(&sp->next_item, 1u); s_next[0] = first; }
        if (wave == 0) {
            const int it0 = (int)to_sgpr_u32(first);
            if (lane < 12 && it0 < a.nrects) s_rect[lane] = reinterpret_cast<const uint32_t *>(a.rects + it0)[lane];
        }
    }
    for (;;) {
        uint32_t *const s_bsat = reinterpret_cast<uint32_t *>(lds + RgbLds::misc) + 4;
        if (wide && threadIdx.x < 2) s_bsat[threadIdx.x] = 256u;
#ifdef SARPRO_RGB_WG_TIMES
        if (threadIdx.x == 0) { wg_ta = wall_clock64(); if (wg_items) wg_t_rows += wg_ta - wg_tc; }
#endif
        __syncthreads();
#ifdef SARPRO_RGB_WG_TIMES
        if (threadIdx.x == 0) { wg_tb = wall_clock64(); wg_t_wait += wg_tb - wg_ta; }
#endif
        if (threadIdx.x == 0) s_next[1] = 2u * kRgbWaves;
        const int item = (int)to_sgpr_u32(s_next[0]);
        if (item >= a.nrects) break;
        uint32_t next_item = 0u;
        if (threadIdx.x == 0) next_item = atomicAdd(&sp->next_item, 1u);
        Rect rc;
        rc.r0 = (int)to_sgpr_u32(s_rect[0]); rc.r1 = (int)to_sgpr_u32(s_rect[1]); rc.c0 = (int)to_sgpr_u32(s_rect[2]); rc.c1 = (int)to_sgpr_u32(s_rect[3]);
        rc.cstart = (int)to_sgpr_u32(s_rect[4]);
#pragma unroll
        for (int k = 0; k < 4; ++k) rc.id[k] = (int)to_sgpr_u32(s_rect[5 + k]);
        rc.pad[0] = (int)to_sgpr_u32(s_rect[9]); rc.pad[1] = 0; rc.pad[2] = 0;
        {
        for (int t = threadIdx.x; t < 2 * 257; t += kRgbBlock) {
            const int b = t / 257, bin = t - b * 257;
            double c[4] = {0.0, 0.0, 0.0, 0.0};
            if (bin < 256) {
#pragma unroll
                for (int k = 0; k < 4; ++k) c[k] = a.cdfs[b][(size_t)rc.id[k] * 256 + bin];
            }
            *reinterpret_cast<double4 *>(lds + RgbLds::cdf64 + (b * 257 + bin) * 32) = make_double4(c[0], c[1], c[2], c[3]);
            const bool saturated = bin < 256 && c[0] == 1.0 && c[1] == 1.0 && c[2] == 1.0 && c[3] == 1.0 && (!(rc.pad[0] & 1) || a.sat_ok);
            const bool zero = c[0] == 0.0 && c[1] == 0.0 && c[2] == 0.0 && c[3] == 0.0;
            const float kz = 0.5f / 255.0f;
            const float c00 = (float)c[0], c01 = (float)c[1], c10 = (float)c[2], c11 = (float)c[3];
            const float4 e32 = saturated ? make_float4(1.001f, 1.001f, 0.0f, 0.0f)
                               : zero    ? make_float4(kz, kz, 0.0f, 0.0f)
                                         : make_float4(c00, c10, c01 - c00, c11 - c10);
            *reinterpret_cast<float4 *>(lds + RgbLds::stage + (b * 257 + bin) * 16) = e32;
            if (wide && saturated && (rc.pad[0] & 1)) atomicMin(&s_bsat[b], (uint32_t)bin);
        }
        for (int i = threadIdx.x; i < 512; i += kRgbBlock) {
// ... 201 lines not shown
                    __builtin_amdgcn_raw_buffer_store_b128(z, rgb_rsrc, 0xFFFFFFF0u, 0, 2);
                    __builtin_amdgcn_raw_buffer_store_b8((uint8_t)0, rgb_rsrc, 0xFFFFFFFFu, 0, 0);
                }
                for (;;) {
                    const int rn = rc.r0 + min(kn, nrows - 1);
                    uint32_t grab = 0u;
                    if (lane == 0) grab = atomicAdd(&s_next[1], 1u);
                    const uint4 n0 = *reinterpret_cast<const uint4 *>(p0 + (size_t)rn * a.in_pitch), n1 = *reinterpret_cast<const uint4 *>(p1 + (size_t)rn * a.in_pitch);
                    const double dyn = row_w[rn].d;
                    const uint32_t srn = (EDGE && a.sat_ok) ? (uint32_t)a.sat_row[rn] : 7u;
                    uint32_t satN[2] = {0u, 0u};
                    if (EDGE) {
                        const uint32_t rb = to_sgpr_u32(srv);
#pragma unroll
                        for (int k = 0; k < 3; ++k)
                            if (!((rb >> k) & 1u)) { satN[0] |= satM[k][0]; satN[1] |= satM[k][1]; }
                    }
                    const double dy = to_sgpr(dyv), omdy = to_sgpr(1.0 - dy);
                    const float wy1 = to_sgpr((float)omdy * 255.0f), wy2 = to_sgpr((float)dy * 255.0f);
                    uint32_t l1[2], l2[2];
                    band_levels(0, c0, dy, omdy, wy1, wy2, satN, l1);
                    band_levels(1, c1, dy, omdy, wy1, wy2, satN, l2);
                    if (GENERAL) {
#pragma unroll
                        for (int k = 0; k < 5; ++k) {
                            sadg[0][k] = __builtin_amdgcn_sad_u8(l1[1], tg[0][k], __builtin_amdgcn_sad_u8(l1[0], tg[0][k], sadg[0][k]));
                            sadg[1][k] = __builtin_amdgcn_sad_u8(l2[1], tg[1][k], __builtin_amdgcn_sad_u8(l2[0], tg[1][k], sadg[1][k]));
                        }
                        if (min_track) {
                            const uint32_t lv[2][2] = {{l1[0], l1[1]}, {l2[0], l2[1]}};
#pragma unroll
                            for (int b = 0; b < 2; ++b) {
                                uint32_t below[2];
#pragma unroll
                                for (int g = 0; g < 2; ++g)
                                    below[g] = ~(((lv[b][g] & 0x7F7F7F7Fu) | 0x80808080u) - tg[b][4]) & ~lv[b][g] & keep[g] & 0x80808080u;
                                if (((min_track >> b) & 1u) && (below[0] | below[1])) {
                                    uint32_t lowest = 256u;
#pragma unroll
                                    for (int j = 0; j < VEC; ++j)
                                        if ((below[j >> 2] >> (8 * (j & 3))) & 0x80u) lowest = min(lowest, (lv[b][j >> 2] >> (8 * (j & 3))) & 0xFFu);
                                    atomicMin(&sp->true_min[b], lowest);
                                    atomicAdd(&sp->below_hist[b][lowest & 127u], 1ull);
                                }
                            }
                        }
                    } else {
#pragma unroll
                        for (int k = 0; k < 3; ++k)
                            sad[k] = __builtin_amdgcn_sad_u8(l2[1], t4[k], __builtin_amdgcn_sad_u8(l2[0], t4[k], __builtin_amdgcn_sad_u8(l1[1], t4[k], __builtin_amdgcn_sad_u8(l1[0], t4[k], sad[k]))));
                    }
                    n_all += 16u; n_kept += 2u * nkeep;
                    uint32_t o[6];
#pragma unroll
                    for (int g = 0; g < 2; ++g) {
                        uint32_t px[4][3];
#pragma unroll
                        for (int j = 0; j < 4; ++j) {
                            const uint32_t v1 = j == 0 ? (l1[g] & 0xFFu) : j == 3 ? (l1[g] >> 24) : __builtin_amdgcn_ubfe(l1[g], 8 * j, 8);
                            const uint32_t v2 = j == 0 ? (l2[g] & 0xFFu) : j == 3 ? (l2[g] >> 24) : __builtin_amdgcn_ubfe(l2[g], 8 * j, 8);
                            uint32_t pair;
                            if (kRgbB2Stride == 256) pair = __builtin_amdgcn_perm(l1[g], l2[g], to_sgpr_u32(0x0c0c0400u + 0x0101u * (uint32_t)j));
                            else asm("v_mad_u32_u24 %0, %1, %2, %3" : "=v"(pair) : "v"(v1), "s"(kRgbB2Stride), "v"(v2));
                            px[j][0] = LDS_AT(uint8_t, RgbLds::tables + v1);
                            px[j][1] = LDS_AT(uint8_t, RgbLds::tables + 256 + v2);
                            px[j][2] = LDS_AT(uint8_t, RgbLds::tables + 512 + pair);
                        }
                        o[3 * g + 0] = pack4(px[0][0], px[0][1], px[0][2], px[1][0]);
                        o[3 * g + 1] = pack4(px[1][1], px[1][2], px[2][0], px[2][1]);
                        o[3 * g + 2] = pack4(px[2][2], px[3][0], px[3][1], px[3][2]);
                    }
                    *reinterpret_cast<uint2 *>(lds + stage_w + lane * 24) = make_uint2(o[0], o[1]);
                    *reinterpret_cast<uint2 *>(lds + stage_w + lane * 24 + 8) = make_uint2(o[2], o[3]);
                    *reinterpret_cast<uint2 *>(lds + stage_w + lane * 24 + 16) = make_uint2(o[4], o[5]);
                    {
                        typedef uint32_t v4u __attribute__((ext_vector_type(4)));
                        const uint32_t soff = (uint32_t)(r - rc.r0) * row_bytes;
                        const v4u d1 = LDS_AT(v4u, stage_w + lane * 16), d2 = LDS_AT(v4u, stage_w + 1024 + lane * 16);
                        const uint32_t e8 = LDS_AT(uint8_t, edge_lds);
                        __builtin_amdgcn_raw_buffer_store_b128(d1, rgb_rsrc, voff1, soff, 2 );
                        asm volatile("s_nop 1" : : "v"(d1) : "memory");
                        __builtin_amdgcn_raw_buffer_store_b128(d2, rgb_rsrc, voff2, soff, 2);
                        asm volatile("s_nop 1" : : "v"(d2) : "memory");
                        __builtin_amdgcn_raw_buffer_store_b8((uint8_t)e8, rgb_rsrc, edge_voff, soff, 0);
                    }
                    c0 = n0; c1 = n1; dyv = dyn; srv = srn;
                    if (kn >= nrows) break;
                    r = rc.r0 + kn;
                    kn = (int)to_sgpr_u32(grab);
                }
            }
        }
        };
        if (!wide) {
            if (rc.pad[0] & 1) item_rows(std::true_type{}, std::false_type{});
            else item_rows(std::false_type{}, std::false_type{});
        } else {
            if (rc.pad[0] & 1) item_rows(std::true_type{}, std::true_type{});
            else item_rows(std::false_type{}, std::true_type{});
        }
        if (wave == 0 && lane < 12) s_rect[lane] = rect_word;
    }
#ifdef SARPRO_RGB_WG_TIMES
    __syncthreads();
    if (threadIdx.x == 0) {
        unsigned long long *o = g_rgb_wg_times[blockIdx.x & 1023];
        o[1] = wall_clock64(); o[2] = wg_t_wait; o[3] = wg_t_pro; o[4] = wg_t_rows; o[5] = wg_items;
    }
#endif
    uint32_t lt0, lt1, below = 0u;
    if (GENERAL) {
        lt0 = 0u; lt1 = 0u;
        const uint32_t na = n_all >> 1, nk = n_kept >> 1;
#pragma unroll
        for (int b = 0; b < 2; ++b) {
            const uint32_t T0 = sp->thr[b][0], T1 = sp->thr[b][1], mn = sp->min_pred[b];
            const uint32_t ge_t0 = T0 == 0u ? nk : T0 > 255u ? 0u : (na + sadg[b][0] - sadg[b][1]) >> 1;
            const uint32_t ge_t0p = T0 + 1u > 255u ? 0u : (na + sadg[b][1] - sadg[b][2]) >> 1;
            const uint32_t ge_t1 = T1 == T0 ? ge_t0 : ge_t0p;
            const uint32_t ge_mn = mn == 0u ? nk : (na + sadg[b][3] - sadg[b][4]) >> 1;
            lt0 += nk - ge_t0; lt1 += nk - ge_t1; below += nk - ge_mn;
        }
    } else {
// ... 513 lines not shown
```

Baseline: 431,700.

## Replace 64K blue pair LUT with factored per-level entries in synRGB kernel

The synthetic RGB kernel no longer looks up blue from a 256x256 pair table in LDS. It reads two 8-byte per-level entries (a float factor plus packed R/G byte and a water flag), multiplies the factors, and packs the result with cvt_pk_u8_f32. The entries are replicated 16 times per band across LDS so each lane uses its own copy, which avoids bank conflicts. The predict and repredict kernels then skip building the 64K pair table and launch one block instead of 64. This trades byte lookups for float math and depends on the blue table factoring exactly into per-level products. When blue factors are unavailable, speculation is disabled.

```diff
diff --git a/include/sarpro_hip.h b/include/sarpro_hip.h
--- a/include/sarpro_hip.h
+++ b/include/sarpro_hip.h
@@ -381,6 +381,9 @@
 int sarpro_hip_host_u8_rescale_lut(unsigned min_level, unsigned max_level, uint8_t lut_out[256]);
 int sarpro_hip_host_synrgb_luts(int strategy, const uint64_t combined_hist[256], uint64_t n_per_band,
                                 uint8_t *luts_out, int *floor_out);
+#define SARPRO_HIP_LEVEL_ENTRY_WATER 2147483648u
+int sarpro_hip_host_synrgb_level_entries(int floor_with_cushion, const uint8_t resc1[256], const uint8_t resc2[256],
+                                         uint32_t entries_out[1024]);
 int sarpro_hip_host_clahe_shape_ok(size_t rows, size_t cols);
 int sarpro_hip_host_clahe_saturated_levels(size_t rows, size_t cols, uint8_t *col_class, uint8_t *row_bits);
 int sarpro_hip_host_stripe_plan(size_t rows, int nranks, size_t *row0_out, size_t *nrows_out);
diff --git a/rust/sarpro-hip-sys/src/lib.rs b/rust/sarpro-hip-sys/src/lib.rs
--- a/rust/sarpro-hip-sys/src/lib.rs
+++ b/rust/sarpro-hip-sys/src/lib.rs
@@ -22,6 +22,7 @@
 pub const SARPRO_HIP_ROUTE_POOL_OVERFLOW: c_int = 3;
 pub const SARPRO_HIP_ROUTE_RETRIED: c_int = 4;
 pub const SARPRO_HIP_ERR_UNSUPPORTED: c_int = -10;
+pub const SARPRO_HIP_LEVEL_ENTRY_WATER: c_uint = 2147483648;
 pub const SARPRO_HIP_SYNTH_NO_WEDGE: c_uint = 1;
 pub const SARPRO_HIP_SYNTH_NO_BRIGHT: c_uint = 2;
 pub const SARPRO_HIP_SYNTH_NO_BAND2: c_uint = 4;
@@ -309,6 +310,7 @@
     pub fn sarpro_hip_host_clahe_cdfs(tile_hists: *const u64, rows: usize, cols: usize, cdfs_out: *mut f64) -> c_int;
     pub fn sarpro_hip_host_u8_rescale_lut(min_level: c_uint, max_level: c_uint, lut_out: *mut u8) -> c_int;
     pub fn sarpro_hip_host_synrgb_luts(strategy: c_int, combined_hist: *const u64, n_per_band: u64, luts_out: *mut u8, floor_out: *mut c_int) -> c_int;
+    pub fn sarpro_hip_host_synrgb_level_entries(floor_with_cushion: c_int, resc1: *const u8, resc2: *const u8, entries_out: *mut u32) -> c_int;
     pub fn sarpro_hip_host_clahe_shape_ok(rows: usize, cols: usize) -> c_int;
     pub fn sarpro_hip_host_clahe_saturated_levels(rows: usize, cols: usize, col_class: *mut u8, row_bits: *mut u8) -> c_int;
     pub fn sarpro_hip_host_stripe_plan(rows: usize, nranks: c_int, row0_out: *mut usize, nrows_out: *mut usize) -> c_int;
diff --git a/sarpro_amd/__init__.py b/sarpro_amd/__init__.py
--- a/sarpro_amd/__init__.py
+++ b/sarpro_amd/__init__.py
@@ -1,7 +1,7 @@
 from .types import AutoscaleStrategy, BitDepth, PolarizationOperation, SyntheticRgbMode
 from .api import (LocalGroup, Context, SarproHipError, Stripe, StripeF32, host_f32_merge_partials, comm_unique_id, host_clahe_bin_lut_u16,
                   host_clahe_cdfs, host_clahe_saturated_levels, host_clahe_shape_ok, host_level_lut_u16, host_stats_from_dn_hist,
-                  host_stripe_plan, host_stripe_resized_rows, host_synrgb_luts, host_u8_rescale_lut, host_window,
+                  host_stripe_plan, host_stripe_resized_rows, host_synrgb_luts, host_synrgb_level_entries, LEVEL_ENTRY_WATER, host_u8_rescale_lut, host_window,
                   host_f32_valid_threshold, host_f32_bin4096_thresholds, host_f32_level_thresholds,
                   host_f32_clahe_bin_thresholds, host_stats_from_bins4096, resize_output_dims, host_jpeg_header, jpeg_bound,
                   read_output_dims, host_read_average_axis,
diff --git a/sarpro_amd/_lib.py b/sarpro_amd/_lib.py
--- a/sarpro_amd/_lib.py
+++ b/sarpro_amd/_lib.py
@@ -92,7 +92,7 @@
     "sarpro_hip_comm_destroy",
     "sarpro_hip_host_stats_from_dn_hist", "sarpro_hip_host_window", "sarpro_hip_host_level_lut_u16",
     "sarpro_hip_host_clahe_bin_lut_u16", "sarpro_hip_host_clahe_cdfs", "sarpro_hip_host_u8_rescale_lut",
-    "sarpro_hip_host_synrgb_luts", "sarpro_hip_host_clahe_shape_ok", "sarpro_hip_host_parse_cpulist", "sarpro_hip_host_stripe_plan",
+    "sarpro_hip_host_synrgb_luts", "sarpro_hip_host_synrgb_level_entries", "sarpro_hip_host_clahe_shape_ok", "sarpro_hip_host_parse_cpulist", "sarpro_hip_host_stripe_plan",
     "sarpro_hip_host_stats_from_bins4096", "sarpro_hip_host_f32_valid_threshold", "sarpro_hip_host_f32_bin4096_thresholds",
     "sarpro_hip_host_f32_level_thresholds", "sarpro_hip_host_f32_clahe_bin_thresholds",
     "sarpro_hip_resize_output_dims", "sarpro_hip_resize_image_data", "sarpro_hip_resize_image_data_dev",
@@ -222,6 +222,7 @@
 _proto("sarpro_hip_host_clahe_cdfs", _i, _vp, _sz, _sz, _vp)
 _proto("sarpro_hip_host_u8_rescale_lut", _i, C.c_uint, C.c_uint, _vp)
 _proto("sarpro_hip_host_synrgb_luts", _i, _i, _vp, _u64, _vp, C.POINTER(_i))
+_proto("sarpro_hip_host_synrgb_level_entries", _i, _i, _vp, _vp, _vp)
 _proto("sarpro_hip_host_clahe_shape_ok", _i, _sz, _sz)
 _proto("sarpro_hip_host_clahe_saturated_levels", _i, _sz, _sz, _vp, _vp)
 _proto("sarpro_hip_host_stripe_plan", _i, _sz, _i, _vp, _vp)
diff --git a/sarpro_amd/api.py b/sarpro_amd/api.py
--- a/sarpro_amd/api.py
+++ b/sarpro_amd/api.py
@@ -808,6 +808,20 @@
     if rc:
         raise SarproHipError(rc, "host_synrgb_luts")
     return luts[:256].copy(), luts[256:512].copy(), luts[512:].reshape(256, 256).copy(), fl.value
+
+
+LEVEL_ENTRY_WATER = 0x80000000
+
+
+def host_synrgb_level_entries(floor_with_cushion: int, resc1: np.ndarray, resc2: np.ndarray) -> np.ndarray:
+    r1, r2 = np.ascontiguousarray(resc1, np.uint8), np.ascontiguousarray(resc2, np.uint8)
+    if r1.size != 256 or r2.size != 256:
+        raise ValueError("the rescale maps have 256 entries each")
+    out = np.empty((2, 256, 2), np.uint32)
+    rc = lib.sarpro_hip_host_synrgb_level_entries(int(floor_with_cushion), _vp(r1), _vp(r2), _vp(out))
+    if rc:
+        raise SarproHipError(rc, "host_synrgb_level_entries")
+    return out
 
 
 def host_clahe_saturated_levels(rows: int, cols: int):
diff --git a/sarpro_amd/csrc/api_u16_chain.cpp b/sarpro_amd/csrc/api_u16_chain.cpp
--- a/sarpro_amd/csrc/api_u16_chain.cpp
+++ b/sarpro_amd/csrc/api_u16_chain.cpp
@@ -20,7 +20,7 @@
 constexpr size_t kChainOffDb = 0, kChainOffSupp = 65536 * 8, kChainOffBlue = kChainOffSupp + 21504;
 constexpr size_t kChainOffBlueDef = kChainOffBlue + 65536, kChainOffDefRg = kChainOffBlueDef + 65536;
 constexpr size_t kChainOffGamma = kChainOffDefRg + 512, kChainOffBluePQ = kChainOffGamma + 3 * 256 * 8, kChainConstBytes = kChainOffBluePQ + 512 * 4;
-constexpr size_t kTablesOffPQ = 66048 + 512, kTablesBytes = kTablesOffPQ + 2 * 256 * 4;
+constexpr size_t kTablesOffEntries = 66048 + 512, kTablesBytes = kTablesOffEntries + 2 * 256 * 8;
 constexpr size_t kStateOffResc = 2 * sizeof(ChainBandState), kStateOffIdent = kStateOffResc + 512,
                  kStateOffFloor = kStateOffIdent + 16, kStateBytes = kStateOffFloor + 16;
 
@@ -143,8 +143,7 @@
         ChainRepredictArgs ra{};
         ra.spec = d_spec; ra.resc_in = state + kStateOffResc; ra.floor_out = reinterpret_cast<int *>(state + kStateOffFloor);
         ra.tables = ctx->tables.as<uint8_t>(); ra.supp_rg = consts + kChainOffSupp; ra.blue_pair_supp = consts + kChainOffBlue;
-        ra.blue_pq = ctx->blue_factors_ok ? reinterpret_cast<const float *>(consts + kChainOffBluePQ) : nullptr;
-        ra.blue_by_level = reinterpret_cast<float *>(ctx->tables.as<uint8_t>() + kTablesOffPQ);
+        ra.blue_pq = T.pa.blue_pq; ra.entries = T.pa.entries; ra.skip_pairs = T.pa.skip_pairs;
         ra.stripes = reduce ? 1u : 0u;
         {
             KernelTimer t(ctx, "chain_repredict");
@@ -243,8 +242,9 @@
         pa.supp_rg = consts + kChainOffSupp; pa.blue_pair_supp = consts + kChainOffBlue;
         pa.force = spec_force_flags(ctx);
         pa.allow_rescaled = ctx->attrs.on(A_NO_SPEC_RESCALE) ? 0u : 1u;
-        pa.blue_pq = ctx->blue_factors_ok ? reinterpret_cast<const float *>(consts + kChainOffBluePQ) : nullptr;
-        pa.blue_by_level = reinterpret_cast<float *>(ctx->tables.as<uint8_t>() + kTablesOffPQ);
+        pa.blue_pq = ctx->blue_factors_ok && !ctx->attrs.on(A_NO_BLUE_FACTORS) ? reinterpret_cast<const float *>(consts + kChainOffBluePQ) : nullptr;
+        pa.entries = reinterpret_cast<uint32_t *>(ctx->tables.as<uint8_t>() + kTablesOffEntries);
+        pa.skip_pairs = 1u;
         pa_first = pa;
         KernelTimer t(ctx, "chain_predict");
         HIPCHK(ctx, launch_chain_predict(pa, ctx->stream));
@@ -344,8 +344,7 @@
         fa.in_pitch = J.in_pitch; fa.rgb = d_rgb; fa.rgb_pitch_px = rgb_pitch_px;
         fa.rects = J.plan->d_rgb_rects.as<Rect>(); fa.nrects = (int)J.plan->rgb_rects.size();
         fa.row_w = J.plan->d_row_w.as<RowWeight>(); fa.col_w = J.plan->d_col_w.as<RowWeight>(); fa.row_off = (int32_t)J.row0;
-        fa.dev_state = d_state; fa.spec = d_spec; fa.tables = ctx->tables.as<uint8_t>();
-        fa.blue_by_level = ctx->blue_factors_ok ? reinterpret_cast<const float *>(ctx->tables.as<uint8_t>() + kTablesOffPQ) : nullptr;
+        fa.dev_state = d_state; fa.spec = d_spec; fa.entries = reinterpret_cast<const uint2 *>(ctx->tables.as<uint8_t>() + kTablesOffEntries);
         fa.sat_ok = J.plan->sat_ok ? 1u : 0u; fa.sat_col = J.plan->d_sat_col.as<uint8_t>(); fa.sat_row = J.plan->d_sat_row.as<uint8_t>() + J.row0;
         fa.sat_cols = (uint32_t)(round_up(J.cols, 64) + 64);
         const uint32_t fused_stride = ctx->attrs.is_set(A_SAMPLE_STRIDE) ? sample_stride : 33u;
diff --git a/sarpro_amd/csrc/chain_kernels.h b/sarpro_amd/csrc/chain_kernels.h
--- a/sarpro_amd/csrc/chain_kernels.h
+++ b/sarpro_amd/csrc/chain_kernels.h
@@ -82,7 +82,8 @@
     uint32_t force;
     uint32_t allow_rescaled;
     const float *blue_pq;
-    float *blue_by_level;
+    uint32_t *entries;
+    uint32_t skip_pairs;
     uint32_t second;
 };
 hipError_t launch_chain_predict(const ChainPredictArgs &a, hipStream_t s);
@@ -94,7 +95,8 @@
     const uint8_t *supp_rg;
     const uint8_t *blue_pair_supp;
     const float *blue_pq;
-    float *blue_by_level;
+    uint32_t *entries;
+    uint32_t skip_pairs;
     uint32_t stripes;
 };
 hipError_t launch_chain_repredict(const ChainRepredictArgs &a, hipStream_t s);
diff --git a/sarpro_amd/csrc/chain_kernels.hip b/sarpro_amd/csrc/chain_kernels.hip
--- a/sarpro_amd/csrc/chain_kernels.hip
+++ b/sarpro_amd/csrc/chain_kernels.hip
@@ -492,9 +492,16 @@
     }
 }
 
+__device__ __forceinline__ void write_level_entries(uint32_t *entries, const float *pq, int t, uint8_t r, uint8_t g, bool water1, bool water2) {
+    entries[2 * t] = __float_as_uint(pq[r]);
+    entries[2 * t + 1] = (uint32_t)r | (water1 ? 0x80000000u : 0u);
+    entries[512 + 2 * t] = __float_as_uint(pq[256 + g]);
+    entries[512 + 2 * t + 1] = ((uint32_t)g << 8) | (water2 ? 0x80000000u : 0u);
+}
+
 __global__ __launch_bounds__(kStatsBlock) void k_chain_predict(ChainPredictArgs a) {
-    if (a.second && !(a.spec->spec_ok == kSpecRescaled && a.spec->verdict == 1u && !a.spec->pool_overflow && a.spec->retry_min == 1u &&
-                      !a.spec->retried && !(a.spec->force & kSpecForceNoRetry))) return;
+    if (a.second && !(a.spec->verdict == 1u && !a.spec->pool_overflow && a.spec->retry_min == 1u &&
+                      !a.spec->retried && !(a.force & kSpecForceNoRetry))) return;
     __shared__ double est[2][256], fin[2][256];
     __shared__ uint8_t resc[2][256];
     __shared__ int s_ok[2], s_fwc, s_f;
@@ -571,6 +578,7 @@
         }
         bool ok = s_ok[0] && s_ok[1];
         if (a.force & kSpecForceNoSpec) ok = false;
+        if (a.entries && !a.blue_pq) ok = false;
         if (a.force & kSpecForceMispredict) f = f < kSpecFloorCap ? f + 1 : kSpecFloorCap - 1;
         if (a.force & kSpecForceMispredict2) f = f + 2 <= kSpecFloorCap ? f + 2 : (f >= 2 ? f - 2 : f);
         for (int i = 0; i <= f && i < 64; ++i) { if (i < f) lt0 += fin[0][i] + fin[1][i]; lt1 += fin[0][i] + fin[1][i]; }
@@ -622,10 +630,10 @@
     if (blockIdx.x == 0 && t < 256) {
         const int r1 = resc[0][t], r2 = resc[1][t];
         const uint8_t r = r1 <= fwc ? 0 : lut_r[r1], g = r2 <= fwc ? 0 : lut_g[r2];
-        R2[t] = r;
-        G2[t] = g;
-        if (a.blue_pq && a.blue_by_level) { a.blue_by_level[t] = a.blue_pq[r]; a.blue_by_level[256 + t] = a.blue_pq[256 + g]; }
-    }
+        if (!a.skip_pairs) { R2[t] = r; G2[t] = g; }
+        if (a.blue_pq && a.entries) write_level_entries(a.entries, a.blue_pq, t, r, g, r1 <= fwc, r2 <= fwc);
+    }
+    if (a.skip_pairs) return;
     for (int i = blockIdx.x * kStatsBlock + t; i < 65536; i += gridDim.x * kStatsBlock) {
         const int r1 = resc[0][i >> 8], r2 = resc[1][i & 255];
         B2[i] = (r1 <= fwc && r2 <= fwc) ? 0 : a.blue_pair_supp[((size_t)lut_r[r1] << 8) | lut_g[r2]];
@@ -667,11 +675,10 @@
     if (blockIdx.x == 0 && t < 256) {
         const int r1 = resc[0][t], r2 = resc[1][t];
         const uint8_t r = r1 <= fwc ? 0 : lut_r[r1], g = r2 <= fwc ? 0 : lut_g[r2];
-        R2[t] = r;
-        G2[t] = g;
-        if (a.blue_pq && a.blue_by_level) { a.blue_by_level[t] = a.blue_pq[r]; a.blue_by_level[256 + t] = a.blue_pq[256 + g]; }
-    }
-    for (int i = blockIdx.x * kStatsBlock + t; i < 65536; i += gridDim.x * kStatsBlock) {
+        if (!a.skip_pairs) { R2[t] = r; G2[t] = g; }
+        if (a.blue_pq && a.entries) write_level_entries(a.entries, a.blue_pq, t, r, g, r1 <= fwc, r2 <= fwc);
+    }
+    for (int i = blockIdx.x * kStatsBlock + t; i < (a.skip_pairs ? 0 : 65536); i += gridDim.x * kStatsBlock) {
         const int r1 = resc[0][i >> 8], r2 = resc[1][i & 255];
         B2[i] = (r1 <= fwc && r2 <= fwc) ? 0 : a.blue_pair_supp[((size_t)lut_r[r1] << 8) | lut_g[r2]];
     }
@@ -776,11 +783,11 @@
     return hipGetLastError();
 }
 hipError_t launch_chain_repredict(const ChainRepredictArgs &a, hipStream_t s) {
-    hipLaunchKernelGGL(k_chain_repredict, dim3(64), dim3(kStatsBlock), 0, s, a);
+    hipLaunchKernelGGL(k_chain_repredict, dim3(a.skip_pairs ? 1 : 64), dim3(kStatsBlock), 0, s, a);
     return hipGetLastError();
 }
 hipError_t launch_chain_predict(const ChainPredictArgs &a, hipStream_t s) {
-    hipLaunchKernelGGL(k_chain_predict, dim3(64), dim3(kStatsBlock), 0, s, a);
+    hipLaunchKernelGGL(k_chain_predict, dim3(a.skip_pairs ? 1 : 64), dim3(kStatsBlock), 0, s, a);
     return hipGetLastError();
 }
 hipError_t launch_chain_remap(const uint8_t *src, size_t src_pitch, uint8_t *dst, size_t dst_pitch, uint32_t rows,
diff --git a/sarpro_amd/csrc/context.h b/sarpro_amd/csrc/context.h
--- a/sarpro_amd/csrc/context.h
+++ b/sarpro_amd/csrc/context.h
@@ -158,7 +158,7 @@
     X(STRIP_ALIGN) X(PIECE_ALIGN) X(CHUNK_ROWS) X(RGB_ITEM_ROWS) X(SAMPLE_ITEM_ROWS) \
     X(NO_MAILBOX) X(NO_STEP_ESTIMATE) X(F32_ZONES) X(F32_ZONES_DEBUG) X(F32_DIRECT) X(F32_DIRECT_QCAP) X(F32_LEVEL_GENERAL) \
     X(F32_LEVEL_TABLE) X(F32_LEVEL_QCAP) X(F32_HOST_CDFS) X(F32_NO_VEC8) X(NO_BAND_TWIN) X(RESIZE_GENERIC) X(NO_RESIZE_LUT) \
-    X(NO_U16_CF) X(U16_ITEM_ROWS) X(PIPE_LANES) X(PIPE_ORDER) X(RGB_GRID) X(PIECE_GRID) X(COMM_RECORD) X(COMM_REPLAY) X(NO_SPEC_RESCALE) X(RGB_TAIL_ROWS) X(RGB_TAIL_ITEM_ROWS)
+    X(NO_U16_CF) X(U16_ITEM_ROWS) X(PIPE_LANES) X(PIPE_ORDER) X(RGB_GRID) X(PIECE_GRID) X(COMM_RECORD) X(COMM_REPLAY) X(NO_SPEC_RESCALE) X(RGB_TAIL_ROWS) X(RGB_TAIL_ITEM_ROWS) X(NO_BLUE_FACTORS)
 namespace sarpro {
 enum Attr : int {
 #define X(n) A_##n,
diff --git a/sarpro_amd/csrc/host_logic.cpp b/sarpro_amd/csrc/host_logic.cpp
--- a/sarpro_amd/csrc/host_logic.cpp
+++ b/sarpro_amd/csrc/host_logic.cpp
@@ -468,6 +468,21 @@
     return ok ? tab : nullptr;
 }
 const uint8_t *synrgb_blue_pair_default() { return blue_pair_table(true); }
+
+bool synrgb_level_entries(int fwc, const uint8_t *resc1, const uint8_t *resc2, uint32_t *out) {
+    const float *pq = synrgb_blue_factors_supp();
+    if (!pq) return false;
+    const uint8_t *lut_r = synrgb_supp_rg_tables() + (size_t)fwc * 512, *lut_g = lut_r + 256;
+    for (unsigned v = 0; v < 256; ++v) {
+        const unsigned r1 = resc1[v], r2 = resc2[v];
+        const unsigned r = lut_r[r1], g = lut_g[r2];
+        std::memcpy(&out[2 * v], &pq[r], 4);
+        out[2 * v + 1] = r | ((int)r1 <= fwc ? kLevelEntryWater : 0u);
+        std::memcpy(&out[512 + 2 * v], &pq[256 + g], 4);
+        out[512 + 2 * v + 1] = (g << 8) | ((int)r2 <= fwc ? kLevelEntryWater : 0u);
+    }
+    return true;
+}
 
 const double *gamma_level_thresholds_u8() {
     static double tab[3][256];
@@ -602,6 +617,12 @@
         if (floor_out) *floor_out = -1;
     }
     return SARPRO_HIP_OK;
+}
+
+int sarpro_hip_host_synrgb_level_entries(int floor_with_cushion, const uint8_t resc1[256], const uint8_t resc2[256],
+                                         uint32_t entries_out[1024]) {
+    if (!resc1 || !resc2 || !entries_out || floor_with_cushion < 0 || floor_with_cushion > 40) return SARPRO_HIP_ERR_INVALID_ARG;
+    return synrgb_level_entries(floor_with_cushion, resc1, resc2, entries_out) ? SARPRO_HIP_OK : SARPRO_HIP_ERR_UNSUPPORTED_SHAPE;
 }
 
 int sarpro_hip_host_clahe_shape_ok(size_t rows, size_t cols) { return clahe_shape_ok(rows, cols) ? 1 : 0; }
diff --git a/sarpro_amd/csrc/host_logic.h b/sarpro_amd/csrc/host_logic.h
--- a/sarpro_amd/csrc/host_logic.h
+++ b/sarpro_amd/csrc/host_logic.h
@@ -58,6 +58,8 @@
 const uint8_t *synrgb_supp_rg_tables();
 const uint8_t *synrgb_blue_pair_supp();
 const float *synrgb_blue_factors_supp();
+constexpr uint32_t kLevelEntryWater = 0x80000000u;
+bool synrgb_level_entries(int floor_with_cushion, const uint8_t *resc1, const uint8_t *resc2, uint32_t *out );
 const uint8_t *synrgb_blue_pair_default();
 const double *gamma_level_thresholds_u8();
 
diff --git a/sarpro_amd/csrc/kernels.h b/sarpro_amd/csrc/kernels.h
--- a/sarpro_amd/csrc/kernels.h
+++ b/sarpro_amd/csrc/kernels.h
@@ -122,9 +122,8 @@
     int32_t row_off;
     const struct ChainBandState *dev_state;
     struct ChainSpecState *spec;
-    const uint8_t *tables;
+    const uint2 *entries;
     const uint8_t *sat_col, *sat_row;
-    const float *blue_by_level;
     uint32_t no_verdict;
     uint32_t sat_cols;
     uint32_t sat_ok;
diff --git a/sarpro_amd/csrc/kernels.hip b/sarpro_amd/csrc/kernels.hip
--- a/sarpro_amd/csrc/kernels.hip
+++ b/sarpro_amd/csrc/kernels.hip
@@ -612,6 +612,7 @@
 constexpr uint32_t kPartialHistLevels = 64;
 typedef float v2f __attribute__((ext_vector_type(2)));
 typedef float v4f __attribute__((ext_vector_type(4)));
+typedef uint32_t v2u __attribute__((ext_vector_type(2)));
 constexpr uint32_t kSpecLutMaxEntries = 16384;
 
 #ifndef SARPRO_CDF_COPIES
@@ -639,12 +640,6 @@
 __device__ __forceinline__ float to_sgpr(float x) {
     return __builtin_bit_cast(float, __builtin_amdgcn_readfirstlane(__builtin_bit_cast(int, x)));
 }
-__device__ __forceinline__ uint32_t lshl_or(uint32_t hi, uint32_t sh, uint32_t lo) {
-    uint32_t d;
-    asm("v_lshl_or_b32 %0, %1, %2, %3" : "=v"(d) : "v"(hi), "n"(sh), "v"(lo));
-    return d;
-}
-#define pack4(b0, b1, b2, b3) lshl_or(lshl_or((b3), 8, (b2)), 16, lshl_or((b1), 8, (b0)))
 __device__ __forceinline__ uint32_t to_sgpr_u32(uint32_t x) { return (uint32_t)__builtin_amdgcn_readfirstlane((int)x); }
 __device__ __forceinline__ double to_sgpr(double x) {
     const unsigned long long u = __builtin_bit_cast(unsigned long long, x);
@@ -1149,20 +1144,15 @@
     }
 }
 
-#ifndef SARPRO_RGB_B2_STRIDE
-#define SARPRO_RGB_B2_STRIDE 260
-#endif
-constexpr uint32_t kRgbB2Stride = SARPRO_RGB_B2_STRIDE;
-static_assert(kRgbB2Stride == 256 || kRgbB2Stride == 260, "blue table rows: 256 (as in global memory) or 260 bytes");
 #ifndef SARPRO_RGB_BLOCK
 #define SARPRO_RGB_BLOCK 1024
 #endif
 #ifndef SARPRO_RGB_POOL
-#define SARPRO_RGB_POOL (SARPRO_RGB_B2_STRIDE == 256 ? 3072 : 3008)
+#define SARPRO_RGB_POOL 3008
 #endif
 constexpr int kRgbBlock = SARPRO_RGB_BLOCK, kRgbWaves = kRgbBlock / kWave;
 constexpr uint32_t kRgbPoolEntries = SARPRO_RGB_POOL;
-constexpr uint32_t kRgbTableBytes = 512 + 256 * kRgbB2Stride;
+constexpr uint32_t kRgbTableBytes = 65536;
 struct RgbLds {
     static constexpr uint32_t tables = 0;
     static constexpr uint32_t stage = kRgbTableBytes;
@@ -1206,10 +1196,8 @@
             for (uint32_t i = threadIdx.x; i <= win_hi[b]; i += kRgbBlock) lds[RgbLds::binof + kb[b] + i] = a.binlut[b][i];
     }
     {
-        const uint32_t *src = reinterpret_cast<const uint32_t *>(a.tables);
-        for (int i = threadIdx.x; i < 512 / 4; i += kRgbBlock) LDS_AT(uint32_t, RgbLds::tables + 4 * i) = src[i];
-        for (int i = threadIdx.x; i < 65536 / 4; i += kRgbBlock)
-            LDS_AT(uint32_t, RgbLds::tables + 512 + (uint32_t)(i >> 6) * kRgbB2Stride + (uint32_t)(i & 63) * 4u) = src[128 + i];
+        for (uint32_t i = threadIdx.x; i < kRgbTableBytes / 8u; i += kRgbBlock)
+            LDS_AT(v2u, RgbLds::tables + 8u * i) = reinterpret_cast<const v2u *>(a.entries)[((i >> 4) & 1u) * 256u + (i >> 5)];
     }
     const uint32_t fpred = (uint32_t)sp->floor_pred;
     const uint32_t t4[3] = {(fpred ? fpred - 1u : 0u) * 0x01010101u, fpred * 0x01010101u, (fpred + 1u) * 0x01010101u};
@@ -1233,6 +1221,8 @@
     }
     const RowWeight *__restrict__ row_w = a.row_w + a.row_off;
     const uint32_t stage_w = RgbLds::stage + (uint32_t)wave * 1536u;
+    const bool swap_bands = (lane & 16) != 0;
+    const uint32_t ecopy = ((uint32_t)(lane & 15) << 3) | (swap_bands ? 128u : 0u), ecopy_other = ecopy ^ 128u;
 
     uint32_t *const s_next = reinterpret_cast<uint32_t *>(lds + RgbLds::misc) + 8;
     uint32_t *const s_rect = reinterpret_cast<uint32_t *>(lds + RgbLds::misc) + 16;
@@ -1540,23 +1530,30 @@
                     }
                     n_all += 16u; n_kept += 2u * nkeep;
                     uint32_t o[6];
+                    v2u e1[VEC], e2[VEC];
+                    const uint32_t la[2] = {swap_bands ? l2[0] : l1[0], swap_bands ? l2[1] : l1[1]}, lb[2] = {swap_bands ? l1[0] : l2[0], swap_bands ? l1[1] : l2[1]};
+#pragma unroll
+                    for (int j = 0; j < VEC; ++j) {
+                        const uint32_t sel = to_sgpr_u32(0x0c0c0400u + 0x0100u * (uint32_t)(j & 3));
+                        e1[j] = LDS_AT(v2u, RgbLds::tables + __builtin_amdgcn_perm(la[j >> 2], ecopy, sel));
+                        e2[j] = LDS_AT(v2u, RgbLds::tables + __builtin_amdgcn_perm(lb[j >> 2], ecopy_other, sel));
+                    }
 #pragma unroll
                     for (int g = 0; g < 2; ++g) {
-                        uint32_t px[4][3];
+                        const v2u *p = e1 + 4 * g, *q = e2 + 4 * g;
+                        float bl[4];
+                        uint32_t m[4];
 #pragma unroll
                         for (int j = 0; j < 4; ++j) {
-                            const uint32_t v1 = j == 0 ? (l1[g] & 0xFFu) : j == 3 ? (l1[g] >> 24) : __builtin_amdgcn_ubfe(l1[g], 8 * j, 8);
-                            const uint32_t v2 = j == 0 ? (l2[g] & 0xFFu) : j == 3 ? (l2[g] >> 24) : __builtin_amdgcn_ubfe(l2[g], 8 * j, 8);
-                            uint32_t pair;
-                            if (kRgbB2Stride == 256) pair = __builtin_amdgcn_perm(l1[g], l2[g], to_sgpr_u32(0x0c0c0400u + 0x0101u * (uint32_t)j));
-                            else asm("v_mad_u32_u24 %0, %1, %2, %3" : "=v"(pair) : "v"(v1), "s"(kRgbB2Stride), "v"(v2));
-                            px[j][0] = LDS_AT(uint8_t, RgbLds::tables + v1);
-                            px[j][1] = LDS_AT(uint8_t, RgbLds::tables + 256 + v2);
-                            px[j][2] = LDS_AT(uint8_t, RgbLds::tables + 512 + pair);
+                            bl[j] = __uint_as_float(__float_as_uint(__uint_as_float(p[j].x) * __uint_as_float(q[j].x)) | (p[j].y & q[j].y));
+                            m[j] = p[j].y | q[j].y;
                         }
-                        o[3 * g + 0] = pack4(px[0][0], px[0][1], px[0][2], px[1][0]);
-                        o[3 * g + 1] = pack4(px[1][1], px[1][2], px[2][0], px[2][1]);
-                        o[3 * g + 2] = pack4(px[2][2], px[3][0], px[3][1], px[3][2]);
+                        const uint32_t w0 = __builtin_amdgcn_perm(m[1], m[0], to_sgpr_u32(0x040c0100u));
+                        const uint32_t w1 = __builtin_amdgcn_perm(m[2], m[1], to_sgpr_u32(0x05040c01u));
+                        const uint32_t w2 = __builtin_amdgcn_perm(m[3], m[3], to_sgpr_u32(0x0c01000cu));
+                        o[3 * g + 0] = __builtin_amdgcn_cvt_pk_u8_f32(bl[0], 2, w0);
+                        o[3 * g + 1] = __builtin_amdgcn_cvt_pk_u8_f32(bl[1], 1, w1);
+                        o[3 * g + 2] = __builtin_amdgcn_cvt_pk_u8_f32(bl[3], 3, __builtin_amdgcn_cvt_pk_u8_f32(bl[2], 0, w2));
                     }
                     *reinterpret_cast<uint2 *>(lds + stage_w + lane * 24) = make_uint2(o[0], o[1]);
                     *reinterpret_cast<uint2 *>(lds + stage_w + lane * 24 + 8) = make_uint2(o[2], o[3]);
```

Result: no change. 437,400, median of 6 (+1.3%).
